# zyt334/AdaFace

Hardware: AMD Instinct MI355X
Metric: 512x512 images/sec @ 50 DDIM steps, batch 8 (higher is better)
Workload: dtype bf16

## Files before the change

### adaface_amd/_lib.py

```python
from __future__ import annotations

import ctypes as C
import os
from pathlib import Path

AF_DTYPE_BF16 = 0
AF_DTYPE_F32 = 1
AF_DTYPE_F16 = 2
DTYPES = {"bf16": AF_DTYPE_BF16, "bfloat16": AF_DTYPE_BF16, "f32": AF_DTYPE_F32, "fp32": AF_DTYPE_F32,
          "float32": AF_DTYPE_F32, "f16": AF_DTYPE_F16, "fp16": AF_DTYPE_F16, "float16": AF_DTYPE_F16}

_LIB_PATH = Path(__file__).resolve().parent / "libadaface_hip.so"


class AfConfig(C.Structure):
    _fields_ = [
        ("dtype", C.c_int),
        ("build_unet", C.c_int),
        ("in_channels", C.c_int), ("model_channels", C.c_int), ("out_channels", C.c_int),
        ("num_res_blocks", C.c_int),
        ("n_attention_resolutions", C.c_int), ("attention_resolutions", C.c_int * 8),
        ("n_channel_mult", C.c_int), ("channel_mult", C.c_int * 8),
        ("num_heads", C.c_int), ("context_dim", C.c_int), ("transformer_depth", C.c_int),
        ("n_context_layers", C.c_int),
        ("build_vae", C.c_int),
        ("vae_ch", C.c_int), ("vae_out_ch", C.c_int), ("vae_num_res_blocks", C.c_int),
        ("vae_z_channels", C.c_int), ("vae_embed_dim", C.c_int),
        ("n_vae_ch_mult", C.c_int), ("vae_ch_mult", C.c_int * 8),
        ("build_vae_encoder", C.c_int), ("vae_in_channels", C.c_int),
        ("build_clip", C.c_int),
        ("clip_vocab", C.c_int), ("clip_hidden", C.c_int), ("clip_layers", C.c_int), ("clip_heads", C.c_int),
        ("clip_intermediate", C.c_int), ("clip_max_pos", C.c_int),
    ]


class AfError(RuntimeError):
    pass


_lib = None

_P = C.c_void_p
_SIGS = [
    ("af_last_error", C.c_char_p, []),
    ("af_version", C.c_int, []),
    ("af_create", C.c_int, [C.c_int, C.POINTER(AfConfig), C.POINTER(_P)]),
    ("af_destroy", None, [_P]),
    ("af_load_tensor", C.c_int, [_P, C.c_char_p, _P, C.c_int, C.POINTER(C.c_int64)]),
    ("af_load_tensor_device", C.c_int, [_P, C.c_char_p, _P, C.c_int, C.POINTER(C.c_int64)]),
    ("af_num_tensors", C.c_int, [_P]),
    ("af_tensor_name", C.c_char_p, [_P, C.c_int]),
    ("af_tensor_loaded", C.c_int, [_P, C.c_int]),
    ("af_tensor_shape", C.c_int, [_P, C.c_int, C.POINTER(C.c_int64)]),
    ("af_set_context", C.c_int, [_P, _P, C.c_int, C.c_int, C.c_int, _P]),
    ("af_unet_forward", C.c_int, [_P, _P, _P, _P, C.c_int, C.c_int, C.c_int, _P]),
    ("af_unet_forward_twin", C.c_int, [_P, _P, _P, _P, C.c_int, C.c_int, C.c_int, _P]),
    ("af_ddim_step", C.c_int, [_P, _P, _P, _P, C.c_int64, C.c_float, C.c_float, C.c_float, C.c_float, C.c_float,
                               C.c_float, _P, _P, _P]),
    ("af_lincomb", C.c_int, [_P, C.c_int64, _P, C.c_float, _P, C.c_float, _P, C.c_float, _P, C.c_float, C.c_int, _P]),
    ("af_vae_decode", C.c_int, [_P, _P, C.c_float, _P, _P, C.c_int, C.c_int, C.c_int, _P]),
    ("af_to_uint8", C.c_int, [_P, _P, C.c_int, C.c_int, C.c_int, _P]),
    ("af_arena_bytes", C.c_int64, [_P]),
    ("af_prof_enable", C.c_int, [C.c_int]),
    ("af_prof_reset", C.c_int, []),
    ("af_set_conv_attn", C.c_int, [_P, C.c_int, C.c_int, C.POINTER(C.c_int), C.POINTER(C.c_int)]),
    ("af_vae_encode", C.c_int, [_P, _P, _P, C.c_int, C.c_int, C.c_int, _P]),
    ("af_posterior_sample", C.c_int, [_P, _P, C.c_float, _P, C.c_int, C.c_int, C.c_int, _P]),
    ("af_prof_set_stride", C.c_int, [C.c_int]),
    ("af_last_gemm_plan", C.c_int, [C.POINTER(C.c_int), C.POINTER(C.c_int), C.POINTER(C.c_int)]),
    ("af_prof_collect", C.c_int, [C.c_int, C.POINTER(C.c_double), C.POINTER(C.c_int64), C.POINTER(C.c_double),
                                  C.POINTER(C.c_double)]),
    ("af_prof_event_overhead_us", C.c_double, [_P, C.c_int]),
    ("af_unet_num_blocks", C.c_int, [_P]),
    ("af_unet_block_shape", C.c_int, [_P, C.c_int, C.c_int, C.c_int, C.POINTER(C.c_int), C.POINTER(C.c_int), C.POINTER(C.c_int)]),
    ("af_unet_set_tap", C.c_int, [_P, C.c_int, _P]),
    ("af_gemm_plan_counts", C.c_int, [C.POINTER(C.c_int64)]),
    ("af_gemm_plan_counts_reset", C.c_int, []),
    ("af_knob_set", C.c_int, [C.c_char_p, C.c_int]),
    ("af_knob_get", C.c_int, [C.c_char_p, C.POINTER(C.c_int)]),
    ("af_knob_reset", C.c_int, []),
    ("af_op_conv2d", C.c_int, [C.c_int, _P, _P, _P, _P, _P] + [C.c_int] * 9 + [_P]),
    ("af_op_linear", C.c_int, [C.c_int, _P, _P, _P, _P, _P, C.c_int64, C.c_int, C.c_int, C.c_int, _P]),
    ("af_op_groupnorm", C.c_int, [C.c_int, _P, _P, _P, C.c_float, C.c_int, _P, C.c_int, C.c_int, C.c_int, C.c_int, _P]),
    ("af_op_conv_gn", C.c_int, [_P, _P, _P, _P, _P, _P, C.c_float, C.c_int, _P, _P] + [C.c_int] * 5 + [_P]),
    ("af_set_fp8", C.c_int, [_P, C.c_int]),
    ("af_fp8_gemm_launches", C.c_int64, []),
    ("af_set_fp8_scope", C.c_int, [_P, C.c_int]),
    ("af_get_fp8_scope", C.c_int, [_P]),
    ("af_ff8_launches", C.c_int64, []),
    ("af_op_ff_fp8", C.c_int, [_P] * 4 + [C.c_float] + [_P] * 5 + [C.c_int64] + [C.c_int] * 5 + [_P, _P, _P, C.POINTER(C.c_int), _P]),
    ("af_fp8_num_sites", C.c_int, [_P]),
    ("af_fp8_site_name", C.c_char_p, [_P, C.c_int]),
    ("af_fp8_record", C.c_int, [_P, C.c_int, _P]),
    ("af_fp8_read_record", C.c_int, [_P, C.c_int, C.POINTER(C.c_float), C.POINTER(C.c_int64), _P]),
    ("af_fp8_get_shifts", C.c_int, [_P, C.c_int, C.POINTER(C.c_int)]),
    ("af_fp8_set_shifts", C.c_int, [_P, C.c_int, C.POINTER(C.c_int)]),
    ("af_fp8_shift_for_amax", C.c_int, [C.c_float, C.c_int]),
    ("af_halo8_launches", C.c_int64, []),
    ("af_rowpanel_launches", C.c_int64, []),
    ("af_up_phase4_launches", C.c_int64, []),
    ("af_gn_producer_launches", C.c_int64, []),
    ("af_attn_short_launches", C.c_int64, []),
    ("af_gn_consumer_launches", C.c_int64, []),
    ("af_xattn_fused_launches", C.c_int64, []),
    ("af_conv_attn_short_launches", C.c_int64, []),
    ("af_op_conv_attention", C.c_int, [C.c_int, _P, _P, _P, _P] + [C.c_int] * 6 + [C.c_float] + [C.c_int] * 3 + [_P]),
    ("af_op_xattn_fused", C.c_int, [C.c_void_p] * 10 + [C.c_int] * 3 + [C.c_void_p]),
    ("af_op_conv2d_fp8", C.c_int, [_P, _P, _P, _P, _P] + [C.c_int] * 10 + [_P]),
    ("af_op_groupnorm_fp8", C.c_int, [_P, _P, _P, C.c_float, C.c_int, _P, C.c_int, C.c_int, C.c_int, C.c_int, C.c_int, _P]),
    ("af_op_layernorm_fp8", C.c_int, [_P, _P, _P, C.c_float, _P, C.c_int64, C.c_int, C.c_int, _P]),
    ("af_op_groupnorm_fp8_rec", C.c_int, [_P, _P, _P, C.c_float, C.c_int, _P, C.c_int, C.c_int, C.c_int, C.c_int, C.c_int, _P, _P]),
    ("af_op_layernorm_fp8_rec", C.c_int, [_P, _P, _P, C.c_float, _P, C.c_int64, C.c_int, C.c_int, _P, _P]),
    ("af_op_layernorm", C.c_int, [C.c_int, _P, _P, _P, C.c_float, _P, C.c_int64, C.c_int, _P]),
    ("af_op_attention", C.c_int, [C.c_int, _P, _P, _P, _P, C.c_int, C.c_int, C.c_int, C.c_int, C.c_int, C.c_float, C.c_int, _P]),
    ("af_clip_embed_tokens", C.c_int, [_P, _P, C.c_int64, _P, _P]),
    ("af_clip_text_forward", C.c_int, [_P, _P, C.c_int, C.c_int, C.c_float, C.c_float, _P, _P]),
    ("af_clip_text_forward3", C.c_int, [_P, _P, C.c_int, C.c_int, C.c_float, C.c_float, C.c_float, _P, _P]),
    ("af_op_timestep_embedding", C.c_int, [C.c_int, _P, _P, C.c_int, C.c_int, _P]),
    ("af_op_gn_conv1x1", C.c_int, [_P, _P, _P, C.c_float, _P, _P, _P, _P] + [C.c_int] * 5 + [_P]),
    ("af_flops_issued", C.c_double, [C.c_int]),
    ("af_clock_probe", C.c_int, [_P, C.c_int, C.POINTER(C.c_double), C.POINTER(C.c_double)]),
]
EXPORTED_SYMBOLS = [s[0] for s in _SIGS]


def lib_path() -> Path:
    return _LIB_PATH


def load():
    global _lib
    if _lib is not None:
        return _lib
    if not _LIB_PATH.exists():
        raise AfError(
            f"{_LIB_PATH} not found: build it with `python -m adaface_amd.build` (needs hipcc). "
            "adaface_amd has no fallback path.")
    lib = C.CDLL(os.fspath(_LIB_PATH))
    for name, res, args in _SIGS:
        fn = getattr(lib, name)
        fn.restype = res
        fn.argtypes = args
    _lib = lib
    return lib


def set_knob(name: str, value: int) -> None:
    check(load().af_knob_set(name.encode(), int(value)), f"af_knob_set({name})")


def reset_knobs() -> None:
    load().af_knob_reset()


def plan_counts(reset: bool = False) -> dict:
    lib = load()
    c = (C.c_int64 * 10)()
    check(lib.af_gemm_plan_counts(c), "af_gemm_plan_counts")
    out = {f"tile{i}": int(c[i]) for i in range(6)}
    out["halo"], out["splitk"], out["ln_consumer"], out["ln_producer"] = int(c[6]), int(c[7]), int(c[8]), int(c[9])
    out["fp8"] = int(lib.af_fp8_gemm_launches())
    out["ff8"] = int(lib.af_ff8_launches())
    out["halo8"] = int(lib.af_halo8_launches())
    out["rowpanel"] = int(lib.af_rowpanel_launches())
    out["up_phase4"] = int(lib.af_up_phase4_launches())
    out["gn_producer"] = int(lib.af_gn_producer_launches())
    out["attn_short"] = int(lib.af_attn_short_launches())
    out["gn_consumer"] = int(lib.af_gn_consumer_launches())
    out["xattn_fused"] = int(lib.af_xattn_fused_launches())
    out["conv_attn_short"] = int(lib.af_conv_attn_short_launches())
    if reset:
        lib.af_gemm_plan_counts_reset()
    return out


def check(rc: int, what: str = "") -> None:
    if rc != 0:
        msg = load().af_last_error().decode("utf-8", "replace")
        raise AfError(f"{what or 'libadaface_hip'} failed (rc={rc}): {msg}")


def stream_ptr():
    import torch
    return C.c_void_p(torch.cuda.current_stream().cuda_stream)


def ptr(t):
    return C.c_void_p(0 if t is None else t.data_ptr())
```

### adaface_amd/csrc/af_common.h

```cpp
#pragma once
#include <hip/hip_runtime.h>
#include <stdint.h>
#include <atomic>

typedef __bf16 bf16;
typedef __attribute__((ext_vector_type(8))) __bf16 bf16x8;
typedef _Float16 f16;
typedef __attribute__((ext_vector_type(8))) _Float16 f16x8;
enum AfStorage { AF_ST_BF16 = 0, AF_ST_F32 = 1, AF_ST_F16 = 2 };
template <typename T> struct StorageOf;
template <> struct StorageOf<__bf16> { static constexpr AfStorage value = AF_ST_BF16; };
template <> struct StorageOf<float> { static constexpr AfStorage value = AF_ST_F32; };
template <> struct StorageOf<_Float16> { static constexpr AfStorage value = AF_ST_F16; };
typedef __attribute__((ext_vector_type(16))) float f32x16;
typedef __attribute__((ext_vector_type(4))) float f32x4;

#define AF_WAVE 64

#define HIP_CHECK_RET(expr)                                                       \
  do {                                                                            \
    hipError_t _e = (expr);                                                       \
    if (_e != hipSuccess) {                                                       \
      af_set_error_msg("%s failed: %s (%s:%d)", #expr, hipGetErrorString(_e),     \
                       __FILE__, __LINE__);                                       \
// ... 32 lines not shown
    if (on) af_prof_begin_impl(cls, s, flops, bytes);
  }
  ~AfProfScope() {
    if (on) af_prof_end_impl(s);
  }
};

struct AfKnobs {
  int splitk_target;
  int conv_halo;
  int gemm_pp;
  int gemm_pp_minfill;
  int gemm_tile;
  int gemm_splitk;
  int gemm_groupm;
  int gemm_dma;
  int attn_ring;
  int gn_small;
  int ln_fuse;
  int geglu_rowpanel;
  int conv_halo8;
  int ablate;
  int gn_producer;
  int conv_up_phase4;
  int attn_short;
  int gemm_m128;
  int small_m_tile64;
  int gn_consumer;
  int xattn_fused;
  int plan_log;
  int ff8_min_k;
  int ff8_min_rows;
  int conv_attn_short;
};
extern AfKnobs g_af_knobs;

template <typename T> __device__ __forceinline__ float to_f32(T v);
template <> __device__ __forceinline__ float to_f32<float>(float v) { return v; }
template <> __device__ __forceinline__ float to_f32<bf16>(bf16 v) { return (float)v; }
template <> __device__ __forceinline__ float to_f32<f16>(f16 v) { return (float)v; }

template <typename T> __device__ __forceinline__ T from_f32(float v);
template <> __device__ __forceinline__ float from_f32<float>(float v) { return v; }
template <> __device__ __forceinline__ bf16 from_f32<bf16>(float v) { return (bf16)v; }
template <> __device__ __forceinline__ f16 from_f32<f16>(float v) { return (f16)v; }

template <typename T> struct Vec16 {
  static constexpr int N = 16 / sizeof(T);
  union {
    uint4 u;
    T e[N];
  };
};

template <typename T> struct Quad;
template <> struct Quad<bf16> {
  union {
    uint2 u;
    bf16 e[4];
  };
  __device__ __forceinline__ void load(const bf16* p) { u = *reinterpret_cast<const uint2*>(p); }
  __device__ __forceinline__ void store(bf16* p) const { *reinterpret_cast<uint2*>(p) = u; }
};
template <> struct Quad<f16> {
  union {
    uint2 u;
// ... 109 lines not shown
    c = __builtin_amdgcn_mfma_f32_32x32x2f32(__builtin_bit_cast(float, a.y),
                                             __builtin_bit_cast(float, b.y), c, 0, 0, 0);
    c = __builtin_amdgcn_mfma_f32_32x32x2f32(__builtin_bit_cast(float, a.z),
                                             __builtin_bit_cast(float, b.z), c, 0, 0, 0);
    c = __builtin_amdgcn_mfma_f32_32x32x2f32(__builtin_bit_cast(float, a.w),
                                             __builtin_bit_cast(float, b.w), c, 0, 0, 0);
  }
};

__device__ __forceinline__ int acc_row(int r, int h) { return (r & 3) + 8 * (r >> 2) + 4 * h; }

enum { AF_EPI_NONE = 0, AF_EPI_GEGLU = 1 };

struct ConvGemmParams {
  const void* src;
  long src_batch_stride;
  int ldc;
  int Cin;
  int Hs, Ws;
  int up;
  int Hi, Wi;
  int Ho, Wo;
  int ks, stride, pad;
  const void* W;
  int ldw;
  int Wrows;
  int M, N, K;
  int k_logical;
  const float* bias;
  const void* rowbias;
  int ldrb;
  const void* residual;
  int ldr;
  void* out;
  int ldo;
  int epilogue;
  float alpha;
  long bs_src, bs_w, bs_out, bs_res;
  int splitk;
  void* ws;
  int group_m;
  int howo_shift, wo_shift;
  float* ln_stats_out;
  const float* ln_stats;
  const float* ln_colsum;
  int ln_parts_n;
  float ln_inv_count, ln_eps;
  int epi_direct;
  int ablate;
  int fp8;
  const unsigned char* w_scale;
  int x_scale_e8;
  const void* W_up4;
  int phase4;
  float* gn_stats_out;
  int gn_cpg;
  const float* gn_ab;
  int gn_hw;
};

struct AfGemmPlan {
  int tile;
  int splitk;
  size_t ws_bytes;
  int halo_tw;
  int group_m;
// ... 13 lines not shown
```

### adaface_amd/csrc/af_conv_gemm.hip

```cpp
#include "af_kernels.h"

#include <cstdlib>
#include <cstring>
#include <mutex>
#include <type_traits>

template <int BM, int BN> struct TileCfg {
  static constexpr int XR = BM / 32, WR = BN / 32;
  static constexpr int WM = BM / 2, WN = BN / 2;
  static constexpr int MI = WM / 32, NI = WN / 32;
  static constexpr int TILE_BYTES = (BM + BN) * 128;
  static constexpr int EPI_LD = BN + 4;
  static constexpr int EPI_BYTES = BM * EPI_LD * 4;
  static constexpr int LDS_BYTES = (2 * TILE_BYTES > EPI_BYTES) ? 2 * TILE_BYTES : EPI_BYTES;
};

__device__ __forceinline__ void lds_dma16(__amdgpu_buffer_rsrc_t rs, char* lds_base, unsigned voffset, unsigned soffset) {
#if defined(__HIP_DEVICE_COMPILE__)
  __builtin_amdgcn_raw_ptr_buffer_load_lds(rs, (__attribute__((address_space(3))) void*)lds_base, 16, voffset, soffset,
                                           0, 0);
#endif
}

__device__ __forceinline__ void tile_coords(int wg, int nwg, int ntm, int ntn, int gm, int& tm, int& tn) {
// ... 1016 lines not shown
  static constexpr int KC = KC_, MJ = MJ_, K = KC * 64, D = D_, NS = D_ + 1;
  static constexpr int WROWS = 16 * MJ, BM = 8 * WROWS;
  static constexpr int BN = GEGLU ? 128 : 160;
  static constexpr int WBYTES = BN * 128, WPIECES = BN / 8;
  static constexpr int NIW = BN / 16;
  static constexpr int OCOLS = GEGLU ? BN / 2 : BN;
  static constexpr int OPITCH = OCOLS * 2 + 16, OBYTES = WROWS * OPITCH;
  static constexpr int LDS_BYTES = NS * WBYTES + 8 * OBYTES;
  static constexpr int CPR = OCOLS / 8;
  static constexpr int NST = WROWS * CPR / 64;
  static_assert(LDS_BYTES <= 160 * 1024 && (WROWS * CPR) % 64 == 0 && (MJ * KC == 10 || (MJ == 1 && KC == 20)) && D >= 2 && D <= KC,
                "row-panel LDS / store mapping / 80 (K = 1280, 16 rows per wave: 160) fragment registers / ring depth");
};
typedef RowPanelCfgT<true> RowPanelCfg;

template <bool GEGLU, int LNMODE, bool RES, int KC_ = 5, int MJ_ = 2, int D_ = 2>
__global__ __launch_bounds__(512) void rowpanel_kernel(const ConvGemmParams p) {
  using C = RowPanelCfgT<GEGLU, KC_, MJ_, D_>;
  typedef bf16 T;
  constexpr int KC = C::KC, NIW = C::NIW, MJ = C::MJ, NST = C::NST, CPR = C::CPR, D = C::D, NS = C::NS;
  static_assert(!(GEGLU && (RES || LNMODE == 2)), "GEGLU: plain or LayerNorm-consumer epilogue, no residual");
  extern __shared__ __attribute__((aligned(1024))) char smem[];
  const int tid = threadIdx.x, lane = tid & 63, wid = __builtin_amdgcn_readfirstlane(tid >> 6);
  const int m0 = blockIdx.x * C::BM;
  const int r0 = m0 + wid * C::WROWS;
  const int ntn_all = p.N / C::BN;
  const int nt_begin = (int)((long)blockIdx.y * ntn_all / gridDim.y), nt_end = (int)((long)(blockIdx.y + 1) * ntn_all / gridDim.y);
  const int ntn = nt_end - nt_begin;
  const __amdgpu_buffer_rsrc_t rs_x = __builtin_amdgcn_make_buffer_rsrc(
      const_cast<T*>(reinterpret_cast<const T*>(p.src)), 0, (int)0xFFFFFFF0u, 0x00020000);
  const __amdgpu_buffer_rsrc_t rs_w = __builtin_amdgcn_make_buffer_rsrc(
      const_cast<T*>(reinterpret_cast<const T*>(p.W)), 0, (int)0xFFFFFFF0u, 0x00020000);
  const __amdgpu_buffer_rsrc_t rs_o = __builtin_amdgcn_make_buffer_rsrc(reinterpret_cast<T*>(p.out), 0, (int)0xFFFFFFF0u, 0x00020000);

  float* vecs = reinterpret_cast<float*>(smem + C::LDS_BYTES);
  const int nvcol = ntn * C::BN;
  float4 vb[3], vc[3];
#pragma unroll
  for (int r = 0; r < 3; ++r) {
    const int c4 = tid + 512 * r;
    const int col = nt_begin * C::BN + 4 * c4;
    vb[r] = vc[r] = float4{0.f, 0.f, 0.f, 0.f};
    if (c4 < nvcol / 4) {
      if (p.bias) vb[r] = *reinterpret_cast<const float4*>(p.bias + col);
      if constexpr (LNMODE == 1) vc[r] = *reinterpret_cast<const float4*>(p.ln_colsum + col);
    }
  }

  pp_u32x4 xr[MJ][KC][2];
  unsigned orow[NST];
#pragma unroll
  for (int i = 0; i < NST; ++i) {
    const int c = lane + 64 * i;
    const int row = c / CPR, ch = c - row * CPR;
    const int m = r0 + row;
    orow[i] = m < p.M ? (unsigned)((long)m * p.ldo * 2) + (unsigned)ch * 16u : 0xFFFFFFFFu;
  }
  float ln_mu[LNMODE == 1 ? MJ : 1], ln_rs[LNMODE == 1 ? MJ : 1];
#pragma unroll
  for (int j = 0; j < MJ; ++j) {
    const int m = r0 + j * 16 + (lane & 15);
    const bool ok = m < p.M;
    const unsigned xo = ok ? (unsigned)((long)m * p.ldc * 2) + (unsigned)(lane >> 4) * 16u : 0xFFFFFFFFu;
#pragma unroll
    for (int kc = 0; kc < KC; ++kc)
#pragma unroll
// ... 197 lines not shown
        }
      }
    } else {
      constexpr int NH = NIW / 2;
      static_assert(NIW % 2 == 0, "row-panel: even number of 16-column blocks");
      float ps[MJ], pq[MJ];
#pragma unroll
      for (int j = 0; j < MJ; ++j) ps[j] = pq[j] = 0.f;
#pragma unroll
      for (int hh = 0; hh < 2; ++hh) {
        float4 bvec[NH], cvec[LNMODE == 1 ? NH : 1];
        {
          const unsigned va = lds0 + (unsigned)C::LDS_BYTES + (unsigned)((ntl * C::BN + hh * NH * 16 + cl) * 4);
          pp_u32x4 tb[NH], tc[LNMODE == 1 ? NH : 1];
          pp_static_for<0, NH>([&](auto ic) {
            constexpr int ii = decltype(ic)::value;
            tb[ii] = pp_lds_read128<ii * 64>(va);
            if constexpr (LNMODE == 1) tc[ii] = pp_lds_read128<ii * 64>(va + (unsigned)nvcol * 4u);
          });
          pp_wait_lgkm0();
#pragma unroll
          for (int ii = 0; ii < NH; ++ii) {
            asm volatile("" : "+v"(tb[ii]));
            bvec[ii] = __builtin_bit_cast(float4, tb[ii]);
            if constexpr (LNMODE == 1) { asm volatile("" : "+v"(tc[ii])); cvec[ii] = __builtin_bit_cast(float4, tc[ii]); }
          }
        }
#pragma unroll
        for (int j = 0; j < MJ; ++j) {
          const int m = r0 + j * 16 + (lane & 15);
          const bool mok = m < p.M;
          Quad<T> rq[RES ? NH : 1];
          if constexpr (RES) {
            const T* rp = reinterpret_cast<const T*>(p.residual) + (long)(mok ? m : 0) * p.ldr + ncol + hh * NH * 16 + cl;
#pragma unroll
            for (int ii = 0; ii < NH; ++ii) rq[ii].load(rp + ii * 16);
          }
#pragma unroll
          for (int ii = 0; ii < NH; ++ii) {
            const int i = hh * NH + ii;
            const float* bp = reinterpret_cast<const float*>(&bvec[ii]);
            const float* cp = reinterpret_cast<const float*>(&cvec[LNMODE == 1 ? ii : 0]);
            Quad<T> o;
#pragma unroll
            for (int e = 0; e < 4; ++e) {
              float v;
              if constexpr (LNMODE == 1) v = (acc[i][j][e] - ln_mu[j] * cp[e]) * ln_rs[j] + bp[e];
              else v = acc[i][j][e] * p.alpha + bp[e];
              if constexpr (RES) v += to_f32<T>(rq[ii].e[e]);
              o.e[e] = from_f32<T>(v);
              if constexpr (LNMODE == 2) {
                const float vr = mok ? to_f32<T>(o.e[e]) : 0.f;
                ps[j] += vr;
                pq[j] += vr * vr;
              }
            }
            o.store(reinterpret_cast<T*>(otile + (j * 16 + (lane & 15)) * C::OPITCH) + i * 16 + cl);
          }
        }
        __builtin_amdgcn_sched_barrier(0);
      }
      if constexpr (LNMODE == 2) {
#pragma unroll
        for (int j = 0; j < MJ; ++j) {
          const int m = r0 + j * 16 + (lane & 15);
          float s1 = ps[j], s2 = pq[j];
          s1 += __shfl_xor(s1, 16, 64); s2 += __shfl_xor(s2, 16, 64);
// ... 1062 lines not shown
  const int lvl = g_af_knobs.geglu_rowpanel;
  if (!lvl || batch != 1 || p.ks != 1 || p.pad != 0 || p.stride != 1 || p.up != 0 || p.splitk > 1 || p.rowbias || p.fp8 ||
      p.Cin != p.K || p.ldc < p.Cin)
    return 0;
  const bool geglu = p.epilogue == AF_EPI_GEGLU;
  if (p.K == RowPanelCfg::K && p.M >= 128 * RowPanelCfg::BM) {
    if (p.gn_ab && (p.gn_hw <= 0 || p.gn_hw % RowPanelCfg::BM != 0)) return 0;
    if (geglu) return (p.N % RowPanelCfg::BN == 0 && !p.residual && !p.ln_stats_out) ? 1 : 0;
    return (lvl >= 2 && p.N % 160 == 0 && p.alpha == 1.0f && !(p.ln_stats && p.ln_stats_out) && (!p.residual || p.ldr % 4 == 0)) ? 2 : 0;
  }
  if (g_af_knobs.gemm_m128 && !geglu && !(p.ln_stats && p.ln_stats_out) && (!p.ln_stats || p.alpha == 1.0f) && !p.gn_ab && p.M % 128 == 0 &&
      p.M <= 8192 && p.N % 160 == 0 &&
      p.K % 64 == 0 && p.K >= 256 && (!p.residual || p.ldr % 4 == 0) && p.ldo % 8 == 0 && ((__UINTPTR_TYPE__)p.out & 15) == 0) {
    const long nb128 = (long)(p.M / 128) * (p.N / 160), nb256 = (long)((p.M + 255) / 256) * (p.N / 160);
    if (nb128 >= 128 && nb128 <= 512 && nb256 <= 170) return 6;
    if (nb128 % 256 == 0 && nb128 <= 1024 && nb256 % 256 != 0) return 6;
  }
  if (g_af_knobs.gemm_m128 && !geglu && !(p.ln_stats && p.ln_stats_out) && (!p.ln_stats || p.alpha == 1.0f) && !p.gn_ab && p.M % 128 == 0 &&
      p.M > 8192 && p.M <= 16384 && p.N % 160 == 0 && p.K % 64 == 0 && p.K >= 256 && p.K <= 1280 && (!p.residual || p.ldr % 4 == 0) &&
      p.ldo % 8 == 0 && ((__UINTPTR_TYPE__)p.out & 15) == 0 && (long)(p.M / 128) * (p.N / 160) == 512)
    return 6;
  if (p.K == 1280)
    return (lvl >= 4 && p.N == 1280 && p.M >= 4096 && !geglu && p.alpha == 1.0f && !p.ln_stats && !p.ln_stats_out && !p.gn_ab &&
            (!p.residual || p.ldr % 4 == 0)) ? 3 : 0;
  if (p.K == 640 && lvl >= 3 && p.M >= 16384 && !p.residual) {
    if (p.gn_ab) return 0;
    if (p.ln_stats_out) return 0;
    if (geglu) return p.N % 128 == 0 ? 4 : 0;
    return (p.N % 160 == 0 && p.N >= 1920 && p.alpha == 1.0f) ? 5 : 0;
  }
  return 0;
}

template <typename T>
int af_launch_conv_gemm(const ConvGemmParams& p_in, int batch, hipStream_t stream, const AfGemmPlan* plan, void* ws) {
  constexpr int BK = 128 / sizeof(T);
  ConvGemmParams p = p_in;
  if (p.fp8) {
    if constexpr (std::is_same_v<T, bf16>) return batch == 1 ? launch_conv_gemm_fp8(p, stream, plan, ws) : (af_set_error_msg("conv_gemm fp8: no batched form"), -1);
    else { af_set_error_msg("conv_gemm: fp8 operands need the bf16 storage mode"); return -1; }
  }
  if (p.gn_ab && !std::is_same_v<T, bf16>) { af_set_error_msg("conv_gemm: consumer-side GroupNorm exists on the bf16 row-panel kernels only"); return -1; }
  if (p.K % BK != 0 || p.Cin % BK != 0 || p.K != p.ks * p.ks * p.Cin) {
    af_set_error_msg("conv_gemm: K=%d Cin=%d ks=%d must satisfy K==ks*ks*Cin and Cin%%%d==0", p.K, p.Cin, p.ks, BK);
    return -1;
  }
  if (p.ldw % (16 / (int)sizeof(T)) != 0 || p.ldc % (16 / (int)sizeof(T)) != 0) {
    af_set_error_msg("conv_gemm: ldw/ldc must be multiples of 16 bytes");
    return -1;
  }
  if (p.N % 4 != 0 || p.ldo % 4 != 0 || (p.residual && p.ldr % 4 != 0) || (p.rowbias && p.ldrb % 4 != 0)) {
    af_set_error_msg("conv_gemm: N/ldo/ldr/ldrb must be multiples of 4 (N=%d ldo=%d)", p.N, p.ldo);
    return -1;
  }
  if (p.epilogue == AF_EPI_GEGLU && p.N % 64 != 0) { af_set_error_msg("conv_gemm: GEGLU needs N%%64==0"); return -1; }
  if (p.M <= 0 || p.N <= 0) return 0;
  {
    const int HoWo = p.Ho * p.Wo > 0 ? p.Ho * p.Wo : 1;
    const double nb = (double)((p.M + HoWo - 1) / HoWo);
    const double src_bytes = nb * (double)p.src_batch_stride * sizeof(T), w_bytes = (double)p.Wrows * p.ldw * sizeof(T);
    if (src_bytes >= 4294967280.0 || w_bytes >= 4294967280.0) {
      af_set_error_msg("conv_gemm: operand of %.2f GB exceeds the 4 GB range of the 32-bit gather offsets (split the batch)",
                       (src_bytes > w_bytes ? src_bytes : w_bytes) / 1e9);
      return -1;
    }
  }
  if constexpr (std::is_same_v<T, bf16>) {
    if (up_phase4_ok(p, batch)) return launch_up_phase4(p, stream);
  }
  AfGemmPlan pl = plan ? *plan : af_plan_conv_gemm(p, batch, StorageOf<T>::value);
  if (pl.splitk > 1 && !ws) pl.splitk = 1;
  if constexpr (std::is_same_v<T, bf16>) {
    if (pl.splitk > 1) {
      ConvGemmParams q = p;
// ... 13 lines not shown
  if (pl.splitk > 1) g_af_plan_counts[7] += 1;
  if (p.ln_stats) g_af_plan_counts[8] += 1;
  if (p.ln_stats_out) g_af_plan_counts[9] += 1;
  set_launch_fields(p, pl);
  if (p.gn_stats_out) {
    if (!std::is_same_v<T, bf16> || batch != 1 || !af_conv_gn_stats_ok(p, pl, p.gn_cpg)) {
      af_set_error_msg("conv_gemm: GroupNorm partial sums asked of a launch that cannot write them (ask af_conv_gn_stats_ok first)");
      return -1;
    }
    g_af_plan_counts[14] += 1;
  }
  const int prof_cls = pl.halo_tw == 256 ? AF_K_HALO8
                       : pl.tile == 5 ? ((p.ks == 1 && p.pad == 0) ? AF_K_PP160_PLAIN : AF_K_PP160_GATHER)
                                      : (pl.tile == 4 ? AF_K_PP128 : AF_K_CONV_GEMM);
  AfProfScope prof(prof_cls, stream, 2.0 * p.M * (double)p.N * (p.k_logical ? p.k_logical : p.K) * batch,
                   ((double)p.M * p.K / (p.ks * p.ks) + (double)p.N * p.K + (double)p.M * p.N) * batch * sizeof(T));
  int rc;
  int rk_pre = 0;
  if constexpr (std::is_same_v<T, bf16>) rk_pre = af_conv_rowpanel_kind(p, batch);
  if ((p.ln_stats || p.ln_stats_out) && rk_pre != 6 && !(pl.tile >= 4 && !pl.halo_tw)) {
    af_set_error_msg("conv_gemm: LayerNorm-fused launch planned on a kernel without that epilogue (tile %d)", pl.tile);
    return -1;
  }
  if constexpr (std::is_same_v<T, bf16>) {
    const int rk = rk_pre;
    if (p.ln_parts_n > 0 && !rk) {
      af_set_error_msg("conv_gemm: un-finalised LayerNorm statistics handed to a launch that is not a row-panel one");
      return -1;
    }
    if (p.gn_ab && !rk) {
      af_set_error_msg("conv_gemm: consumer-side GroupNorm asked of a launch that is not a row-panel one (ask af_conv_rowpanel_kind first)");
      return -1;
    }
    if (p.gn_ab) g_af_gn_consumer_launches += 1;
    if (rk) g_af_plan_counts[12] += 1;
    switch (rk) {
      case 1: return launch_geglu_rowpanel(p, stream);
      case 2: return launch_plain_rowpanel(p, stream);
      case 3: return launch_plain_rowpanel_k1280(p, stream);
      case 4: return launch_geglu_rowpanel(p, stream, true);
      case 5: return launch_plain_rowpanel(p, stream, true);
      case 6: return launch_gemm_m128(p, stream);
      default: break;
    }
  }
  if (pl.halo_tw == 8 || pl.halo_tw == 256) {
    if constexpr (std::is_same_v<T, bf16>) {
      rc = pl.halo_tw == 8 ? af_launch_conv_s8(p, stream) : launch_halo8(p, stream);
    } else {
      af_set_error_msg(pl.halo_tw == 8 ? "conv_gemm: the 8 x 8-map kernel is bf16 only" : "conv_gemm: the eight-wave halo kernel is bf16 only");
      return -1;
    }
  } else if (pl.halo_tw) {
    const bool bn128 = pl.tile == 0 || pl.tile == 1;
    if (pl.halo_tw == 32) return bn128 ? launch_halo<T, 32, 128>(p, stream) : launch_halo<T, 32, 64>(p, stream);
    return bn128 ? launch_halo<T, 16, 128>(p, stream) : launch_halo<T, 16, 64>(p, stream);
  } else {
    switch (pl.tile) {
      case 4:
      case 5:
        if constexpr (std::is_same_v<T, bf16>) {
          rc = pl.tile == 4 ? launch_pp<128>(p, stream) : launch_pp<160>(p, stream);
        } else {
          af_set_error_msg("conv_gemm: ping-pong tiles are bf16 only");
          return -1;
        }
// ... 15 lines not shown
```

### adaface_amd/csrc/af_kernels.h

```cpp
#pragma once
#include "af_common.h"

AfGemmPlan af_plan_conv_gemm(const ConvGemmParams& p, int batch, AfStorage st);
template <typename T>
int af_launch_conv_gemm(const ConvGemmParams& p, int batch, hipStream_t stream, const AfGemmPlan* plan = nullptr,
                        void* ws = nullptr);
template <typename T> int af_launch_attention(const AttnParams& p, int B, int dh, hipStream_t stream);
template <typename T> long af_attn_short_pack_elems(int B, int H, int dh, int Nk);
template <typename T>
int af_launch_attn_short_pack(const void* v, int ldv, long bsv, int Nk, int H, int dh, int B, void* vt, hipStream_t stream);
extern std::atomic<long> g_af_attn_short_launches;
bool af_conv_attn_short_ok(bool is_bf16, int dh, int Nk, bool vt_pack, int ks, int groups);
int af_launch_conv_attn_short(const AttnParams& p, int B, int dh, int ks, int groups, int Hh, int Ww, const float* amap,
                              hipStream_t stream);
extern std::atomic<long> g_af_conv_attn_short_launches;
struct AfXattnFusedParams {
  const void* x; int ldx; int M; int rows_per_sample;
  const float* ln_stats; int ln_parts_n; float ln_inv_count, ln_eps;
  const void* wq; int ldwq; const float* q_colsum; const float* q_bias;
  const void* kvpack;
  const void* wo; int ldwo; const float* o_bias;
  void* out; int ldo;
  float* ln_stats_out;
  int Nk;
};
bool af_xattn_fused_ok(int M, int rows_per_sample, int C, int H, int dh, int Nk);
long af_xattn_fused_pack_elems(int B, int H, int dh, int Nk);
int af_launch_xattn_fused_pack(const void* kv, int ldk, long bsk, int Nk, int B, void* pack, hipStream_t stream);
int af_launch_xattn_fused_permute_wo(const void* w, int ldw, int rows, void* wp, int ldp, hipStream_t stream);
int af_launch_xattn_fused(const AfXattnFusedParams& a, hipStream_t stream);
extern std::atomic<long> g_af_xattn_fused_launches;

bool af_ff_geglu_fp8_ok(const ConvGemmParams& p);
int af_launch_ff_geglu_fp8(ConvGemmParams p, float out_mul, unsigned* rec, hipStream_t stream);
extern std::atomic<long> g_af_ff8_launches;

size_t af_gn_workspace_bytes(int B, int HW);
template <typename T>
int af_launch_groupnorm(const void* x, long x_bs, int ldx, int B, int HW, int Cn, const float* gamma,
                        const float* beta, float eps, int silu, void* y, long y_bs, int ldy, void* workspace,
                        hipStream_t stream, float fp8_mul = 0.f,
                        const float* pre_partial = nullptr, int pre_npart = 0,
                        unsigned* fp8_rec = nullptr);
template <typename T>
int af_launch_groupnorm_fold(const void* x, long x_bs, int ldx, int B, int HW, int Cn, const float* gamma, const float* beta,
                             float eps, void* workspace, hipStream_t stream, const float* pre_partial, int pre_npart,
                             float* ab_out);
bool af_conv_gn_stats_ok(const ConvGemmParams& p, const AfGemmPlan& pl, int cpg);
bool af_conv_s8_ok(const ConvGemmParams& p, int batch);
int af_conv_s8_slices(const ConvGemmParams& p, int batch);
int af_launch_conv_s8(const ConvGemmParams& p, hipStream_t stream);
int af_conv_rowpanel_kind(const ConvGemmParams& p, int batch);
template <typename T>
int af_launch_layernorm(const void* x, int ldx, long rows, int Cn, const float* gamma, const float* beta,
                        float eps, void* y, int ldy, hipStream_t stream, float fp8_mul = 0.f, unsigned* fp8_rec = nullptr);

template <typename T>
int af_launch_nchw_to_nhwc(const float* x, void* y, int B, int Cn, int HW, int Cpad, float scale, hipStream_t s);
template <typename T> int af_launch_nhwc_to_nchw(const void* x, float* y, int B, int Cn, int HW, int ld, hipStream_t s);
template <typename T> int af_launch_cast_f32(const float* x, void* y, long n, hipStream_t s);
template <typename T>
int af_launch_gather_rows_cast(const float* x, const int* rowmap, void* y, long rows, int D, hipStream_t s);
template <typename T>
int af_launch_conv_attn(const void* q, int ldq, long bsq, const void* kv, int ldk, long bsk, int tok0, float* sN,
// ... 49 lines not shown
```

### adaface_amd/csrc/af_model.hip

```cpp
#include "../../include/adaface_hip.h"
#include "af_kernels.h"

#include <cmath>
#include <cstdarg>
#include <cstdio>
#include <cstdlib>
#include <cstring>
#include <algorithm>
#include <map>
#include <memory>
#include <string>
#include <vector>

static thread_local char g_err[1024] = "";
void af_set_error_msg(const char* fmt, ...) {
  va_list ap;
  va_start(ap, fmt);
  vsnprintf(g_err, sizeof(g_err), fmt, ap);
  va_end(ap);
}
static int knob_env(const char* name, int dflt) {
  const char* s = getenv(name);
  return s ? atoi(s) : dflt;
}
AfKnobs g_af_knobs = {
    knob_env("AF_SPLITK_TARGET", 320), knob_env("AF_CONV_HALO", 1),       knob_env("AF_GEMM_PP", 1),
    knob_env("AF_GEMM_PP_MINFILL", 50), knob_env("AF_GEMM_TILE", -1),
    knob_env("AF_GEMM_SPLITK", -1),    knob_env("AF_GEMM_GROUPM", -1),    knob_env("AF_GEMM_DMA", -1),
    knob_env("AF_ATTN_RING", 3),       knob_env("AF_GN_SMALL", 1),
    knob_env("AF_LN_FUSE", 1),         knob_env("AF_GEGLU_ROWPANEL", 4), knob_env("AF_CONV_HALO8", 3), knob_env("AF_ABLATE", 0),
    knob_env("AF_GN_PRODUCER", 1),     knob_env("AF_CONV_UP_PHASE4", 1), knob_env("AF_ATTN_SHORT", 1),
    knob_env("AF_GEMM_M128", 1),       knob_env("AF_SMALL_M_TILE64", 1),  knob_env("AF_GN_CONSUMER", 1),
    knob_env("AF_XATTN_FUSED", 1),     knob_env("AF_PLAN_LOG", 0),      knob_env("AF_FF8_MIN_K", 512),   knob_env("AF_FF8_MIN_ROWS", 0),
    knob_env("AF_CONV_ATTN_SHORT", 1)};
static const AfKnobs g_af_knobs_initial = g_af_knobs;
static int* knob_slot(const char* name) {
  static const struct { const char* n; int AfKnobs::*m; } tab[] = {
      {"splitk_target", &AfKnobs::splitk_target}, {"conv_halo", &AfKnobs::conv_halo}, {"gemm_pp", &AfKnobs::gemm_pp},
      {"gemm_pp_minfill", &AfKnobs::gemm_pp_minfill},
      {"gemm_tile", &AfKnobs::gemm_tile}, {"gemm_splitk", &AfKnobs::gemm_splitk}, {"gemm_groupm", &AfKnobs::gemm_groupm},
      {"gemm_dma", &AfKnobs::gemm_dma}, {"attn_ring", &AfKnobs::attn_ring},
      {"gn_small", &AfKnobs::gn_small}, {"ln_fuse", &AfKnobs::ln_fuse},
      {"geglu_rowpanel", &AfKnobs::geglu_rowpanel}, {"conv_halo8", &AfKnobs::conv_halo8}, {"ablate", &AfKnobs::ablate}, {"gn_producer", &AfKnobs::gn_producer}, {"conv_up_phase4", &AfKnobs::conv_up_phase4},
      {"attn_short", &AfKnobs::attn_short},
      {"gemm_m128", &AfKnobs::gemm_m128}, {"small_m_tile64", &AfKnobs::small_m_tile64}, {"gn_consumer", &AfKnobs::gn_consumer}, {"xattn_fused", &AfKnobs::xattn_fused}, {"plan_log", &AfKnobs::plan_log}, {"ff8_min_k", &AfKnobs::ff8_min_k}, {"ff8_min_rows", &AfKnobs::ff8_min_rows},
      {"conv_attn_short", &AfKnobs::conv_attn_short}};
  if (!name) return nullptr;
  for (auto& t : tab)
    if (strcmp(t.n, name) == 0) return &(g_af_knobs.*(t.m));
  return nullptr;
}

int g_af_prof_enabled = 0;
int g_af_prof_stride = 1;
std::atomic<long> g_af_prof_seen[AF_K_COUNT] = {};
std::atomic<double> g_af_flops_issued{0.0};
namespace {
struct ProfRec {
  hipEvent_t start, stop;
  int cls;
  double flops, bytes;
};
std::vector<ProfRec> g_prof_recs;
std::vector<hipEvent_t> g_prof_pool;
size_t g_prof_pool_used = 0;
hipEvent_t prof_event() {
  if (g_prof_pool_used == g_prof_pool.size()) {
    hipEvent_t e;
    hipEventCreate(&e);
    g_prof_pool.push_back(e);
  }
  return g_prof_pool[g_prof_pool_used++];
}
}
void af_prof_begin_impl(int cls, hipStream_t s, double flops, double bytes) {
  ProfRec r;
  r.start = prof_event();
  r.stop = prof_event();
  r.cls = cls;
// ... 151 lines not shown
  std::vector<VLevel> vlevels;
  Linear quant_conv, enc_conv_in, enc_conv_out;
  Norm enc_norm_out;
  VaeAttnW eattn;
  std::vector<Linear> edown;
  int emid1 = -1, emid2 = -1;
  std::vector<VLevel> elevels;

  void* clip_tok = nullptr;
  void* clip_pos = nullptr;
  std::vector<ClipLayerW> clip_layers;
  Norm clip_final_ln;

  int conv_ks = 0;
  std::vector<int> conv_batch;
  std::vector<int> conv_tokens;
  int* ctx_rowmap = nullptr;
  size_t ctx_rowmap_n = 0;

  bool ln_fold_dirty = true;
  bool fp8_on = false;
  bool fp8_dirty = true;
  int fp8_scope = AF_FP8_SCOPE_BASE;
  int fp8_nbase = 0;
  int fp8_nsites() const { return (fp8_scope & AF_FP8_SCOPE_FF) ? (int)fp8_shift.size() : fp8_nbase; }
  std::vector<int> fp8_shift;
  std::vector<std::string> fp8_site_names;
  unsigned* fp8_rec = nullptr;
  bool fp8_recording = false;
  bool up4_dirty = true;
  float* gn_carry = nullptr;
  size_t gn_carry_bytes = 0, gn_carry_need = 0;

  int tap_index = -1;
  float* tap_out = nullptr;

  Arena arena;
  float* stage = nullptr;
  size_t stage_bytes = 0;
  std::vector<CtxKV> ctx_kv;
  void* ctx_cast = nullptr;
  size_t ctx_cast_bytes = 0;
  int ctx_Bf = 0, ctx_tokens = 0;
  bool ctx_set = false;
};

struct Builder {
  af_handle* h;
  int rc = 0;
  void* dmalloc(size_t bytes, bool zero = true) {
    void* p = nullptr;
    if (hipMalloc(&p, bytes) != hipSuccess) {
      af_set_error_msg("hipMalloc(%zu) failed", bytes);
      rc = AF_ERR_HIP;
      return nullptr;
    }
    if (zero) hipMemset(p, 0, bytes);
    h->owned.push_back(p);
    return p;
  }
  void add_slot(const std::string& name, const Slot& s) {
    h->slots[name] = s;
    h->slot_names.push_back(name);
  }
  void alloc_linear(Linear& L, int cin, int cout_rows, int ks, bool pad_cin) {
    const int bk = bk_of(h->dtype);
// ... 489 lines not shown
    Act f8 = x8;
    f8.C = f8.ld = ff2.cin;
    ConvGemmParams p;
    conv_params(p, ff1, x8, f8, 1, 0, nullptr, nullptr, 0, ff1.cout, -1);
    return af_ff_geglu_fp8_ok(p) && fp8_capable(ff2, f8, out);
  }
  int ff_geglu8(const Linear& L, const Act& x8, Act& y8) {
    AF_TRY(check(y8));
    if (!x8.f8 || !y8.f8 || !L.w8) { af_set_error_msg("ff_geglu8: e4m3 operands and an fp8 weight twin needed"); return AF_ERR_STATE; }
    ConvGemmParams p;
    conv_params(p, L, x8, y8, 1, 0, nullptr, nullptr, 0, L.cout, -1);
    if (dry) return 0;
    return af_launch_ff_geglu_fp8(p, ldexpf(1.f, y8.f8_shift), fp8_rec_of(y8), s);
  }
  int ln_capable(const Linear& L, const Act& x, const Act& out, int n_valid = -1) const {
    if (dt != AF_DTYPE_BF16 || L.ks != 1) return 0;
    ConvGemmParams p;
    conv_params(p, L, x, out, 1, 0, nullptr, nullptr, 0, n_valid, -1);
    const AfGemmPlan pl = af_plan_conv_gemm(p, 1, storage_of(dt));
    if (pl.tile < 4 || pl.splitk > 1 || pl.halo_tw) return 0;
    return (p.N / (pl.tile == 5 ? 160 : 128)) * 2;
  }
  bool rowpanel_capable(const Linear& L, const Act& x, const Act& out, const LnArgs* ln, int gn_hw) const {
    if (dt != AF_DTYPE_BF16 || L.ks != 1 || x.f8) return false;
    ConvGemmParams p;
    conv_params(p, L, x, out, 1, 0, nullptr, nullptr, 0, -1, -1);
    if (ln) { p.ln_stats = ln->stats; p.ln_colsum = ln->colsum; p.ln_stats_out = ln->stats_out; }
    p.gn_ab = reinterpret_cast<const float*>(1);
    p.gn_hw = gn_hw;
    const AfGemmPlan pl = af_plan_conv_gemm(p, 1, storage_of(dt));
    p.splitk = pl.splitk;
    return af_conv_rowpanel_kind(p, 1) != 0;
  }
  int groupnorm_fold(const Norm& N, const Act& x, float* ab) {
    const int HW = x.H * x.W;
    void* ws = A.alloc(af_gn_workspace_bytes(x.B, HW));
    if (!ws || !ab) { af_set_error_msg("arena exhausted (groupnorm fold)"); return AF_ERR_STATE; }
    if (dry) return 0;
    if (x.C != N.C) { af_set_error_msg("groupnorm: C mismatch %d vs %d", x.C, N.C); return AF_ERR_INVALID; }
    const float* pre = g_af_knobs.gn_producer ? x.gn_part : nullptr;
    return DISPATCH(dt, af_launch_groupnorm_fold<bf16>(x.p, (long)HW * x.ld, x.ld, x.B, HW, x.C, N.gamma, N.beta, N.eps, ws, s, pre, x.gn_npart, ab),
                    af_launch_groupnorm_fold<float>(x.p, (long)HW * x.ld, x.ld, x.B, HW, x.C, N.gamma, N.beta, N.eps, ws, s, pre, x.gn_npart, ab),
                    af_launch_groupnorm_fold<f16>(x.p, (long)HW * x.ld, x.ld, x.B, HW, x.C, N.gamma, N.beta, N.eps, ws, s, pre, x.gn_npart, ab));
  }
  int conv(const Linear& L, const Act& x, Act& out, int stride, int up, const Act* residual, const void* rowbias,
           int ldrb, int n_valid = -1, int pad = -1, const LnArgs* ln = nullptr, int want_gn = 0) {
    AF_TRY(check(out));
    out.gn_part = nullptr; out.gn_npart = 0;
    ConvGemmParams p;
    conv_params(p, L, x, out, stride, up, residual, rowbias, ldrb, n_valid, pad);
    bool ln_parts_pending = false;
    if (ln) {
      p.ln_stats = ln->stats; p.ln_colsum = ln->colsum;
      p.ln_stats_out = ln->stats_out;
      if (ln->parts_in) {
        p.ln_stats = ln->stats_buf;
        ln_parts_pending = true;
      }
      p.gn_ab = ln->gn_ab;
      p.gn_hw = ln->gn_hw;
    }
    if (x.C < L.cin || x.ld < L.cin_pad) {
      af_set_error_msg("conv: input has %d channels (ld %d), layer expects %d (padded %d)", x.C, x.ld, L.cin, L.cin_pad);
      return AF_ERR_INVALID;
    }
    if (x.f8 && (!L.w8 || ln)) { af_set_error_msg("conv: e4m3 input without an fp8 weight twin"); return AF_ERR_STATE; }
    const AfGemmPlan pl = af_plan_conv_gemm(p, 1, storage_of(dt));
    if (x.f8 && pl.tile < 4) { af_set_error_msg("conv: e4m3 input on a shape without an fp8 plan"); return AF_ERR_STATE; }
    if (ln_parts_pending) {
      ConvGemmParams q = p;
      q.splitk = pl.splitk;
      int kind = dt == AF_DTYPE_BF16 ? af_conv_rowpanel_kind(q, 1) : 0;
      if (!kind && dt == AF_DTYPE_BF16 && pl.splitk > 1) {
        q.splitk = 1;
        if (af_conv_rowpanel_kind(q, 1) == 6) kind = 6;
      }
      if (kind) {
        p.ln_stats = ln->parts_in;
        p.ln_parts_n = ln->parts_n;
        p.ln_inv_count = 1.0f / (float)ln->count;
        p.ln_eps = ln->eps;
      } else {
        AF_TRY(ln_finalize(ln->parts_in, ln->parts_n, (long)p.M, ln->count, ln->eps, ln->stats_buf));
// ... 92 lines not shown

static int run_resblock(Runner& R, const ResBlockW& w, const Act& x, Act& out, const void* emb_all, int emb_ld) {
  const size_t mk = R.A.mark();
  Act t2 = R.alloc_act(x.B, x.H, x.W, w.cout);
  Act t1 = R.fp8_capable(w.c1, x, t2) ? R.alloc_act8(x.B, x.H, x.W, x.C, w.c1) : R.alloc_act(x.B, x.H, x.W, x.C);
  AF_TRY(R.groupnorm(w.n1, x, t1, 1));
  const void* rb = (emb_all && w.emb_off >= 0) ? R.elem_ptr(const_cast<void*>(emb_all), w.emb_off) : nullptr;
  AF_TRY(R.conv(w.c1, t1, t2, 1, 0, nullptr, rb, emb_ld, -1, -1, nullptr, 1));
  Act t3 = R.fp8_capable(w.c2, t2, out) ? R.alloc_act8(x.B, x.H, x.W, w.cout, w.c2) : R.alloc_act(x.B, x.H, x.W, w.cout);
  AF_TRY(R.groupnorm(w.n2, t2, t3, 1));
  Act sk = x;
  if (w.has_skip) {
    sk = R.alloc_act(x.B, x.H, x.W, w.cout);
    AF_TRY(R.conv(w.skip, x, sk, 1, 0, nullptr, nullptr, 0));
  }
  AF_TRY(R.conv(w.c2, t3, out, 1, 0, &sk, nullptr, 0, -1, -1, nullptr, 2));
  R.A.release(mk);
  return 0;
}

static int run_xfmr(Runner& R, const XfmrW& w, const Act& x, Act& out, bool twin = false) {
  af_handle* h = R.h;
  const size_t mk = R.A.mark();
  const int Bh = x.B, B = twin ? 2 * x.B : x.B, H = x.H, W = x.W, N = H * W, C = w.heads * w.dh;
  auto half = [&](Act a) { if (twin) a.B = Bh; return a; };
  auto dup = [&](const Act& a) -> int {
    Act src = a, dst = a;
    src.B = dst.B = Bh;
    dst.p = R.elem_ptr(a.p, (long)Bh * a.H * a.W * a.ld);
    return R.copy_channels(src, dst, 0);
  };
  Act g = R.alloc_act(B, H, W, x.C);
  Act t = R.alloc_act(B, H, W, C);
  Act f_probe = t;
  f_probe.C = 4 * C; f_probe.ld = 4 * C;
  Act qkv_probe = t;
  qkv_probe.C = 3 * C; qkv_probe.ld = 3 * C;
  int ln_parts = 0;
  if (g_af_knobs.ln_fuse && !w.blocks.empty() && w.blocks[0].qkv1_ln.w) {
    const XfmrBlockW& b0 = w.blocks[0];
    const int pp = R.ln_capable(w.proj_in, g, t);
    const bool ok = pp > 0 && R.ln_capable(b0.out1, t, t) == pp && R.ln_capable(b0.out2, t, t) == pp &&
                    R.ln_capable(b0.ff2, f_probe, t) == pp && R.ln_capable(b0.qkv1_ln, t, qkv_probe) > 0 &&
                    R.ln_capable(b0.q2_ln, t, t) > 0 && R.ln_capable(b0.ff1_ln, t, f_probe, 8 * C) > 0;
    if (ok) ln_parts = pp;
    if (ok && twin) {
      const Act gh = half(g), th = half(t), qh = half(qkv_probe);
      if (R.ln_capable(w.proj_in, gh, th) != pp || R.ln_capable(b0.out1, th, th) != pp || R.ln_capable(b0.qkv1_ln, th, qh) <= 0)
        ln_parts = 0;
    }
  }
  const size_t st_elems = (size_t)ln_parts * B * N * 2;
  float* st_part = ln_parts ? reinterpret_cast<float*>(R.A.alloc(st_elems * sizeof(float))) : nullptr;
  float* st_row = ln_parts ? reinterpret_cast<float*>(R.A.alloc((size_t)B * N * 2 * sizeof(float))) : nullptr;
  if (ln_parts && !st_row) { af_set_error_msg("arena exhausted (LayerNorm statistics)"); return AF_ERR_STATE; }
  float *st_t = st_part, *st_1 = st_part, *st_2 = st_part;
  auto producer = [&](float* st) { Runner::LnArgs a; a.stats_out = st; return a; };
  auto consumer = [&](const float* st, const float* cs, const Norm& ln) {
    Runner::LnArgs a; a.colsum = cs;
    a.parts_in = st; a.parts_n = ln_parts; a.count = C; a.eps = ln.eps;
    a.stats_buf = st_row;
    return a;
  };
  auto consumer_final = [&](const float* cs) {
    Runner::LnArgs a; a.colsum = cs;
    a.stats = st_row;
// ... 24 lines not shown
    const bool pre = twin && d == 0;
    const int Bp = pre ? Bh : B;
    auto pv = [&](Act a) { a.B = Bp; return a; };
    Act n = R.alloc_act(B, H, W, C);
    Act qkv = R.alloc_act(B, H, W, 3 * C);
    {
      const Act tp = pv(t);
      Act np = pv(n), qkvp = pv(qkv);
      if (R.fp8_capable(blk.qkv1, tp, qkvp)) {
        Act n8 = R.alloc_act8(Bp, H, W, C, blk.qkv1);
        AF_TRY(R.layernorm(blk.ln1, tp, n8));
        AF_TRY(R.conv(blk.qkv1, n8, qkvp, 1, 0, nullptr, nullptr, 0));
      } else if (ln_parts) {
        const Runner::LnArgs ca = consumer(st_t, blk.qkv1_cs, blk.ln1);
        AF_TRY(R.conv(blk.qkv1_ln, tp, qkvp, 1, 0, nullptr, nullptr, 0, -1, -1, &ca));
      } else {
        AF_TRY(R.layernorm(blk.ln1, tp, np));
        AF_TRY(R.conv(blk.qkv1, np, qkvp, 1, 0, nullptr, nullptr, 0));
      }
    }
    Act a = R.alloc_act(B, H, W, C);
    {
      Act ap = pv(a);
      AF_TRY(R.attention(qkv.p, 3 * C, (long)N * 3 * C, R.elem_ptr(qkv.p, C), 3 * C, (long)N * 3 * C,
                         R.elem_ptr(qkv.p, 2 * C), 3 * C, (long)N * 3 * C, ap, N, N, w.heads, w.dh));
    }
    Act t1 = R.alloc_act(B, H, W, C);
    {
      const Runner::LnArgs pa = producer(st_1);
      const Act ap = pv(a), tp = pv(t);
      Act t1p = pv(t1);
      AF_TRY(R.conv(blk.out1, ap, t1p, 1, 0, &tp, nullptr, 0, -1, -1, ln_parts ? &pa : nullptr));
    }
    if (pre) {
      AF_TRY(R.check(t1));
      AF_TRY(dup(t1));
      AF_TRY(dup(x));
    }
    const CtxKV& kv = h->ctx_kv[w.ca_slot + d];
    const int S = h->ctx_tokens;
    if (!R.dry && (!kv.kv || h->ctx_Bf != B)) {
      af_set_error_msg("context not set for batch %d (af_set_context)", B);
      return AF_ERR_STATE;
    }
    const int ca_layer = (w.ca_slot + (int)d) / (int)w.blocks.size();
    const bool conv_attn = h->conv_ks >= 2 && !h->conv_batch.empty() && !(ca_layer >= 6 && ca_layer <= 10);
    Act t2 = R.alloc_act(B, H, W, C);
    Act q = R.alloc_act(B, H, W, C);
    const bool fused_ca = g_af_knobs.xattn_fused && R.dt == AF_DTYPE_BF16 && ln_parts == 4 && !conv_attn && blk.out2_perm && blk.q2_ln.w &&
                          t1.ld == C && t2.ld == C && af_xattn_fused_ok(B * N, N, C, w.heads, w.dh, S > 0 ? S : 77);
    if (fused_ca) {
      AF_TRY(R.check(t2));
      if (pre) AF_TRY(finalize(st_1, blk.ln2, (long)Bh * N));
      if (pre && !R.dry)
        HIP_CHECK_RET(hipMemcpyAsync(st_row + (size_t)Bh * N * 2, st_row, (size_t)Bh * N * 2 * sizeof(float), hipMemcpyDeviceToDevice, R.s));
      if (!R.dry) {
        if (!kv.xf_pack) { af_set_error_msg("fused cross-attention: no K / V pack for this layer (af_set_context)"); return AF_ERR_STATE; }
        AfXattnFusedParams a;
        memset(&a, 0, sizeof(a));
        a.x = t1.p; a.ldx = t1.ld; a.M = B * N; a.rows_per_sample = N;
        if (pre) { a.ln_stats = st_row; a.ln_parts_n = 0; }
        else { a.ln_stats = st_1; a.ln_parts_n = ln_parts; a.ln_inv_count = 1.0f / (float)C; a.ln_eps = blk.ln2.eps; }
        a.wq = blk.q2_ln.w; a.ldwq = blk.q2_ln.ldw; a.q_colsum = blk.q2_cs; a.q_bias = blk.q2_ln.bias;
        a.kvpack = kv.xf_pack;
        a.wo = blk.out2_perm; a.ldwo = blk.out2.ldw; a.o_bias = blk.out2.bias;
        a.out = t2.p; a.ldo = t2.ld;
        a.ln_stats_out = st_2;
        a.Nk = S;
        AF_TRY(af_launch_xattn_fused(a, R.s));
      }
    } else {
    if (ln_parts) {
      Runner::LnArgs ca = consumer(st_1, blk.q2_cs, blk.ln2);
      if (pre) {
        AF_TRY(finalize(st_1, blk.ln2, (long)Bh * N));
        if (!R.dry)
          HIP_CHECK_RET(hipMemcpyAsync(st_row + (size_t)Bh * N * 2, st_row, (size_t)Bh * N * 2 * sizeof(float), hipMemcpyDeviceToDevice, R.s));
        ca = consumer_final(blk.q2_cs);
      }
      AF_TRY(R.conv(blk.q2_ln, t1, q, 1, 0, nullptr, nullptr, 0, -1, -1, &ca));
    } else {
      AF_TRY(R.layernorm(blk.ln2, t1, n));
      AF_TRY(R.conv(blk.q2, n, q, 1, 0, nullptr, nullptr, 0));
    }
    if (!conv_attn) {
      AF_TRY(R.attention(q.p, C, (long)N * C, kv.kv, 2 * C, (long)S * 2 * C, R.dry ? nullptr : R.elem_ptr(kv.kv, C),
                         2 * C, (long)S * 2 * C, a, N, S, w.heads, w.dh, 0, -1, nullptr, 0, kv.vt, B > 0 ? kv.vt_bytes / (size_t)B : 0));
    } else {
      const size_t mk3 = R.A.mark();
      const int nt = h->conv_ks * h->conv_ks;
      auto groups = [&](int b) { return (int)std::count(h->conv_batch.begin(), h->conv_batch.end(), b); };
      int ng_max = 0;
      for (int b = 0; b < B; ++b) ng_max = std::max(ng_max, groups(b));
// ... 53 lines not shown
        }
        b0 = b1;
      }
      R.A.release(mk3);
    }
    {
      const Runner::LnArgs pa = producer(st_2);
      AF_TRY(R.conv(blk.out2, a, t2, 1, 0, &t1, nullptr, 0, -1, -1, ln_parts ? &pa : nullptr));
    }
    }
    if (!(ln_parts && d + 1 < w.blocks.size()) && R.ff8_capable(blk.ff1, blk.ff2, t2, t)) {
      Act n8 = R.alloc_act8(B, H, W, C, blk.ff1);
      AF_TRY(R.layernorm(blk.ln3, t2, n8));
      Act f8 = R.alloc_act8(B, H, W, 4 * C, blk.ff2);
      AF_TRY(R.ff_geglu8(blk.ff1, n8, f8));
      AF_TRY(R.conv(blk.ff2, f8, t, 1, 0, &t2, nullptr, 0));
      R.A.release(mk2);
      continue;
    }
    Act f = R.alloc_act(B, H, W, 4 * C);
    if (ln_parts) {
      const Runner::LnArgs ca = consumer(st_2, blk.ff1_cs, blk.ln3);
      AF_TRY(R.conv(blk.ff1_ln, t2, f, 1, 0, nullptr, nullptr, 0, 8 * C, -1, &ca));
    } else {
      AF_TRY(R.layernorm(blk.ln3, t2, n));
      AF_TRY(R.conv(blk.ff1, n, f, 1, 0, nullptr, nullptr, 0, 8 * C));
    }
    {
      const Runner::LnArgs pa = producer(st_t);
      AF_TRY(R.conv(blk.ff2, f, t, 1, 0, &t2, nullptr, 0, -1, -1, (ln_parts && d + 1 < w.blocks.size()) ? &pa : nullptr));
    }
    R.A.release(mk2);
  }
  {
    Act xf = x;
    xf.B = B;
    AF_TRY(R.conv(w.proj_out, t, out, 1, 0, &xf, nullptr, 0));
  }
  R.A.release(mk);
  return 0;
}

static int fold_layernorms(af_handle* h, hipStream_t s) {
  if (!h->ln_fold_dirty || h->dtype != AF_DTYPE_BF16) { h->ln_fold_dirty = false; return 0; }
  for (auto& x : h->xf)
    for (auto& t : x.blocks) {
      if (!t.qkv1_ln.w) continue;
      const int C = x.heads * x.dh;
      AF_TRY(af_launch_ln_fold<bf16>(t.qkv1.w, t.qkv1_ln.w, t.ln1.gamma, t.ln1.beta, t.qkv1.bias, t.qkv1_cs, t.qkv1_ln.bias,
                                     t.qkv1.rows_pad, C, t.qkv1.ldw, s));
      AF_TRY(af_launch_ln_fold<bf16>(t.q2.w, t.q2_ln.w, t.ln2.gamma, t.ln2.beta, t.q2.bias, t.q2_cs, t.q2_ln.bias,
                                     t.q2.rows_pad, C, t.q2.ldw, s));
      AF_TRY(af_launch_ln_fold<bf16>(t.ff1.w, t.ff1_ln.w, t.ln3.gamma, t.ln3.beta, t.ff1.bias, t.ff1_cs, t.ff1_ln.bias,
                                     t.ff1.rows_pad, C, t.ff1.ldw, s));
      if (t.out2_perm) AF_TRY(af_launch_xattn_fused_permute_wo(t.out2.w, t.out2.ldw, C, t.out2_perm, t.out2.ldw, s));
    }
  h->ln_fold_dirty = false;
  return 0;
}

static std::vector<Linear*> fp8_twin_list(af_handle* h, int scope) {
  std::vector<Linear*> twins;
  if (scope & AF_FP8_SCOPE_BASE) {
    for (auto& r : h->res) { twins.push_back(&r.c1); twins.push_back(&r.c2); }
    for (auto& x : h->xf)
      for (auto& t : x.blocks) twins.push_back(&t.qkv1);
  }
  if (scope & AF_FP8_SCOPE_FF)
    for (auto& x : h->xf)
      for (auto& t : x.blocks) {
        if (t.ff1.cin_pad % 64 != 0 || t.ff2.cin_pad % 64 != 0) continue;
// ... 72 lines not shown
    AF_TRY(af_launch_up_phase4_weights(L->w, L->rows_pad, L->cin_pad, L->ldw, L->w_up4, s));
  }
  return 0;
}

static int ensure_gn_carry(af_handle* h, hipStream_t s) {
  if (h->gn_carry_need <= h->gn_carry_bytes) return 0;
  HIP_CHECK_RET(hipStreamSynchronize(s));
  void* p = nullptr;
  if (hipMalloc(&p, h->gn_carry_need) != hipSuccess) { af_set_error_msg("hipMalloc of the GroupNorm carry buffer failed"); return AF_ERR_HIP; }
  h->owned.push_back(p);
  h->gn_carry = reinterpret_cast<float*>(p);
  h->gn_carry_bytes = h->gn_carry_need;
  return 0;
}

static int ensure_arena(af_handle* h, size_t need) {
  if (need <= h->arena.cap) return 0;
  if (h->arena.base) hipFree(h->arena.base);
  h->arena.base = nullptr;
  h->arena.cap = 0;
  need += need / 16;
  void* p = nullptr;
  if (hipMalloc(&p, need) != hipSuccess) {
    af_set_error_msg("hipMalloc of %zu-byte activation arena failed", need);
    return AF_ERR_HIP;
  }
  h->arena.base = reinterpret_cast<char*>(p);
  h->arena.cap = need;
  return 0;
}

static int unet_forward_impl(af_handle* h, hipStream_t s, const float* x_dev, const int64_t* t_dev, float* eps_dev,
                             int Bf, int H, int W, bool twin = false) {
  Runner R(h, s);
  const af_config& c = h->cfg;
  const int dt = h->dtype;
  const int mc = c.model_channels, ted = 4 * mc;
  R.A.off = 0;
  const int Bin = twin ? Bf / 2 : Bf;
  auto dup_half = [&](const Act& a) -> int {
    Act src = a, dst = a;
    src.B = dst.B = Bin;
    dst.p = R.elem_ptr(a.p, (long)Bin * a.H * a.W * a.ld);
    return R.copy_channels(src, dst, 0);
  };
  const bool twin_prefix = twin && h->input_blocks.size() >= 2 && h->input_blocks[0].layers.size() == 1 &&
                           h->input_blocks[0].layers[0].kind == L_CONV_IN && h->input_blocks[1].layers.size() == 2 &&
                           h->input_blocks[1].layers[0].kind == L_RES && h->input_blocks[1].layers[1].kind == L_XFMR;

  Act x = R.alloc_act(Bf, H, W, c.in_channels, h->conv_in.cin_pad);
  AF_TRY(R.check(x));
  Act temb = R.alloc_act(Bf, 1, 1, mc);
  Act e1 = R.alloc_act(Bf, 1, 1, ted);
  Act e2 = R.alloc_act(Bf, 1, 1, ted);
  Act emb_all = R.alloc_act(Bf, 1, 1, h->emb_total);
  AF_TRY(R.check(emb_all));
  if (!R.dry) {
    AF_TRY(DISPATCH(dt, af_launch_nchw_to_nhwc<bf16>(x_dev, x.p, Bin, c.in_channels, H * W, x.ld, 1.0f, s),
                    af_launch_nchw_to_nhwc<float>(x_dev, x.p, Bin, c.in_channels, H * W, x.ld, 1.0f, s),
                    af_launch_nchw_to_nhwc<f16>(x_dev, x.p, Bin, c.in_channels, H * W, x.ld, 1.0f, s)));
    AF_TRY(DISPATCH(dt, af_launch_timestep_embedding<bf16>((const long long*)t_dev, temb.p, Bin, mc, s),
                    af_launch_timestep_embedding<float>((const long long*)t_dev, temb.p, Bin, mc, s),
                    af_launch_timestep_embedding<f16>((const long long*)t_dev, temb.p, Bin, mc, s)));
  }
  if (twin && !twin_prefix) AF_TRY(dup_half(x));
  {
    Act tb = temb, e1b = e1, e2b = e2, eab = emb_all;
    tb.B = e1b.B = e2b.B = eab.B = Bin;
    AF_TRY(R.conv(h->time_embed0, tb, e1b, 1, 0, nullptr, nullptr, 0));
    if (!R.dry) AF_TRY(DISPATCH(dt, af_launch_silu<bf16>(e1.p, e1.p, (long)Bin * ted, s), af_launch_silu<float>(e1.p, e1.p, (long)Bin * ted, s), af_launch_silu<f16>(e1.p, e1.p, (long)Bin * ted, s)));
    AF_TRY(R.conv(h->time_embed2, e1b, e2b, 1, 0, nullptr, nullptr, 0));
    if (!R.dry) AF_TRY(DISPATCH(dt, af_launch_silu<bf16>(e2.p, e2.p, (long)Bin * ted, s), af_launch_silu<float>(e2.p, e2.p, (long)Bin * ted, s), af_launch_silu<f16>(e2.p, e2.p, (long)Bin * ted, s)));
    AF_TRY(R.conv(h->emb_all, e2b, eab, 1, 0, nullptr, nullptr, 0));
    if (twin) AF_TRY(dup_half(emb_all));
  }

  auto run_block = [&](const UBlock& ub, Act hcur, Act& result, const Act* final_out, int nb, bool twin_x) -> int {
    hcur.B = nb;
    for (size_t li = 0; li < ub.layers.size(); ++li) {
      const LayerRef& l = ub.layers[li];
      const bool use_final = final_out && li + 1 == ub.layers.size();
      Act out;
      auto new_act = [&](int Hh, int Ww, int Cc) -> Act {
        Act v;
        if (use_final) {
          v = *final_out;
          if (v.H != Hh || v.W != Ww || v.C != Cc) v.p = nullptr;
        } else {
          v = R.alloc_act(Bf, Hh, Ww, Cc);
        }
        v.B = nb;
        return v;
      };
      switch (l.kind) {
        case L_CONV_IN: {
          out = new_act(hcur.H, hcur.W, mc);
          Act xin = hcur;
          xin.C = h->conv_in.cin;
          AF_TRY(R.conv(h->conv_in, xin, out, 1, 0, nullptr, nullptr, 0));
        } break;
        case L_RES: {
          const ResBlockW& w = h->res[l.idx];
          out = new_act(hcur.H, hcur.W, w.cout);
          AF_TRY(run_resblock(R, w, hcur, out, emb_all.p, emb_all.ld));
        } break;
        case L_XFMR: {
          out = new_act(hcur.H, hcur.W, hcur.C);
          if (twin_x) {
            out.B = 2 * nb;
            nb = 2 * nb;
            AF_TRY(run_xfmr(R, h->xf[l.idx], hcur, out, true));
          } else {
            AF_TRY(run_xfmr(R, h->xf[l.idx], hcur, out));
          }
        } break;
        case L_DOWN: {
          out = new_act(hcur.H / 2, hcur.W / 2, hcur.C);
          AF_TRY(R.conv(h->updown[l.idx], hcur, out, 2, 0, nullptr, nullptr, 0));
        } break;
        case L_UP: {
          out = new_act(hcur.H * 2, hcur.W * 2, hcur.C);
          AF_TRY(R.conv(h->updown[l.idx], hcur, out, 1, 1, nullptr, nullptr, 0));
        } break;
      }
      hcur = out;
    }
    result = hcur;
    return 0;
  };

  struct Shp { int C, H, W; };
  auto out_shape = [&](const UBlock& ub, Shp in) -> Shp {
    for (auto& l : ub.layers) {
      if (l.kind == L_CONV_IN) in.C = mc;
      else if (l.kind == L_RES) in.C = h->res[l.idx].cout;
      else if (l.kind == L_DOWN) { in.H /= 2; in.W /= 2; }
      else if (l.kind == L_UP) { in.H *= 2; in.W *= 2; }
// ... 319 lines not shown
    int rc = build_vae(b);
    if (rc) { af_destroy(h.release()); return rc; }
    if (cfg->build_vae_encoder) {
      if (cfg->vae_in_channels <= 0) { af_set_error_msg("af_create: vae_in_channels"); af_destroy(h.release()); return AF_ERR_INVALID; }
      rc = build_vae_encoder(b);
      if (rc) { af_destroy(h.release()); return rc; }
    }
  }
  if (cfg->build_clip) {
    if (cfg->clip_vocab <= 0 || cfg->clip_layers <= 0 || cfg->clip_max_pos <= 0) { af_set_error_msg("af_create: bad CLIP config"); af_destroy(h.release()); return AF_ERR_INVALID; }
    int rc = build_clip(b);
    if (rc) { af_destroy(h.release()); return rc; }
  }
  if (b.rc) { af_destroy(h.release()); return b.rc; }
  if (hipError_t e = hipDeviceSynchronize(); e != hipSuccess) {
    af_set_error_msg("af_create: %s", hipGetErrorString(e));
    af_destroy(h.release());
    return AF_ERR_HIP;
  }
  *out = h.release();
  return 0;
}

void af_destroy(af_handle* h) {
  if (!h) return;
  hipSetDevice(h->device);
  hipDeviceSynchronize();
  for (void* p : h->owned) hipFree(p);
  for (auto& kv : h->ctx_kv) { if (kv.kv) hipFree(kv.kv); if (kv.vt) hipFree(kv.vt); if (kv.xf_pack) hipFree(kv.xf_pack); }
  if (h->ctx_rowmap) hipFree(h->ctx_rowmap);
  if (h->ctx_cast) hipFree(h->ctx_cast);
  if (h->arena.base) hipFree(h->arena.base);
  if (h->stage) hipFree(h->stage);
  delete h;
}

int af_num_tensors(af_handle* h) { return h ? (int)h->slot_names.size() : 0; }
const char* af_tensor_name(af_handle* h, int i) {
  if (!h || i < 0 || i >= (int)h->slot_names.size()) return nullptr;
  return h->slot_names[i].c_str();
}
int af_tensor_loaded(af_handle* h, int i) {
  if (!h || i < 0 || i >= (int)h->slot_names.size()) return 0;
  return h->slots[h->slot_names[i]].loaded ? 1 : 0;
}
int af_tensor_shape(af_handle* h, int i, int64_t* shape4) {
  if (!h || i < 0 || i >= (int)h->slot_names.size()) return AF_ERR_INVALID;
  const Slot& s = h->slots[h->slot_names[i]];
  for (int d = 0; d < 4; ++d) shape4[d] = d < (int)s.shape.size() ? s.shape[d] : 0;
  return (int)s.shape.size();
}

static int load_tensor_impl(af_handle* h, const char* name, const float* data, int ndim, const int64_t* shape,
                            bool on_device);
int af_load_tensor(af_handle* h, const char* name, const float* host_data, int ndim, const int64_t* shape) {
  return load_tensor_impl(h, name, host_data, ndim, shape, false);
}
int af_load_tensor_device(af_handle* h, const char* name, const float* dev_data, int ndim, const int64_t* shape) {
  return load_tensor_impl(h, name, dev_data, ndim, shape, true);
}
static int load_tensor_impl(af_handle* h, const char* name, const float* host_data, int ndim, const int64_t* shape,
                            bool on_device) {
  if (!h || !name || !host_data) { af_set_error_msg("af_load_tensor: null argument"); return AF_ERR_INVALID; }
  auto it = h->slots.find(name);
  if (it == h->slots.end()) { af_set_error_msg("af_load_tensor: unknown tensor '%s'", name); return AF_ERR_NAME; }
  Slot& s = it->second;
// ... 10 lines not shown
  HIP_CHECK_RET(hipSetDevice(h->device));
  const size_t bytes = (size_t)n * sizeof(float);
  const float* srcp = host_data;
  if (on_device) {
    HIP_CHECK_RET(hipDeviceSynchronize());
  } else if (bytes > h->stage_bytes) {
    if (h->stage) hipFree(h->stage);
    h->stage = nullptr;
    h->stage_bytes = 0;
    void* p = nullptr;
    HIP_CHECK_RET(hipMalloc(&p, bytes));
    h->stage = reinterpret_cast<float*>(p);
    h->stage_bytes = bytes;
  }
  if (!on_device) {
    HIP_CHECK_RET(hipMemcpy(h->stage, host_data, bytes, hipMemcpyHostToDevice));
    srcp = h->stage;
  }
  if (s.kind == Slot::TABLE) {
    AF_TRY(DISPATCH(h->dtype, af_launch_cast_f32<bf16>(srcp, s.dst, (long)n, 0), af_launch_cast_f32<float>(srcp, s.dst, (long)n, 0), af_launch_cast_f32<f16>(srcp, s.dst, (long)n, 0)));
  } else if (s.kind == Slot::WEIGHT) {
    AF_TRY(DISPATCH(h->dtype,
                    af_launch_repack_weight<bf16>(srcp, s.dst, s.rows, s.cin, s.cin_pad, s.ks, s.ldw, s.row_off, s.perm, 0),
                    af_launch_repack_weight<float>(srcp, s.dst, s.rows, s.cin, s.cin_pad, s.ks, s.ldw, s.row_off, s.perm, 0),
                    af_launch_repack_weight<f16>(srcp, s.dst, s.rows, s.cin, s.cin_pad, s.ks, s.ldw, s.row_off, s.perm, 0)));
  } else {
    AF_TRY(af_launch_permute_bias(srcp, s.dst_f, s.rows, s.perm, 0));
  }
  HIP_CHECK_RET(hipStreamSynchronize(0));
  s.loaded = true;
  h->ln_fold_dirty = true;
  h->fp8_dirty = true;
  h->up4_dirty = true;
  return 0;
}

static int check_loaded(af_handle* h, const char* prefix) {
  for (auto& kv : h->slots)
    if (!kv.second.loaded && kv.first.compare(0, strlen(prefix), prefix) == 0) {
      af_set_error_msg("tensor '%s' has not been loaded (af_load_tensor)", kv.first.c_str());
      return AF_ERR_STATE;
    }
  return 0;
}

int af_set_conv_attn(af_handle* h, int ks, int n_subj, const int* batch_idx, const int* token_idx) {
  if (!h) { af_set_error_msg("af_set_conv_attn: null handle"); return AF_ERR_INVALID; }
  if (ks <= 1 || n_subj <= 0) {
    h->conv_ks = 0; h->conv_batch.clear(); h->conv_tokens.clear();
    h->ctx_set = false;
    return AF_OK;
  }
  if (ks > 4) { af_set_error_msg("af_set_conv_attn: kernel size %d (the reference has 2, 3 and 4: ldm/util.py:747-760)", ks); return AF_ERR_INVALID; }
  if (!batch_idx || !token_idx) { af_set_error_msg("af_set_conv_attn: null index arrays"); return AF_ERR_INVALID; }
  h->conv_ks = ks;
  h->conv_batch.assign(batch_idx, batch_idx + n_subj);
  h->conv_tokens.assign(token_idx, token_idx + (size_t)n_subj * ks * ks);
  h->ctx_set = false;
  return AF_OK;
}

int af_set_context(af_handle* h, const float* ctx_dev, int Bf, int n_tokens, int layerwise, void* stream) {
  if (!h || !ctx_dev || Bf <= 0 || n_tokens <= 0) { af_set_error_msg("af_set_context: bad argument"); return AF_ERR_INVALID; }
  if (!h->cfg.build_unet) { af_set_error_msg("af_set_context: handle has no UNet"); return AF_ERR_STATE; }
  HIP_CHECK_RET(hipSetDevice(h->device));
  AF_TRY(check_loaded(h, "model.diffusion_model."));
// ... 80 lines not shown
                    af_launch_gather_rows_cast<f16>(ctx_dev, h->ctx_rowmap, h->ctx_cast, (long)rows, D, s)));
  } else {
    AF_TRY(DISPATCH(dt, af_launch_cast_f32<bf16>(ctx_dev, h->ctx_cast, (long)n, s), af_launch_cast_f32<float>(ctx_dev, h->ctx_cast, (long)n, s), af_launch_cast_f32<f16>(ctx_dev, h->ctx_cast, (long)n, s)));
  }
  for (size_t i = 0; i < h->ca_list.size(); ++i) {
    const XfmrW& x = h->xf[h->ca_list[i].first];
    const XfmrBlockW& blk = x.blocks[h->ca_list[i].second];
    const int C = x.heads * x.dh;
    const int layer = layerwise ? x.ca_slot / (int)x.blocks.size() : 0;
    ConvGemmParams p;
    memset(&p, 0, sizeof(p));
    p.src = reinterpret_cast<char*>(h->ctx_cast) + (size_t)layer * n_tokens * D * esize(dt);
    p.src_batch_stride = (long)L * n_tokens * D;
    p.ldc = D; p.Cin = D;
    p.Hs = 1; p.Ws = n_tokens; p.Hi = 1; p.Wi = n_tokens; p.Ho = 1; p.Wo = n_tokens;
    p.ks = 1; p.stride = 1; p.pad = 0;
    p.W = blk.kv2.w; p.ldw = blk.kv2.ldw; p.Wrows = blk.kv2.rows_pad;
    p.M = Bf * n_tokens; p.N = 2 * C; p.K = D;
    p.out = h->ctx_kv[i].kv; p.ldo = 2 * C; p.alpha = 1.0f;
    AF_TRY(DISPATCH(dt, af_launch_conv_gemm<bf16>(p, 1, s), af_launch_conv_gemm<float>(p, 1, s), af_launch_conv_gemm<f16>(p, 1, s)));
    if (h->ctx_kv[i].xf_pack)
      AF_TRY(af_launch_xattn_fused_pack(h->ctx_kv[i].kv, 2 * C, (long)n_tokens * 2 * C, n_tokens, Bf,
                                        h->ctx_kv[i].xf_pack, s));
    if (h->ctx_kv[i].vt)
      AF_TRY(af_launch_attn_short_pack<bf16>(reinterpret_cast<char*>(h->ctx_kv[i].kv) + (size_t)C * 2, 2 * C, (long)n_tokens * 2 * C,
                                             n_tokens, x.heads, x.dh, Bf, h->ctx_kv[i].vt, s));
  }
  h->ctx_Bf = Bf;
  h->ctx_tokens = n_tokens;
  h->ctx_set = true;
  return 0;
}

static int unet_forward_entry(af_handle* h, const float* x_dev, const int64_t* t_dev, float* eps_dev, int Bf, int H, int W,
                              void* stream, bool twin) {
  if (!h || !x_dev || !t_dev || !eps_dev) { af_set_error_msg("af_unet_forward: null argument"); return AF_ERR_INVALID; }
  if (twin && (Bf < 2 || Bf % 2)) { af_set_error_msg("af_unet_forward_twin: the batch [x; x] must be even, got %d", Bf); return AF_ERR_INVALID; }
  if (!h->cfg.build_unet) { af_set_error_msg("af_unet_forward: handle has no UNet"); return AF_ERR_STATE; }
  if (!h->ctx_set || h->ctx_Bf != Bf) { af_set_error_msg("af_unet_forward: call af_set_context for batch %d first", Bf); return AF_ERR_STATE; }
  const int down = 1 << (h->cfg.n_channel_mult - 1);
  if (H % down || W % down) { af_set_error_msg("af_unet_forward: H,W must be multiples of %d", down); return AF_ERR_INVALID; }
  HIP_CHECK_RET(hipSetDevice(h->device));
  hipStream_t s = reinterpret_cast<hipStream_t>(stream);
  AF_TRY(fold_layernorms(h, s));
  AF_TRY(ensure_fp8_twins(h, s));
  AF_TRY(ensure_up4_twins(h, s));
  h->arena.dry = true; h->arena.peak = 0;
  int rc = unet_forward_impl(h, s, x_dev, t_dev, eps_dev, Bf, H, W, twin);
  h->arena.dry = false;
  if (rc) return rc;
  if (h->arena.peak > h->arena.cap) { HIP_CHECK_RET(hipStreamSynchronize(s)); AF_TRY(ensure_arena(h, h->arena.peak)); }
  AF_TRY(ensure_gn_carry(h, s));
  return unet_forward_impl(h, s, x_dev, t_dev, eps_dev, Bf, H, W, twin);
}
int af_unet_forward(af_handle* h, const float* x_dev, const int64_t* t_dev, float* eps_dev, int Bf, int H, int W,
                    void* stream) {
  return unet_forward_entry(h, x_dev, t_dev, eps_dev, Bf, H, W, stream, false);
}
int af_unet_forward_twin(af_handle* h, const float* x_dev, const int64_t* t_dev, float* eps_dev, int Bf, int H, int W,
                         void* stream) {
  return unet_forward_entry(h, x_dev, t_dev, eps_dev, Bf, H, W, stream, true);
}

int af_unet_num_blocks(af_handle* h) {
  return (h && h->cfg.build_unet) ? (int)(h->input_blocks.size() + 1 + h->output_blocks.size()) : 0;
}

int af_unet_block_shape(af_handle* h, int block, int H, int W, int* C_out, int* H_out, int* W_out) {
  if (!h || !h->cfg.build_unet || block < 0 || block >= af_unet_num_blocks(h) || !C_out || !H_out || !W_out) {
    af_set_error_msg("af_unet_block_shape: bad argument");
    return AF_ERR_INVALID;
  }
  int C = h->cfg.in_channels, idx = 0;
  auto walk = [&](const UBlock& ub, int skipC) {
    C += skipC;
    for (auto& l : ub.layers) {
      if (l.kind == L_CONV_IN) C = h->cfg.model_channels;
      else if (l.kind == L_RES) C = h->res[l.idx].cout;
      else if (l.kind == L_DOWN) { H /= 2; W /= 2; }
      else if (l.kind == L_UP) { H *= 2; W *= 2; }
    }
  };
  for (auto& ub : h->input_blocks) { walk(ub, 0); if (idx++ == block) goto done; }
  walk(h->middle_block, 0);
  if (idx++ == block) goto done;
  for (auto& ub : h->output_blocks) { walk(ub, 0); if (idx++ == block) goto done; }
// ... 96 lines not shown
  if (!h->cfg.build_vae || !h->cfg.build_vae_encoder) { af_set_error_msg("af_vae_encode: handle has no VAE encoder"); return AF_ERR_STATE; }
  const int f = 1 << (h->cfg.n_vae_ch_mult - 1);
  if (H % f != 0 || W % f != 0) { af_set_error_msg("af_vae_encode: H, W must be multiples of %d", f); return AF_ERR_INVALID; }
  HIP_CHECK_RET(hipSetDevice(h->device));
  AF_TRY(check_loaded(h, "first_stage_model.encoder."));
  AF_TRY(check_loaded(h, "first_stage_model.quant_conv."));
  hipStream_t s = reinterpret_cast<hipStream_t>(stream);
  h->arena.dry = true; h->arena.peak = 0;
  int rc = vae_encode_impl(h, s, x_dev, moments_dev, B, H, W);
  h->arena.dry = false;
  if (rc) return rc;
  if (h->arena.peak > h->arena.cap) { HIP_CHECK_RET(hipStreamSynchronize(s)); AF_TRY(ensure_arena(h, h->arena.peak)); }
  AF_TRY(ensure_gn_carry(h, s));
  return vae_encode_impl(h, s, x_dev, moments_dev, B, H, W);
}

int af_posterior_sample(const float* moments_dev, const float* noise_dev, float scale, float* z_dev, int B, int C,
                        int HW, void* stream) {
  if (!moments_dev || !z_dev || B <= 0 || C <= 0 || HW <= 0) { af_set_error_msg("af_posterior_sample: bad argument"); return AF_ERR_INVALID; }
  return af_launch_posterior_sample(moments_dev, noise_dev, scale, z_dev, B, C, (long)HW, reinterpret_cast<hipStream_t>(stream));
}

int af_to_uint8(const float* img_dev, uint8_t* u8_dev, int B, int H, int W, void* stream) {
  if (!img_dev || !u8_dev) { af_set_error_msg("af_to_uint8: null argument"); return AF_ERR_INVALID; }
  return af_launch_nchw_to_uint8(img_dev, u8_dev, B, H * W, reinterpret_cast<hipStream_t>(stream));
}

int64_t af_arena_bytes(af_handle* h) { return h ? (int64_t)h->arena.cap : 0; }

int af_knob_set(const char* name, int value) {
  int* k = knob_slot(name);
  if (!k) { af_set_error_msg("af_knob_set: unknown knob '%s'", name ? name : "(null)"); return AF_ERR_NAME; }
  *k = value;
  return AF_OK;
}
int af_knob_get(const char* name, int* value) {
  int* k = knob_slot(name);
  if (!k || !value) { af_set_error_msg("af_knob_get: unknown knob '%s'", name ? name : "(null)"); return AF_ERR_NAME; }
  *value = *k;
  return AF_OK;
}
int af_knob_reset(void) {
  g_af_knobs = g_af_knobs_initial;
  return AF_OK;
}

int af_prof_enable(int class_mask) {
  g_af_prof_enabled = class_mask;
  return 0;
}
int af_prof_reset(void) {
  g_prof_recs.clear();
  g_prof_pool_used = 0;
  for (int c = 0; c < AF_K_COUNT; ++c) g_af_prof_seen[c] = 0;
  return 0;
}
double af_flops_issued(int reset) {
  const double v = reset ? g_af_flops_issued.exchange(0.0) : g_af_flops_issued.load();
  return v;
}
int af_prof_set_stride(int every) {
  if (every < 1) { af_set_error_msg("af_prof_set_stride: stride must be >= 1"); return AF_ERR_INVALID; }
  g_af_prof_stride = every;
  return AF_OK;
}
int af_last_gemm_plan(int* tile, int* splitk, int* halo_tw) {
  const AfGemmPlan lp = af_get_last_plan();
  if (tile) *tile = lp.tile;
  if (splitk) *splitk = lp.splitk;
  if (halo_tw) *halo_tw = lp.halo_tw;
  return AF_OK;
}
int af_gemm_plan_counts(int64_t* counts10) {
  if (!counts10) { af_set_error_msg("af_gemm_plan_counts: null argument"); return AF_ERR_INVALID; }
  for (int i = 0; i < 10; ++i) counts10[i] = g_af_plan_counts[i];
  return AF_OK;
}
int af_gemm_plan_counts_reset(void) {
  g_af_attn_short_launches = 0;
  g_af_xattn_fused_launches = 0;
  g_af_conv_attn_short_launches = 0;
  g_af_gn_consumer_launches = 0;
  g_af_ff8_launches = 0;
  for (int i = 0; i < 15; ++i) g_af_plan_counts[i] = 0;
  return AF_OK;
}
int64_t af_fp8_gemm_launches(void) { return g_af_plan_counts[10]; }
int64_t af_ff8_launches(void) { return g_af_ff8_launches; }
int64_t af_halo8_launches(void) { return g_af_plan_counts[11]; }
int64_t af_rowpanel_launches(void) { return g_af_plan_counts[12]; }
int64_t af_up_phase4_launches(void) { return g_af_plan_counts[13]; }
int64_t af_gn_producer_launches(void) { return g_af_plan_counts[14]; }
int64_t af_attn_short_launches(void) { return g_af_attn_short_launches; }
int64_t af_xattn_fused_launches(void) { return g_af_xattn_fused_launches; }
int64_t af_conv_attn_short_launches(void) { return g_af_conv_attn_short_launches; }
int64_t af_gn_consumer_launches(void) { return g_af_gn_consumer_launches; }
int af_set_fp8(af_handle* h, int on) {
  if (!h) { af_set_error_msg("af_set_fp8: null handle"); return AF_ERR_INVALID; }
  if (on && h->dtype != AF_DTYPE_BF16) { af_set_error_msg("af_set_fp8: the fp8 convolutions extend the bf16 mode (handle is %s)", h->dtype == AF_DTYPE_F16 ? "f16" : "f32"); return AF_ERR_STATE; }
  h->fp8_on = on != 0;
  return AF_OK;
}
int af_set_fp8_scope(af_handle* h, int mask) {
  if (!h) { af_set_error_msg("af_set_fp8_scope: null handle"); return AF_ERR_INVALID; }
  if (h->dtype != AF_DTYPE_BF16) { af_set_error_msg("af_set_fp8_scope: the fp8 mode extends the bf16 mode (handle is %s)", h->dtype == AF_DTYPE_F16 ? "f16" : "f32"); return AF_ERR_STATE; }
  if (!(mask & AF_FP8_SCOPE_BASE) || (mask & ~(AF_FP8_SCOPE_BASE | AF_FP8_SCOPE_FF))) {
    af_set_error_msg("af_set_fp8_scope: mask %d (AF_FP8_SCOPE_BASE is always part of the scope, AF_FP8_SCOPE_FF may be added)", mask);
    return AF_ERR_INVALID;
  }
  if (mask != h->fp8_scope) h->fp8_dirty = true;
  h->fp8_scope = mask;
  return AF_OK;
}
int af_get_fp8_scope(af_handle* h) { return h ? h->fp8_scope : 0; }
int af_fp8_num_sites(af_handle* h) { return h ? h->fp8_nsites() : 0; }
const char* af_fp8_site_name(af_handle* h, int i) {
  if (!h || i < 0 || i >= h->fp8_nsites()) return nullptr;
  return h->fp8_site_names[i].c_str();
}
static int fp8_sites_arg(af_handle* h, int n, const char* who) {
  if (!h) { af_set_error_msg("%s: null handle", who); return AF_ERR_INVALID; }
  if (n != h->fp8_nsites()) { af_set_error_msg("%s: n = %d, the handle has %d fp8 sites in its scope", who, n, h->fp8_nsites()); return AF_ERR_INVALID; }
  return AF_OK;
}
int af_fp8_record(af_handle* h, int on, void* stream) {
  if (!h) { af_set_error_msg("af_fp8_record: null handle"); return AF_ERR_INVALID; }
  if (on && !h->fp8_rec) { af_set_error_msg("af_fp8_record: the handle has no fp8 sites (f32 or fp16 handle, or no UNet)"); return AF_ERR_STATE; }
// ... 83 lines not shown
```

### adaface_amd/csrc/af_xattn_fused.hip

```cpp
#include "af_kernels.h"

#include <type_traits>

namespace xf {
typedef bf16 T;
typedef __attribute__((ext_vector_type(4))) unsigned u32x4;
typedef __attribute__((ext_vector_type(2))) unsigned u32x2;

constexpr int C = 320, H = 8, DH = 40, KC = 5, NPAIR = 4;
constexpr int BNT = 80, NIW = 5, NTILE = 4;
constexpr int MJ = 2, WROWS = 32, BM = 256;
constexpr int D = 4, NS = 5;
constexpr int WBYTES = BNT * 128, WPIECES = BNT / 8;
constexpr int NKB = 5, SMAX = 16 * NKB;
constexpr int NSP = (NKB + 1) / 2;
constexpr int K_FRAGS = 2 * NKB * 2, V_FRAGS = 2 * 3 * NSP;
constexpr int KV_PPW = (K_FRAGS + V_FRAGS + 7) / 8;
constexpr int KVBUF = KV_PPW * 8 * 1024;
constexpr int BN3 = 160, NIW3 = 10, NTILE3 = 2, D3 = 2, NS3 = 3, WBYTES3 = BN3 * 128, WPIECES3 = BN3 / 8;
constexpr int OPITCH = BN3 * 2 + 16;
constexpr int OCH = BN3 / 8, OSLOTS = OCH + 1;
constexpr int NST = WROWS * OCH / 64;
constexpr int NRES = (WROWS * OSLOTS + 63) / 64;
constexpr int OBYTES = NRES * 1024;
// ... 84 lines not shown
}
template <int I, int N, typename F> __device__ __forceinline__ void static_for(F&& f) {
  if constexpr (I < N) {
    f(std::integral_constant<int, I>{});
    static_for<I + 1, N>(f);
  }
}
__device__ __forceinline__ f32x4 mma(const u32x4& a, const u32x4& b, const f32x4& c) {
  return __builtin_amdgcn_mfma_f32_16x16x32_bf16(__builtin_bit_cast(bf16x8, a), __builtin_bit_cast(bf16x8, b), c, 0, 0, 0);
}
__device__ __forceinline__ unsigned pack2(float a, float b) {
  typedef __attribute__((ext_vector_type(2))) __bf16 bf16x2;
  return __builtin_bit_cast(unsigned, __builtin_convertvector(f32x2{a, b}, bf16x2));
}
template <int NOPS> __device__ __forceinline__ float max3f(float a, float b, float c) {
  float r;
  if constexpr (NOPS > 0) asm volatile("s_nop %4\n\tv_max3_f32 %0, %1, %2, %3" : "=v"(r) : "v"(a), "v"(b), "v"(c), "n"(NOPS - 1));
  else asm volatile("v_max3_f32 %0, %1, %2, %3" : "=v"(r) : "v"(a), "v"(b), "v"(c));
  return r;
}
__device__ __forceinline__ f32x2 unpack2(unsigned w) {
  return f32x2{__builtin_bit_cast(float, w << 16), __builtin_bit_cast(float, w & 0xFFFF0000u)};
}
__device__ __forceinline__ float xgroup_max(float v) {
  v = fmaxf(v, __shfl_xor(v, 16, 64));
  return fmaxf(v, __shfl_xor(v, 32, 64));
}
__device__ __forceinline__ u32x2 pack4(const f32x4& v) { return u32x2{pack2(v[0], v[1]), pack2(v[2], v[3])}; }
__device__ __forceinline__ u32x4 cat(const u32x2& a, const u32x2& b) { return u32x4{a.x, a.y, b.x, b.y}; }

struct Params {
  const void* x; int ldx;
  int M;
  const float* ln_stats;
  int ln_parts_n; float ln_inv_count, ln_eps;
  const void* wq; int ldwq;
  const float* q_colsum; const float* q_bias;
  const void* kvpack; int rows_per_sample;
  const void* wo; int ldwo;
  const float* o_bias;
  void* out; int ldo;
  float* ln_stats_out;
  int Nk;
  float sl2;
  int lab;
};

__global__ __launch_bounds__(512) void xattn_fused_kernel(const Params p) {
  extern __shared__ __attribute__((aligned(1024))) char smem[];
  const int tid = threadIdx.x, lane = tid & 63, wid = __builtin_amdgcn_readfirstlane(tid >> 6);
#ifdef AF_LAB_ABLATE
  const int lab = p.lab;
#else
  constexpr int lab = 0;
#endif
  const int l15 = lane & 15, g = lane >> 4;
  const int m0 = blockIdx.x * BM, r0 = m0 + wid * WROWS;
  const int bsample = m0 / p.rows_per_sample;
  const __amdgpu_buffer_rsrc_t rs_x = __builtin_amdgcn_make_buffer_rsrc(const_cast<T*>(reinterpret_cast<const T*>(p.x)), 0, (int)0xFFFFFFF0u, 0x00020000);
  const __amdgpu_buffer_rsrc_t rs_wq = __builtin_amdgcn_make_buffer_rsrc(const_cast<T*>(reinterpret_cast<const T*>(p.wq)), 0, (int)0xFFFFFFF0u, 0x00020000);
  const __amdgpu_buffer_rsrc_t rs_wo = __builtin_amdgcn_make_buffer_rsrc(const_cast<T*>(reinterpret_cast<const T*>(p.wo)), 0, (int)0xFFFFFFF0u, 0x00020000);
  const __amdgpu_buffer_rsrc_t rs_kv = __builtin_amdgcn_make_buffer_rsrc(
      const_cast<T*>(reinterpret_cast<const T*>(p.kvpack) + (long)bsample * NPAIR * PACK_ELEMS_PER_PAIR), 0,
      (int)(NPAIR * PACK_ELEMS_PER_PAIR * 2), 0x00020000);
  const __amdgpu_buffer_rsrc_t rs_o = __builtin_amdgcn_make_buffer_rsrc(reinterpret_cast<T*>(p.out), 0, (int)0xFFFFFFF0u, 0x00020000);

  auto stage_kv = [&](int pair) {
    char* base = smem + KV0 + (pair & 1) * KVBUF;
#pragma unroll
    for (int q = 0; q < KV_PPW; ++q) {
      const int piece = wid + 8 * q;
      lds_dma16(rs_kv, base + piece * 1024, (unsigned)(lane * 16), (unsigned)(pair * (int)(PACK_ELEMS_PER_PAIR * 2) + piece * 1024));
    }
  };
  stage_kv(0);
  stage_kv(1);
  if (tid < 3 * (C / 4)) {
    const int v = tid / (C / 4), c4 = tid - v * (C / 4);
    const float* src = v == 0 ? p.q_colsum : (v == 1 ? p.q_bias : p.o_bias);
    const float4 val = src ? *reinterpret_cast<const float4*>(src + 4 * c4) : float4{0.f, 0.f, 0.f, 0.f};
    *reinterpret_cast<float4*>(smem + VEC0 + (v * C + 4 * c4) * 4) = val;
  }
  asm volatile("s_waitcnt lgkmcnt(0)" ::: "memory");

  u32x4 xr[MJ][KC][2];
  float ln_mu[MJ], ln_rs[MJ];
#pragma unroll
  for (int j = 0; j < MJ; ++j) {
    const int m = r0 + j * 16 + l15;
    const bool ok = m < p.M;
    const unsigned xo = ok ? (unsigned)((long)m * p.ldx * 2) + (unsigned)g * 16u : 0xFFFFFFFFu;
#pragma unroll
    for (int kc = 0; kc < KC; ++kc)
#pragma unroll
      for (int u = 0; u < 2; ++u)
        xr[j][kc][u] = (lab & 8) ? u32x4{0u, 0u, 0u, 0u} : __builtin_bit_cast(u32x4, __builtin_amdgcn_raw_buffer_load_b128(rs_x, xo, (kc * 64 + u * 32) * 2, 0));
    float2 st = float2{0.f, 0.f};
    if (ok && p.ln_parts_n > 0) {
      float s1 = 0.f, s2 = 0.f;
      for (int q = 0; q < p.ln_parts_n; ++q) {
        const float2 pq2 = *reinterpret_cast<const float2*>(p.ln_stats + ((long)q * p.M + m) * 2);
        s1 += pq2.x;
        s2 += pq2.y;
      }
      const float mu = s1 * p.ln_inv_count;
      const float var = fmaxf(s2 * p.ln_inv_count - mu * mu, 0.f);
      st = float2{mu, __builtin_amdgcn_rsqf(var + p.ln_eps)};
    } else if (ok) {
      st = *reinterpret_cast<const float2*>(p.ln_stats + (long)m * 2);
    }
    ln_mu[j] = st.x;
    ln_rs[j] = st.y;
  }

  const int srow = lane >> 3;
  const unsigned dchunk = (unsigned)((lane & 7) ^ srow);
  const int nwq = wid < WPIECES - 8 ? 2 : 1;
  unsigned wq_off[2];
#pragma unroll
  for (int q = 0; q < 2; ++q) wq_off[q] = (unsigned)(((wid + 8 * q) * 8 + srow) * p.ldwq * 2) + dchunk * 16u;
  const unsigned tstride_q = (unsigned)(BNT * p.ldwq * 2);
  constexpr int T1 = NTILE * KC;
  auto stage = [&](int t, int slot) {
    const bool live = t < T1;
    const int ntl = t / KC, kc = t - ntl * KC;
    const unsigned so = (unsigned)ntl * tstride_q + (unsigned)kc * 128u;
    lds_dma16(rs_wq, smem + RING0 + slot * WBYTES + wid * 1024, live ? wq_off[0] : 0xFFFFFFFFu, so);
    if (wid < WPIECES - 8) lds_dma16(rs_wq, smem + RING0 + slot * WBYTES + (wid + 8) * 1024, live ? wq_off[1] : 0xFFFFFFFFu, so);
  };
  unsigned wo_off[3];
#pragma unroll
  for (int q = 0; q < 3; ++q) wo_off[q] = (unsigned)(((wid + 8 * q) * 8 + srow) * p.ldwo * 2) + dchunk * 16u;
  const unsigned tstride_o = (unsigned)(BN3 * p.ldwo * 2);
  const int nw3 = wid < WPIECES3 - 16 ? 3 : 2;
  constexpr int T3 = NTILE3 * KC;
  auto stage3 = [&](int t, int slot) {
    const bool live = t < T3;
    const int ntl = t / KC, kc = t - ntl * KC;
    const unsigned so = (unsigned)ntl * tstride_o + (unsigned)kc * 128u;
    lds_dma16(rs_wo, smem + RING0 + slot * WBYTES3 + wid * 1024, live ? wo_off[0] : 0xFFFFFFFFu, so);
    lds_dma16(rs_wo, smem + RING0 + slot * WBYTES3 + (wid + 8) * 1024, live ? wo_off[1] : 0xFFFFFFFFu, so);
    if (wid < WPIECES3 - 16) lds_dma16(rs_wo, smem + RING0 + slot * WBYTES3 + (wid + 16) * 1024, live ? wo_off[2] : 0xFFFFFFFFu, so);
// ... 349 lines not shown
    if constexpr (nt + 1 < NTILE3) {
      asm volatile("s_waitcnt lgkmcnt(0)" ::: "memory");
      stage_res(nt + 1);
      init_acc3((nt + 1) * BN3);
    }
  });
  wait_vm<NST>();
}
}

long af_xattn_fused_pack_elems(int B, int H, int dh, int Nk) {
  if (H != xf::H || dh != xf::DH || Nk <= xf::SMAX - 16 || Nk > xf::SMAX || B <= 0) return 0;
  return (long)B * xf::NPAIR * xf::PACK_ELEMS_PER_PAIR;
}
int af_launch_xattn_fused_pack(const void* kv, int ldk, long bsk, int Nk, int B, void* pack, hipStream_t stream) {
  const long total = (long)B * xf::NPAIR * xf::PACK_ELEMS_PER_PAIR;
  unsigned blocks = (unsigned)((total + 255) / 256);
  if (blocks > 4096) blocks = 4096;
  hipLaunchKernelGGL(xf::pack_kv_kernel, dim3(blocks), dim3(256), 0, stream, reinterpret_cast<const bf16*>(kv), ldk, bsk, Nk, B,
                     reinterpret_cast<bf16*>(pack));
  HIP_CHECK_RET(hipGetLastError());
  return 0;
}
int af_launch_xattn_fused_permute_wo(const void* w, int ldw, int rows, void* wp, int ldp, hipStream_t stream) {
  hipLaunchKernelGGL(xf::permute_wo_kernel, dim3(400), dim3(256), 0, stream, reinterpret_cast<const bf16*>(w), ldw, rows,
                     reinterpret_cast<bf16*>(wp), ldp);
  HIP_CHECK_RET(hipGetLastError());
  return 0;
}
bool af_xattn_fused_ok(int M, int rows_per_sample, int C, int H, int dh, int Nk) {
  return C == xf::C && H == xf::H && dh == xf::DH && Nk > xf::SMAX - 16 && Nk <= xf::SMAX && rows_per_sample % xf::BM == 0 && M % xf::BM == 0 && M > 0;
}
std::atomic<long> g_af_xattn_fused_launches{0};
int af_launch_xattn_fused(const AfXattnFusedParams& a, hipStream_t stream) {
  if (!af_xattn_fused_ok(a.M, a.rows_per_sample, xf::C, xf::H, xf::DH, a.Nk) || a.ldx % 8 || a.ldo % 8 || a.ldwq % 8 || a.ldwo % 8) {
    af_set_error_msg("xattn_fused: unsupported shape M=%d rows/sample=%d Nk=%d", a.M, a.rows_per_sample, a.Nk);
    return -1;
  }
  static unsigned long long attr_done = 0;
  if (int rc = af_ensure_dynamic_lds(attr_done, reinterpret_cast<const void*>(&xf::xattn_fused_kernel), xf::LDS_BYTES)) return rc;
  xf::Params p;
  p.x = a.x; p.ldx = a.ldx; p.M = a.M;
  p.ln_stats = a.ln_stats; p.ln_parts_n = a.ln_parts_n; p.ln_inv_count = a.ln_inv_count; p.ln_eps = a.ln_eps;
  p.wq = a.wq; p.ldwq = a.ldwq; p.q_colsum = a.q_colsum; p.q_bias = a.q_bias;
  p.kvpack = a.kvpack; p.rows_per_sample = a.rows_per_sample;
  p.wo = a.wo; p.ldwo = a.ldwo; p.o_bias = a.o_bias;
  p.out = a.out; p.ldo = a.ldo; p.ln_stats_out = a.ln_stats_out; p.Nk = a.Nk;
  p.sl2 = 1.0f / sqrtf((float)xf::DH) * 1.44269504088896340736f;
  p.lab = g_af_knobs.xattn_fused >> 4;
  const double flops = 2.0 * 2.0 * a.M * (double)xf::C * xf::C + 4.0 * a.M * (double)a.Nk * xf::C;
  AfProfScope prof(AF_K_ATTENTION, stream, flops, 2.0 * a.M * (double)xf::C * 2);
  hipLaunchKernelGGL(xf::xattn_fused_kernel, dim3(a.M / xf::BM), dim3(512), xf::LDS_BYTES, stream, p);
  HIP_CHECK_RET(hipGetLastError());
  g_af_xattn_fused_launches += 1;
  return 0;
}
```

### adaface_amd/engine.py

```python
from __future__ import annotations

import contextlib
import ctypes as C
from typing import Dict, Iterable, Optional, Sequence

import torch

from . import _lib
from ._lib import AfConfig, DTYPES, check, ptr, stream_ptr

UNET_PREFIX = "model.diffusion_model."
VAE_PREFIX = "first_stage_model."


def _fill(arr, values: Sequence[int]):
    if len(values) > 8:
        raise ValueError("at most 8 entries supported")
    for i, v in enumerate(values):
        arr[i] = int(v)


class Engine:
    def __init__(self, *, dtype: str = "bf16", device: int = 0, unet: Optional[dict] = None, vae: Optional[dict] = None,
                 clip: Optional[dict] = None):
# ... 77 lines not shown

    def load_state_dict(self, sd: Dict[str, torch.Tensor], prefix: str = "", strict: bool = True):
        table = self.tensor_table()
        for name in table:
            key = name if not prefix else name
            if key in sd:
                self.load_tensor(name, sd[key])
        missing = self.missing_tensors()
        if strict and missing:
            raise KeyError(f"{len(missing)} tensors missing from state_dict, e.g. {missing[:5]}")
        return missing

    def set_context(self, ctx: torch.Tensor, Bf: int, layerwise: bool):
        if not ctx.is_cuda:
            raise ValueError("context must be a device tensor")
        ctx = ctx.contiguous().float()
        n_tokens = ctx.shape[1]
        L = self.unet_cfg.get("n_context_layers", 16) if layerwise else 1
        if ctx.shape[0] != Bf * L or ctx.shape[2] != self.unet_cfg["context_dim"]:
            raise ValueError(f"context shape {tuple(ctx.shape)} does not match batch {Bf} x layers {L}")
        check(self._lib.af_set_context(self._h, ptr(ctx), Bf, n_tokens, 1 if layerwise else 0, stream_ptr()),
              "af_set_context")

    def set_conv_attn(self, ks: int, batch_idx=(), token_idx=()):
        n = len(batch_idx)
        bi = (C.c_int * max(n, 1))(*[int(b) for b in batch_idx])
        flat = [int(t) for row in token_idx for t in row]
        ti = (C.c_int * max(len(flat), 1))(*flat)
        if n and len(flat) != ks * ks * n:
            raise ValueError(f"set_conv_attn: {ks * ks} token positions per subject sample for a {ks}x{ks} kernel")
        check(self._lib.af_set_conv_attn(self._h, int(ks), n, bi, ti), "af_set_conv_attn")
        self._ctx_key = None

    def unet_forward(self, x: torch.Tensor, t: torch.Tensor, out: Optional[torch.Tensor] = None) -> torch.Tensor:
        x = x.contiguous().float()
        t = t.contiguous().long()
        Bf, _, H, W = x.shape
        if out is None:
            out = torch.empty(Bf, self.unet_cfg["out_channels"], H, W, device=x.device, dtype=torch.float32)
        check(self._lib.af_unet_forward(self._h, ptr(x), ptr(t), ptr(out), Bf, H, W, stream_ptr()), "af_unet_forward")
        return out

    def unet_forward_twin(self, x: torch.Tensor, t: torch.Tensor, out: Optional[torch.Tensor] = None) -> torch.Tensor:
        x = x.contiguous().float()
        t = t.contiguous().long()
        B, _, H, W = x.shape
        if out is None:
            out = torch.empty(2 * B, self.unet_cfg["out_channels"], H, W, device=x.device, dtype=torch.float32)
        check(self._lib.af_unet_forward_twin(self._h, ptr(x), ptr(t), ptr(out), 2 * B, H, W, stream_ptr()),
              "af_unet_forward_twin")
        return out

    def unet_block_outputs(self, x: torch.Tensor, t: torch.Tensor, blocks=None) -> Dict[int, torch.Tensor]:
        x = x.contiguous().float()
        Bf, _, H, W = x.shape
        n = self._lib.af_unet_num_blocks(self._h)
        out = {}
        c, hh, ww = C.c_int(), C.c_int(), C.c_int()
        for b in (range(n) if blocks is None else blocks):
            check(self._lib.af_unet_block_shape(self._h, b, H, W, C.byref(c), C.byref(hh), C.byref(ww)), "af_unet_block_shape")
            buf = torch.empty(Bf, c.value, hh.value, ww.value, device=x.device, dtype=torch.float32)
            check(self._lib.af_unet_set_tap(self._h, b, ptr(buf)), "af_unet_set_tap")
            try:
                self.unet_forward(x, t)
            finally:
                self._lib.af_unet_set_tap(self._h, -1, None)
            out[b] = buf
        return out

    def vae_decode(self, z: torch.Tensor, scale_factor: float = 1.0, want_uint8: bool = False, want_float: bool = True):
        z = z.contiguous().float()
        B, _, H, W = z.shape
        f = 2 ** (len(self.vae_cfg["ch_mult"]) - 1)
        img = torch.empty(B, self.vae_cfg["out_ch"], H * f, W * f, device=z.device, dtype=torch.float32) if want_float else None
        u8 = torch.empty(B, H * f, W * f, 3, device=z.device, dtype=torch.uint8) if want_uint8 else None
        check(self._lib.af_vae_decode(self._h, ptr(z), float(scale_factor), ptr(img), ptr(u8), B, H, W, stream_ptr()),
              "af_vae_decode")
        if want_float and want_uint8:
            return img, u8
        return u8 if want_uint8 else img

    def vae_encode(self, x: torch.Tensor) -> torch.Tensor:
        x = x.contiguous().float()
        B, _, H, W = x.shape
# ... 113 lines not shown
```

### adaface_amd/ldm/models/diffusion/ddim.py

```python
from __future__ import annotations

import numpy as np
import torch

from adaface_amd import ops
from adaface_amd.ldm.modules.diffusionmodules.util import (extract_into_tensor, make_ddim_sampling_parameters,
                                                           make_ddim_timesteps, noise_like)


class DDIMSampler(object):
    def __init__(self, model, schedule="linear", **kwargs):
        super().__init__()
        self.model = model
        self.ddpm_num_timesteps = model.num_timesteps
        self.schedule = schedule
        self._twin_cache = None

    def register_buffer(self, name, attr):
        if isinstance(attr, torch.Tensor) and attr.device != self.model.device:
            attr = attr.to(self.model.device)
        setattr(self, name, attr)

    def make_schedule(self, ddim_num_steps, ddim_discretize="uniform", ddim_eta=0., verbose=True):
        self.ddim_timesteps = make_ddim_timesteps(ddim_discr_method=ddim_discretize, num_ddim_timesteps=ddim_num_steps,
                                                  num_ddpm_timesteps=self.ddpm_num_timesteps, verbose=verbose)
        alphas_cumprod = self.model.alphas_cumprod
        assert alphas_cumprod.shape[0] == self.ddpm_num_timesteps, 'alphas have to be defined for each timestep'
        to_torch = lambda x: x.clone().detach().to(torch.float32).to(self.model.device)
        acp_cpu = alphas_cumprod.detach().float().cpu()

        self.register_buffer('betas', to_torch(self.model.betas))
        self.register_buffer('alphas_cumprod', to_torch(alphas_cumprod))
        self.register_buffer('alphas_cumprod_prev', to_torch(self.model.alphas_cumprod_prev))
        self.register_buffer('sqrt_alphas_cumprod', to_torch(np.sqrt(acp_cpu)))
        self.register_buffer('sqrt_one_minus_alphas_cumprod', to_torch(np.sqrt(1. - acp_cpu)))
        self.register_buffer('log_one_minus_alphas_cumprod', to_torch(np.log(1. - acp_cpu)))
        self.register_buffer('sqrt_recip_alphas_cumprod', to_torch(np.sqrt(1. / acp_cpu)))
        self.register_buffer('sqrt_recipm1_alphas_cumprod', to_torch(np.sqrt(1. / acp_cpu - 1)))

        ddim_sigmas, ddim_alphas, ddim_alphas_prev = make_ddim_sampling_parameters(
# ... 21 lines not shown
                                  noise_dropout=noise_dropout, temperature=temperature,
                                  score_corrector=score_corrector, corrector_kwargs=corrector_kwargs, x_T=x_T,
                                  log_every_t=log_every_t, guidance_scale=guidance_scale,
                                  unconditional_conditioning=unconditional_conditioning, verbose=verbose, **kwargs)

    @torch.no_grad()
    def ddim_sampling(self, cond, shape, x_T=None, ddim_use_original_steps=False, callback=None, timesteps=None,
                      quantize_denoised=False, mask=None, x0=None, img_callback=None, log_every_t=100,
                      temperature=1., noise_dropout=0., score_corrector=None, corrector_kwargs=None,
                      guidance_scale=1., unconditional_conditioning=None, verbose=False, **kwargs):
        device = self.model.betas.device
        b = shape[0]
        img = torch.randn(shape, device=device) if x_T is None else x_T
        if timesteps is None:
            timesteps = self.ddpm_num_timesteps if ddim_use_original_steps else self.ddim_timesteps
        elif not ddim_use_original_steps:
            subset_end = int(min(timesteps / self.ddim_timesteps.shape[0], 1) * self.ddim_timesteps.shape[0]) - 1
            timesteps = self.ddim_timesteps[:subset_end]
        intermediates = {'x_inter': [img], 'pred_x0': [img]}
        time_range = reversed(range(0, timesteps)) if ddim_use_original_steps else np.flip(timesteps)
        total_steps = timesteps if ddim_use_original_steps else timesteps.shape[0]
        if verbose:
            print(f"Running DDIM Sampling with {total_steps} timesteps")

        if isinstance(guidance_scale, (list, tuple)):
            max_guide_scale, min_guide_scale = guidance_scale
        else:
            max_guide_scale = min_guide_scale = guidance_scale
        max_guide_anneal_steps = total_steps - 1
        delta = (max_guide_scale - min_guide_scale) / max_guide_anneal_steps if max_guide_anneal_steps > 0 else 0.
        guide_scale = max_guide_scale
        self._twin_cache = None

        for i, step in enumerate(time_range):
            index = total_steps - i - 1
            ts = torch.full((b,), int(step), device=device, dtype=torch.long)
            if mask is not None:
                assert x0 is not None
                img_orig = self.model.q_sample(x0, ts)
                img = img_orig * mask + (1. - mask) * img
            img, pred_x0 = self.p_sample_ddim(img, cond, ts, index=index, use_original_steps=ddim_use_original_steps,
                                              quantize_denoised=quantize_denoised, temperature=temperature,
                                              noise_dropout=noise_dropout, score_corrector=score_corrector,
                                              corrector_kwargs=corrector_kwargs, guidance_scale=guide_scale,
                                              unconditional_conditioning=unconditional_conditioning)
            if callback:
                callback(i)
            if img_callback:
                img_callback(pred_x0, i)
            if index % log_every_t == 0 or index == total_steps - 1:
                intermediates['x_inter'].append(img)
                intermediates['pred_x0'].append(pred_x0)
            guide_scale = guide_scale - delta if i <= max_guide_anneal_steps else 1
        self._twin_cache = None
        return img, intermediates

    def _twin_condition(self, c, uc):
        key = (id(c), id(uc))
        if self._twin_cache is not None and self._twin_cache[0] == key:
            return self._twin_cache[1]
        if isinstance(c, tuple):
            c_c, c_in_c, extra_info = c
            c_u, c_in_u, _ = uc
            twin = (torch.cat([c_c, c_u]), sum([list(c_in_c), list(c_in_u)], []), extra_info)
        else:
            twin = torch.cat([c, uc])
        self._twin_cache = (key, twin, c, uc)
        return twin

    @torch.no_grad()
    def p_sample_ddim(self, x, c, t, index, repeat_noise=False, use_original_steps=False, quantize_denoised=False,
                      temperature=1., noise_dropout=0., score_corrector=None, corrector_kwargs=None,
                      guidance_scale=1., unconditional_conditioning=None):
        b, device = x.shape[0], x.device
        if unconditional_conditioning is None or guidance_scale == 1.:
            e_c, e_u = self.model.apply_model(x, t, c), None
        else:
            twin = self._twin_condition(c, unconditional_conditioning)
            if hasattr(self.model, "apply_model_cfg_twin"):
                e = self.model.apply_model_cfg_twin(x, t, twin)
            else:
                e = self.model.apply_model(torch.cat([x] * 2), torch.cat([t] * 2), twin)
            e_c, e_u = e[:b], e[b:]

        alphas = self.model.alphas_cumprod if use_original_steps else self.ddim_alphas
        alphas_prev = self.model.alphas_cumprod_prev if use_original_steps else self.ddim_alphas_prev
        sqrt_one_minus_alphas = self.model.sqrt_one_minus_alphas_cumprod if use_original_steps else self.ddim_sqrt_one_minus_alphas
        sigmas = self.ddim_sigmas_for_original_num_steps if use_original_steps else self.ddim_sigmas
        f32 = lambda v: float(np.float32(float(v)))
        sigma_t = f32(sigmas[index])
        noise = noise_like(x.shape, device, repeat_noise)
        if noise_dropout > 0.:
            noise = torch.nn.functional.dropout(noise, p=noise_dropout)
        if sigma_t == 0.:
            noise = None
        if score_corrector is not None:
            assert self.model.parameterization == "eps"
            e_t = e_c if e_u is None else ops.lincomb([(e_c, guidance_scale), (e_u, 0.0)], cfg=True)
            e_c, e_u = score_corrector.modify_score(self.model, e_t, x, t, c, **(corrector_kwargs or {})), None
        x_prev, pred_x0 = ops.ddim_step(x, e_c, e_u, guidance_scale, f32(alphas[index]), f32(alphas_prev[index]),
                                        f32(sqrt_one_minus_alphas[index]), sigma_t, noise, temperature)
        if quantize_denoised:
            q, _, *_ = self.model.first_stage_model.quantize(pred_x0)
            sa = float(np.sqrt(np.float32(f32(alphas_prev[index]))))
            x_prev = ops.lincomb([(x_prev, 1.0), (pred_x0, -sa), (q, sa)])
            pred_x0 = q
        return x_prev, pred_x0

    @torch.no_grad()
    def stochastic_encode(self, x0, t, use_original_steps=False, noise=None):
        if use_original_steps:
            sqrt_alphas_cumprod = self.sqrt_alphas_cumprod
            sqrt_one_minus_alphas_cumprod = self.sqrt_one_minus_alphas_cumprod
        else:
            sqrt_alphas_cumprod = torch.sqrt(self.ddim_alphas).to(x0.device)
            sqrt_one_minus_alphas_cumprod = torch.as_tensor(self.ddim_sqrt_one_minus_alphas).to(x0.device)
        if noise is None:
            noise = torch.randn_like(x0)
        return (extract_into_tensor(sqrt_alphas_cumprod, t, x0.shape) * x0 +
                extract_into_tensor(sqrt_one_minus_alphas_cumprod, t, x0.shape) * noise)

    @torch.no_grad()
    def decode(self, x_latent, cond, t_start, guidance_scale=1.0, unconditional_conditioning=None,
               use_original_steps=False):
        timesteps = np.arange(self.ddpm_num_timesteps) if use_original_steps else self.ddim_timesteps
        timesteps = timesteps[:t_start]
        time_range = np.flip(timesteps)
        total_steps = timesteps.shape[0]
        max_g = guidance_scale
        min_g = min(2.0, max_g)
        delta = (max_g - min_g) / (total_steps - 1) if total_steps > 1 else 0.
        g = max_g
        x_dec = x_latent
        self._twin_cache = None
        for i, step in enumerate(time_range):
            index = total_steps - i - 1
            ts = torch.full((x_latent.shape[0],), int(step), device=x_latent.device, dtype=torch.long)
            x_dec, _ = self.p_sample_ddim(x_dec, cond, ts, index=index, use_original_steps=use_original_steps,
                                          guidance_scale=g, unconditional_conditioning=unconditional_conditioning)
            g = g - delta
        self._twin_cache = None
        return x_dec
```

### adaface_amd/ldm/models/diffusion/ddpm.py

```python
from __future__ import annotations

from contextlib import contextmanager
from functools import partial

import numpy as np
import torch
import torch.nn as nn

from adaface_amd.ldm.modules.diffusionmodules.util import extract_into_tensor, make_beta_schedule
from adaface_amd.ldm.util import instantiate_from_config


class DiffusionWrapper(nn.Module):

    def __init__(self, diff_model_config, conditioning_key):
        super().__init__()
        self.diffusion_model = instantiate_from_config(diff_model_config)
        self.conditioning_key = conditioning_key
        if conditioning_key not in (None, "crossattn"):
            raise NotImplementedError(f"conditioning_key '{conditioning_key}' is not used by SD-v1 txt2img")

    def forward(self, x, t, c_concat: list = None, c_crossattn: list = None, cfg_twin: bool = False):
        if self.conditioning_key is None:
            raise NotImplementedError("unconditional UNet is not on the path")
        c0 = c_crossattn[0]
        if isinstance(c0, tuple):
            c_static_emb, c_in, extra_info = c0
        else:
            c_static_emb, c_in, extra_info = c0, None, None
        if cfg_twin:
            return self.diffusion_model(x, t, context=c_static_emb, context_in=c_in, extra_info=extra_info, cfg_twin=True)
        return self.diffusion_model(x, t, context=c_static_emb, context_in=c_in, extra_info=extra_info)


class DDPM(nn.Module):

    def __init__(self, unet_config, timesteps=1000, beta_schedule="linear", linear_start=1e-4, linear_end=2e-2,
                 cosine_s=8e-3, given_betas=None, conditioning_key=None, parameterization="eps", use_ema=True,
                 first_stage_key="image", image_size=256, channels=3, log_every_t=100, v_posterior=0.,
                 use_layerwise_embedding=False, **ignored_training_kwargs):
        super().__init__()
        assert parameterization in ("eps", "x0")
        self.parameterization = parameterization
        self.first_stage_key = first_stage_key
        self.image_size = image_size
        self.channels = channels
        self.log_every_t = log_every_t
        self.use_layerwise_embedding = use_layerwise_embedding
        self.N_CA_LAYERS = 16 if use_layerwise_embedding else 1
        self.use_ema = False
        self.v_posterior = v_posterior
        self.model = DiffusionWrapper(unet_config, conditioning_key)
        self.register_schedule(given_betas=given_betas, beta_schedule=beta_schedule, timesteps=timesteps,
                               linear_start=linear_start, linear_end=linear_end, cosine_s=cosine_s)

    def register_schedule(self, given_betas=None, beta_schedule="linear", timesteps=1000, linear_start=1e-4,
                          linear_end=2e-2, cosine_s=8e-3):
        betas = given_betas if given_betas is not None else make_beta_schedule(
            beta_schedule, timesteps, linear_start=linear_start, linear_end=linear_end, cosine_s=cosine_s)
        alphas = 1. - betas
        alphas_cumprod = np.cumprod(alphas, axis=0)
        alphas_cumprod_prev = np.append(1., alphas_cumprod[:-1])
        self.num_timesteps = int(betas.shape[0])
        self.linear_start, self.linear_end = linear_start, linear_end
        to_torch = partial(torch.tensor, dtype=torch.float32)
# ... 72 lines not shown
                                      "(ddpm.py:1010-1053): not part of the inference path")
        if zs_clip_features is not None or zs_id_embs is not None:
            if not getattr(self.embedding_manager, "do_zero_shot", False):
                raise NotImplementedError("zero-shot identity conditioning needs an EmbeddingManager built with do_zero_shot=True "
                                          "(plus the Arc2Face encoder and SubjBasisGenerator weights, absent offline)")
            self.embedding_manager.set_zs_image_features(zs_clip_features, zs_id_embs, zs_out_id_embs_scale_range)
        if self.cond_stage_model is None:
            raise RuntimeError("this LatentDiffusion was built without a cond_stage_config: pass an embedding tensor")
        self.cond_stage_model.device = self.device
        if self.empty_context is not None:
            self.empty_context = self.empty_context.to(self.device)
        if randomize_clip_weights:
            self.cond_stage_model.sample_last_layers_skip_weights()
        self.embedding_manager.set_curr_iter_type(embman_iter_type or 'recon_iter')
        static_prompt_embedding = self.cond_stage_model.encode(cond_in, embedding_manager=self.embedding_manager)
        import copy
        extra_info = {'use_layerwise_context': self.use_layerwise_embedding,
                      'use_conv_attn_kernel_size': self.embedding_manager.use_conv_attn_kernel_size,
                      'placeholder2indices': copy.copy(self.embedding_manager.placeholder2indices),
                      'prompt_emb_mask': copy.copy(self.embedding_manager.prompt_emb_mask),
                      'is_training': self.embedding_manager.training,
                      'compel_cfg_weight_level_range': self.compel_cfg_weight_level_range,
                      'apply_compel_cfg_prob': self.apply_compel_cfg_prob,
                      'empty_context': self.empty_context,
                      'capture_distill_attn': False}
        prompts = list(cond_in) if not isinstance(cond_in, torch.Tensor) else [""] * cond_in.shape[0]
        return (static_prompt_embedding, prompts, extra_info)

    @staticmethod
    def layerwise_repeat(emb, n_layers=16):
        B, T, D = emb.shape
        return emb.unsqueeze(1).expand(B, n_layers, T, D).reshape(B * n_layers, T, D).contiguous()

    def apply_model(self, x_noisy, t, cond, return_ids=False):
        if not isinstance(cond, dict):
            if not isinstance(cond, list):
                cond = [cond]
            key = 'c_concat' if self.model.conditioning_key == 'concat' else 'c_crossattn'
            cond = {key: cond}
        x_recon = self.model(x_noisy, t, **cond)
        if isinstance(x_recon, tuple) and not return_ids:
            return x_recon[0]
        return x_recon

    def apply_model_cfg_twin(self, x_noisy, t, cond_twin):
        cond = cond_twin
        if not isinstance(cond, dict):
            if not isinstance(cond, list):
                cond = [cond]
            cond = {'c_crossattn': cond}
        if 'c_crossattn' not in cond:
            return self.apply_model(torch.cat([x_noisy] * 2), torch.cat([t] * 2), cond_twin)
        return self.model(x_noisy, t, cfg_twin=True, **cond)

    @torch.no_grad()
    def decode_first_stage(self, z, predict_cids=False, force_not_quantize=False):
        if predict_cids:
            raise NotImplementedError("VQ codebook ids are not used by the KL autoencoder")
        return self.first_stage_model.decode(z, scale_factor=self.scale_factor)

    @torch.no_grad()
    def decode_first_stage_uint8(self, z):
        return self.first_stage_model.decode(z, scale_factor=self.scale_factor, return_uint8=True)

    @torch.no_grad()
    def encode_first_stage(self, x, mask=None):
        return self.first_stage_model.encode(x, mask)

    @torch.no_grad()
    def get_first_stage_encoding(self, encoder_posterior):
        from adaface_amd.ldm.models.autoencoder import DiagonalGaussianDistribution
        if isinstance(encoder_posterior, DiagonalGaussianDistribution):
            return encoder_posterior.sample(scale=self.scale_factor)
        if isinstance(encoder_posterior, torch.Tensor):
            return self.scale_factor * encoder_posterior
        raise NotImplementedError(f"encoder_posterior of type '{type(encoder_posterior)}' not yet implemented")

    @torch.no_grad()
    def calibrate_fp8(self, conditioning, unconditional_conditioning=None, shape=None, batch_size=1, S=10,
                      guidance_scale=7.5, x_T=None, passes=2, headroom=1):
        from adaface_amd.ldm.models.diffusion.ddim import DDIMSampler
        unet = self.model.diffusion_model
        if shape is None:
            shape = [unet.in_channels, unet.image_size, unet.image_size]
        if x_T is None:
# ... 32 lines not shown
```

### adaface_amd/ldm/models/diffusion/plms.py

```python
from __future__ import annotations

import numpy as np
import torch

from adaface_amd import ops
from adaface_amd.ldm.modules.diffusionmodules.util import (make_ddim_sampling_parameters, make_ddim_timesteps,
                                                            noise_like)


class PLMSSampler(object):
    def __init__(self, model, schedule="linear", **kwargs):
        super().__init__()
        self.model = model
        self.ddpm_num_timesteps = model.num_timesteps
        self.schedule = schedule
        self._twin_cache = None

    def register_buffer(self, name, attr):
        if isinstance(attr, torch.Tensor) and attr.device != self.model.device:
            attr = attr.to(self.model.device)
        setattr(self, name, attr)

    def make_schedule(self, ddim_num_steps, ddim_discretize="uniform", ddim_eta=0., verbose=True):
        if ddim_eta != 0:
            raise ValueError('ddim_eta must be 0 for PLMS')
        self.ddim_timesteps = make_ddim_timesteps(ddim_discr_method=ddim_discretize, num_ddim_timesteps=ddim_num_steps,
                                                  num_ddpm_timesteps=self.ddpm_num_timesteps, verbose=verbose)
        acp = self.model.alphas_cumprod.detach().float().cpu()
        assert acp.shape[0] == self.ddpm_num_timesteps, 'alphas have to be defined for each timestep'
        to_dev = lambda x: x.clone().detach().to(torch.float32).to(self.model.device)
        self.register_buffer('betas', to_dev(self.model.betas))
        self.register_buffer('alphas_cumprod', to_dev(self.model.alphas_cumprod))
        self.register_buffer('alphas_cumprod_prev', to_dev(self.model.alphas_cumprod_prev))
        self.register_buffer('sqrt_one_minus_alphas_cumprod', to_dev(np.sqrt(1. - acp)))
        sig, a, a_prev = make_ddim_sampling_parameters(alphacums=acp, ddim_timesteps=self.ddim_timesteps, eta=ddim_eta,
                                                       verbose=verbose)
        self.ddim_sigmas, self.ddim_alphas, self.ddim_alphas_prev = sig, a, a_prev
        self.ddim_sqrt_one_minus_alphas = np.sqrt(1. - a)

    @torch.no_grad()
    def sample(self, S, batch_size, shape, conditioning=None, callback=None, normals_sequence=None, img_callback=None,
               quantize_x0=False, eta=0., mask=None, x0=None, temperature=1., noise_dropout=0., score_corrector=None,
               corrector_kwargs=None, verbose=True, x_T=None, log_every_t=100, unconditional_guidance_scale=1.,
               unconditional_conditioning=None, **kwargs):
        self.make_schedule(ddim_num_steps=S, ddim_eta=eta, verbose=verbose)
        C, H, W = shape
        return self.plms_sampling(conditioning, (batch_size, C, H, W), callback=callback, img_callback=img_callback,
                                  quantize_denoised=quantize_x0, mask=mask, x0=x0, ddim_use_original_steps=False,
                                  noise_dropout=noise_dropout, temperature=temperature, score_corrector=score_corrector,
                                  corrector_kwargs=corrector_kwargs, x_T=x_T, log_every_t=log_every_t,
                                  unconditional_guidance_scale=unconditional_guidance_scale,
                                  unconditional_conditioning=unconditional_conditioning)

    @torch.no_grad()
    def plms_sampling(self, cond, shape, x_T=None, ddim_use_original_steps=False, callback=None, timesteps=None,
                      quantize_denoised=False, mask=None, x0=None, img_callback=None, log_every_t=100, temperature=1.,
                      noise_dropout=0., score_corrector=None, corrector_kwargs=None, unconditional_guidance_scale=1.,
                      unconditional_conditioning=None):
        if ddim_use_original_steps:
            raise NotImplementedError("ddim_use_original_steps is not used by txt2img")
        device = self.model.betas.device
        b = shape[0]
        img = torch.randn(shape, device=device) if x_T is None else x_T
        if timesteps is None:
            timesteps = self.ddim_timesteps
        else:
            subset_end = int(min(timesteps / self.ddim_timesteps.shape[0], 1) * self.ddim_timesteps.shape[0]) - 1
            timesteps = self.ddim_timesteps[:subset_end]
        intermediates = {'x_inter': [img], 'pred_x0': [img]}
        time_range = np.flip(timesteps)
        total_steps = timesteps.shape[0]
        old_eps = []
        self._twin_cache = None
        for i, step in enumerate(time_range):
            index = total_steps - i - 1
            ts = torch.full((b,), int(step), device=device, dtype=torch.long)
            ts_next = torch.full((b,), int(time_range[min(i + 1, len(time_range) - 1)]), device=device, dtype=torch.long)
            if mask is not None:
                assert x0 is not None
                img = self.model.q_sample(x0, ts) * mask + (1. - mask) * img
            img, pred_x0, e_t = self.p_sample_plms(img, cond, ts, index=index, quantize_denoised=quantize_denoised,
                                                   temperature=temperature, noise_dropout=noise_dropout,
                                                   score_corrector=score_corrector, corrector_kwargs=corrector_kwargs,
                                                   unconditional_guidance_scale=unconditional_guidance_scale,
                                                   unconditional_conditioning=unconditional_conditioning,
                                                   old_eps=old_eps, t_next=ts_next)
            old_eps.append(e_t)
            if len(old_eps) >= 4:
                old_eps.pop(0)
            if callback:
                callback(i)
            if img_callback:
                img_callback(pred_x0, i)
            if index % log_every_t == 0 or index == total_steps - 1:
                intermediates['x_inter'].append(img)
                intermediates['pred_x0'].append(pred_x0)
        self._twin_cache = None
        return img, intermediates

    def _twin_condition(self, c, uc):
        key = (id(c), id(uc))
        if self._twin_cache is not None and self._twin_cache[0] == key:
            return self._twin_cache[1]
        if isinstance(c, tuple):
            c_c, c_in_c, info = c
            c_u, c_in_u, _ = uc
            twin = (torch.cat([c_u, c_c]), sum([list(c_in_u), list(c_in_c)], []), info)
        else:
            twin = torch.cat([uc, c])
        self._twin_cache = (key, twin, c, uc)
        return twin

    @torch.no_grad()
    def p_sample_plms(self, x, c, t, index, repeat_noise=False, use_original_steps=False, quantize_denoised=False,
                      temperature=1., noise_dropout=0., score_corrector=None, corrector_kwargs=None,
                      unconditional_guidance_scale=1., unconditional_conditioning=None, old_eps=None, t_next=None):
        if quantize_denoised or score_corrector is not None or use_original_steps:
            raise NotImplementedError("quantize_denoised / score_corrector / use_original_steps are not on the txt2img path")
        b = x.shape[0]
        f32 = lambda v: float(np.float32(float(v)))

        def get_model_output(xx, tt):
            if unconditional_conditioning is None or unconditional_guidance_scale == 1.:
                return self.model.apply_model(xx, tt, c)
            twin = self._twin_condition(c, unconditional_conditioning)
            if hasattr(self.model, "apply_model_cfg_twin"):
                e = self.model.apply_model_cfg_twin(xx, tt, twin)
            else:
                e = self.model.apply_model(torch.cat([xx] * 2), torch.cat([tt] * 2), twin)
            return ops.lincomb([(e[b:], unconditional_guidance_scale), (e[:b], 0.0)], cfg=True)

        def get_x_prev_and_pred_x0(e, idx):
            sigma_t = f32(self.ddim_sigmas[idx])
            noise = noise_like(x.shape, x.device, repeat_noise)
            if noise_dropout > 0.:
                noise = torch.nn.functional.dropout(noise, p=noise_dropout)
            return ops.ddim_step(x, e, None, 1.0, f32(self.ddim_alphas[idx]), f32(self.ddim_alphas_prev[idx]),
                                 f32(self.ddim_sqrt_one_minus_alphas[idx]), sigma_t,
                                 None if sigma_t == 0. else noise, temperature)

        e_t = get_model_output(x, t)
        if len(old_eps) == 0:
            x_prev, _ = get_x_prev_and_pred_x0(e_t, index)
            e_t_next = get_model_output(x_prev, t_next)
            e_t_prime = ops.lincomb([(e_t, 0.5), (e_t_next, 0.5)])
        elif len(old_eps) == 1:
            e_t_prime = ops.lincomb([(e_t, 3 / 2), (old_eps[-1], -1 / 2)])
        elif len(old_eps) == 2:
            e_t_prime = ops.lincomb([(e_t, 23 / 12), (old_eps[-1], -16 / 12), (old_eps[-2], 5 / 12)])
        else:
            e_t_prime = ops.lincomb([(e_t, 55 / 24), (old_eps[-1], -59 / 24), (old_eps[-2], 37 / 24), (old_eps[-3], -9 / 24)])
        x_prev, pred_x0 = get_x_prev_and_pred_x0(e_t_prime, index)
        return x_prev, pred_x0, e_t
```

### adaface_amd/ldm/modules/diffusionmodules/openaimodel.py

```python
from __future__ import annotations

from typing import Optional

import torch

from adaface_amd import layout
from adaface_amd.ldm._hipmodule import HipModule, build_param_tree


class UNetModel(HipModule):
    _ckpt_prefix = "model.diffusion_model."

    def __init__(self, image_size, in_channels, model_channels, out_channels, num_res_blocks, attention_resolutions,
                 dropout=0, channel_mult=(1, 2, 4, 8), conv_resample=True, dims=2, num_classes=None,
                 use_checkpoint=False, use_fp16=False, num_heads=-1, num_head_channels=-1, num_heads_upsample=-1,
                 use_scale_shift_norm=False, resblock_updown=False, use_new_attention_order=False,
                 use_spatial_transformer=False, transformer_depth=1, context_dim=None, n_embed=None, legacy=True):
        super().__init__()
        unsupported = {
            "dims != 2": dims != 2, "num_classes": num_classes is not None, "use_scale_shift_norm": use_scale_shift_norm,
            "resblock_updown": resblock_updown, "n_embed": n_embed is not None, "dropout": dropout != 0,
            "not conv_resample": not conv_resample, "not use_spatial_transformer": not use_spatial_transformer,
            "num_head_channels": num_head_channels != -1,
            "num_heads_upsample": num_heads_upsample not in (-1, num_heads),
# ... 66 lines not shown
            if half > 0:
                ctx[:half, l] = ops.lincomb([(ctx[:half, l].contiguous(), w), (e, 1.0 - w)])
        ctx = ctx.reshape(context.shape)
        if deterministic:
            object.__setattr__(self, "_compel_key", key)
            object.__setattr__(self, "_compel_ctx", ctx)
            object.__setattr__(self, "_compel_refs", (context, empty))
        return ctx, deterministic

    @staticmethod
    def _conv_attn_spec(ks, placeholder2indices):
        if ks is None or ks <= 1 or not placeholder2indices:
            return (0, (), ())
        if ks not in (2, 3, 4):
            raise NotImplementedError(f"conv attention kernel size {ks}: the reference pads for 2, 3 and 4 only (util.py:747-760)")
        batch, tokens = [], []
        for indices in placeholder2indices.values():
            if indices is None:
                continue
            idx_b = [int(v) for v in torch.as_tensor(indices[0]).tolist()]
            idx_n = [int(v) for v in torch.as_tensor(indices[1]).tolist()]
            if not idx_b:
                continue
            uniq = sorted(set(idx_b))
            M = len(idx_n) // len(uniq)
            if M < ks * ks:
                raise ValueError(f"{M} embeddings are not enough to cover a {ks}x{ks} kernel")
            for i, bi in enumerate(uniq):
                batch.append(bi)
                tokens.append(tuple(idx_n[i * M: i * M + ks * ks]))
        return (ks, tuple(batch), tuple(tokens))

    @torch.no_grad()
    def forward(self, x, timesteps=None, context=None, y=None, context_in=None, extra_info=None, cfg_twin=False, **kwargs):
        if y is not None:
            raise NotImplementedError("class-conditional UNet (num_classes) is not on the path")
        if timesteps is None or context is None:
            raise ValueError("UNetModel.forward needs timesteps and context")
        info = extra_info if extra_info is not None else {}
        layerwise = bool(info.get("use_layerwise_context", False))
        ks = info.get("use_conv_attn_kernel_size", None)
        conv = self._conv_attn_spec(ks, info.get("placeholder2indices", None))
        if info.get("img_mask", None) is not None or info.get("capture_distill_attn", False):
            raise NotImplementedError("img_mask / capture_distill_attn are training-time options")
        if info.get("iter_type", "normal_recon") == "mix_hijk":
            raise NotImplementedError("iter_type 'mix_hijk' (separate k/v contexts) is a training-time option")
        eng = self.engine(x.device)
        B = x.shape[0] * (2 if cfg_twin else 1)
        cache_ok = True
        if layerwise and info.get("apply_compel_cfg_prob", 0) > 0:
            context, cache_ok = self._compel_cfg(context.to(x.device), B, info)
        key = (id(context), getattr(context, "_version", 0), tuple(context.shape), layerwise, B, conv)
        if key != self._ctx_key or not cache_ok:
            eng.set_conv_attn(*conv)
            eng.set_context(context.to(x.device), B, layerwise)
            object.__setattr__(self, "_ctx_key", key if cache_ok else None)
            object.__setattr__(self, "_ctx_ref", context)
        out = (eng.unet_forward_twin if cfg_twin else eng.unet_forward)(x, timesteps.to(x.device))
        if extra_info is not None:
            extra_info["ca_layers_activations"] = {k: {} for k in ("outfeat", "attn", "attnscore", "q")}
        return out.type(x.dtype) if x.dtype != torch.float32 else out
```

### adaface_amd/ldm/modules/diffusionmodules/util.py

```python
from __future__ import annotations

import numpy as np
import torch


def make_beta_schedule(schedule, n_timestep, linear_start=1e-4, linear_end=2e-2, cosine_s=8e-3):
    if schedule == "linear":
        betas = torch.linspace(linear_start ** 0.5, linear_end ** 0.5, n_timestep, dtype=torch.float64) ** 2
    elif schedule == "sqrt_linear":
        betas = torch.linspace(linear_start, linear_end, n_timestep, dtype=torch.float64)
    elif schedule == "sqrt":
        betas = torch.linspace(linear_start, linear_end, n_timestep, dtype=torch.float64) ** 0.5
    elif schedule == "cosine":
        steps = torch.arange(n_timestep + 1, dtype=torch.float64) / n_timestep + cosine_s
        alphas = torch.cos(steps / (1 + cosine_s) * np.pi / 2).pow(2)
        alphas = alphas / alphas[0]
        betas = (1 - alphas[1:] / alphas[:-1]).clamp(min=0, max=0.999)
    else:
        raise ValueError(f"schedule '{schedule}' unknown.")
    return betas.numpy()


def make_ddim_timesteps(ddim_discr_method, num_ddim_timesteps, num_ddpm_timesteps, verbose=True):
    if ddim_discr_method == "uniform":
# ... 6 lines not shown
    steps_out = ddim_timesteps + 1
    if verbose:
        print(f"Selected timesteps for ddim sampler: {steps_out}")
    return steps_out


def make_ddim_sampling_parameters(alphacums, ddim_timesteps, eta, verbose=True):
    alphas = alphacums[ddim_timesteps]
    alphas_prev = np.asarray([alphacums[0]] + alphacums[ddim_timesteps[:-1]].tolist())
    sigmas = eta * np.sqrt((1 - alphas_prev) / (1 - alphas) * (1 - alphas / alphas_prev))
    if verbose:
        print(f"Selected alphas for ddim sampler: a_t: {alphas}; a_(t-1): {alphas_prev}")
        print(f"For the chosen value of eta, which is {eta}, this results in sigma_t schedule {sigmas}")
    return sigmas, alphas, alphas_prev


def noise_like(shape, device, repeat=False):
    if repeat:
        return torch.randn((1, *shape[1:]), device=device).repeat(shape[0], *((1,) * (len(shape) - 1)))
    return torch.randn(shape, device=device)


def extract_into_tensor(a, t, x_shape):
    b = t.shape[0]
    out = a.gather(-1, t)
    return out.reshape(b, *((1,) * (len(x_shape) - 1)))


def timestep_embedding(timesteps, dim, max_period=10000, repeat_only=False, dtype="f32"):
    from adaface_amd import ops
    if max_period != 10000 or repeat_only:
        raise NotImplementedError("only max_period=10000, repeat_only=False is on the hot path")
    return ops.timestep_embedding(timesteps, dim, dtype=dtype)
```

### include/adaface_hip.h

```cpp
#ifndef ADAFACE_HIP_H
#define ADAFACE_HIP_H
#include <stdint.h>
#ifdef __cplusplus
extern "C" {
#endif

typedef struct af_handle af_handle;

enum { AF_DTYPE_BF16 = 0, AF_DTYPE_F32 = 1, AF_DTYPE_F16 = 2 };
enum {
  AF_OK = 0,
  AF_ERR_INVALID = -1,
  AF_ERR_HIP = -2,
  AF_ERR_NAME = -3,
  AF_ERR_STATE = -4
};

typedef struct af_config {
  int dtype;
  int build_unet;
  int in_channels, model_channels, out_channels, num_res_blocks;
  int n_attention_resolutions, attention_resolutions[8];
  int n_channel_mult, channel_mult[8];
  int num_heads, context_dim, transformer_depth;
  int n_context_layers;
  int build_vae;
  int vae_ch, vae_out_ch, vae_num_res_blocks, vae_z_channels, vae_embed_dim;
  int n_vae_ch_mult, vae_ch_mult[8];
  int build_vae_encoder;
  int vae_in_channels;
  int build_clip;
  int clip_vocab, clip_hidden, clip_layers, clip_heads, clip_intermediate, clip_max_pos;
} af_config;

const char* af_last_error(void);
int af_version(void);

int af_create(int device_id, const af_config* cfg, af_handle** out);
void af_destroy(af_handle* h);

int af_load_tensor(af_handle* h, const char* name, const float* host_data, int ndim, const int64_t* shape);
int af_load_tensor_device(af_handle* h, const char* name, const float* dev_data, int ndim, const int64_t* shape);
int af_num_tensors(af_handle* h);
const char* af_tensor_name(af_handle* h, int i);
int af_tensor_loaded(af_handle* h, int i);
int af_tensor_shape(af_handle* h, int i, int64_t* shape4 );

int af_set_conv_attn(af_handle* h, int ks, int n_subj, const int* batch_idx, const int* token_idx);
int af_set_context(af_handle* h, const float* ctx_dev, int Bf, int n_tokens, int layerwise, void* stream);

int af_unet_forward(af_handle* h, const float* x_dev, const int64_t* t_dev, float* eps_dev, int Bf, int H, int W,
                    void* stream);
int af_unet_forward_twin(af_handle* h, const float* x_dev, const int64_t* t_dev, float* eps_dev, int Bf, int H, int W,
                         void* stream);

int af_clip_embed_tokens(af_handle* h, const int64_t* ids_dev, int64_t n, float* emb_dev, void* stream);
int af_clip_text_forward(af_handle* h, const float* inputs_embeds_dev, int Bn, int T, float w_prev, float w_last,
                         float* out_dev, void* stream);
int af_clip_text_forward3(af_handle* h, const float* inputs_embeds_dev, int Bn, int T, float w_prev2, float w_prev, float w_last,
                          float* out_dev, void* stream);

int af_unet_num_blocks(af_handle* h);
int af_unet_block_shape(af_handle* h, int block, int H, int W, int* C_out, int* H_out, int* W_out);
int af_unet_set_tap(af_handle* h, int block, float* out_dev);

int af_ddim_step(const float* x_dev, const float* eps_cond_dev, const float* eps_uncond_dev, const float* noise_dev,
                 int64_t n, float guidance, float a_t, float a_prev, float sqrt_one_minus_at, float sigma_t,
                 float temperature, float* x_prev_dev, float* pred_x0_dev, void* stream);

int af_lincomb(float* out_dev, int64_t n, const float* x0_dev, float w0, const float* x1_dev, float w1,
               const float* x2_dev, float w2, const float* x3_dev, float w3, int mode, void* stream);

int af_vae_decode(af_handle* h, const float* z_dev, float scale_factor, float* img_dev, uint8_t* u8_dev, int B, int H,
                  int W, void* stream);

int af_vae_encode(af_handle* h, const float* x_dev, float* moments_dev, int B, int H, int W, void* stream);
int af_posterior_sample(const float* moments_dev, const float* noise_dev, float scale, float* z_dev, int B, int C,
                        int HW, void* stream);
int af_to_uint8(const float* img_dev, uint8_t* u8_dev, int B, int H, int W, void* stream);

int64_t af_arena_bytes(af_handle* h);

int af_prof_enable(int class_mask);
int af_prof_reset(void);
int af_prof_set_stride(int every);
double af_flops_issued(int reset);
int af_clock_probe(void* stream, int iters, double* mfma_mhz, double* mfma_tflops);
// ... 13 lines not shown
int af_op_linear(int dtype, const float* x_dev, const float* w_dev, const float* bias_dev, const float* residual_dev,
                 float* y_dev, int64_t M, int K, int N, int geglu, void* stream);
int af_op_conv_gn(const float* x_dev, const float* w_dev, const float* bias_dev, const float* residual_dev,
                  const float* gamma_dev, const float* beta_dev, float eps, int silu, float* h_dev, float* y_dev, int B,
                  int Cin, int H, int W, int Cout, void* stream);
int af_op_groupnorm(int dtype, const float* x_dev, const float* gamma_dev, const float* beta_dev, float eps, int silu,
                    float* y_dev, int B, int C, int H, int W, void* stream);
int af_set_fp8(af_handle* h, int on);
#define AF_FP8_SHIFT_MIN (-16)
#define AF_FP8_SHIFT_MAX 8
#define AF_FP8_SHIFT_DEFAULT 3
int af_fp8_num_sites(af_handle* h);
const char* af_fp8_site_name(af_handle* h, int i);
int af_fp8_record(af_handle* h, int on, void* stream);
int af_fp8_read_record(af_handle* h, int n, float* amax, int64_t* nsat, void* stream);
int af_fp8_get_shifts(af_handle* h, int n, int* shifts);
int af_fp8_set_shifts(af_handle* h, int n, const int* shifts);
int af_fp8_shift_for_amax(float amax, int headroom);
#define AF_FP8_SCOPE_BASE 1
#define AF_FP8_SCOPE_FF 2
int af_set_fp8_scope(af_handle* h, int mask);
int af_get_fp8_scope(af_handle* h);
int64_t af_ff8_launches(void);
int af_op_ff_fp8(const float* x_dev, const unsigned char* x8_dev, const float* gamma_dev, const float* beta_dev, float eps,
                 const float* w1_dev, const float* b1_dev, const float* w2_dev, const float* b2_dev, const float* residual_dev,
                 int64_t M, int C, int F, int Cout, int shift1, int shift2, void* rec_out_dev, float* y_dev,
                 unsigned char* mid8_dev, int* plan_out, void* stream);
int64_t af_fp8_gemm_launches(void);
int64_t af_halo8_launches(void);
int64_t af_gn_producer_launches(void);
int64_t af_attn_short_launches(void);
int64_t af_xattn_fused_launches(void);
int64_t af_conv_attn_short_launches(void);
int af_op_conv_attention(int dtype, const float* q_dev, const float* k_dev, const float* v_dev, float* o_dev, int B, int Hh,
                         int Ww, int Nk, int heads, int dh, float scale, int ks, int n_groups, int path, void* stream);
int af_op_xattn_fused(const float* x_dev, const float* ln_stats_dev, const float* gamma_dev, const float* beta_dev,
                      const float* wq_dev, const float* kv_dev, const float* wo_dev, const float* bo_dev, float* y_dev,
                      float* ln_parts_out_dev, int B, int N, int S, void* stream);
int64_t af_gn_consumer_launches(void);
int64_t af_up_phase4_launches(void);
int64_t af_rowpanel_launches(void);
int af_op_conv2d_fp8(const float* x_dev, const float* w_dev, const float* bias_dev, const float* residual_dev, float* y_dev,
                     int B, int Cin, int H, int W, int Cout, int ks, int stride, int pad, int upsample, int act_shift,
                     void* stream);
int af_op_groupnorm_fp8(const float* x_dev, const float* gamma_dev, const float* beta_dev, float eps, int silu,
                        unsigned char* y8_dev, int B, int C, int H, int W, int act_shift, void* stream);
int af_op_layernorm_fp8(const float* x_dev, const float* gamma_dev, const float* beta_dev, float eps, unsigned char* y8_dev,
                        int64_t rows, int C, int act_shift, void* stream);
int af_op_groupnorm_fp8_rec(const float* x_dev, const float* gamma_dev, const float* beta_dev, float eps, int silu,
                            unsigned char* y8_dev, int B, int C, int H, int W, int act_shift, void* rec_out_dev, void* stream);
int af_op_layernorm_fp8_rec(const float* x_dev, const float* gamma_dev, const float* beta_dev, float eps, unsigned char* y8_dev,
                            int64_t rows, int C, int act_shift, void* rec_out_dev, void* stream);
int af_op_gn_conv1x1(const float* x_dev, const float* gamma_dev, const float* beta_dev, float eps, const float* w_dev,
                     const float* bias_dev, float* y_plain_dev, float* y_fused_dev, int B, int C, int H, int W, int N,
                     void* stream);
int af_op_layernorm(int dtype, const float* x_dev, const float* gamma_dev, const float* beta_dev, float eps,
                    float* y_dev, int64_t rows, int C, void* stream);
int af_op_attention(int dtype, const float* q_dev, const float* k_dev, const float* v_dev, float* o_dev, int B, int Nq,
                    int Nk, int heads, int dh, float scale, int causal, void* stream);
int af_op_timestep_embedding(int dtype, const int64_t* t_dev, float* y_dev, int B, int dim, void* stream);

#ifdef __cplusplus
}
#endif
#endif
```

Measured before the change: 10.57.

## Cache timestep embeddings per step and read twin residuals via wrapped addressing

Adds a per-handle device cache of the projected timestep embedding, keyed by a uniform timestep value the sampler now passes down, so later calls with the same timestep skip the sinusoidal embedding, the time-MLP GEMMs and SiLU. It also stops duplicating the shared prefix half of x and t1 in the CFG-twin transformer path. Instead the proj_out row-panel GEMM and the fused cross-attention kernel read the residual and input through wrapped row offsets. The cache is keyed by timestep alone, invalidated on weight or knob changes and skipped during graph capture. This adds host-side bookkeeping and restricts the wrap to specific kernel configurations.

Result: no change. 10.64 (median of 6 runs) (+0.6%).

```diff
diff --git a/adaface_amd/_lib.py b/adaface_amd/_lib.py
--- a/adaface_amd/_lib.py
+++ b/adaface_amd/_lib.py
@@ -55,6 +55,9 @@
     ("af_set_context", C.c_int, [_P, _P, C.c_int, C.c_int, C.c_int, _P]),
     ("af_unet_forward", C.c_int, [_P, _P, _P, _P, C.c_int, C.c_int, C.c_int, _P]),
     ("af_unet_forward_twin", C.c_int, [_P, _P, _P, _P, C.c_int, C.c_int, C.c_int, _P]),
+    ("af_unet_forward_t", C.c_int, [_P, _P, _P, C.c_int64, _P, C.c_int, C.c_int, C.c_int, _P]),
+    ("af_unet_forward_twin_t", C.c_int, [_P, _P, _P, C.c_int64, _P, C.c_int, C.c_int, C.c_int, _P]),
+    ("af_temb_cache_stats", C.c_int, [_P, C.POINTER(C.c_int64), C.POINTER(C.c_int64), C.POINTER(C.c_int64)]),
     ("af_ddim_step", C.c_int, [_P, _P, _P, _P, C.c_int64, C.c_float, C.c_float, C.c_float, C.c_float, C.c_float,
                                C.c_float, _P, _P, _P]),
     ("af_lincomb", C.c_int, [_P, C.c_int64, _P, C.c_float, _P, C.c_float, _P, C.c_float, _P, C.c_float, C.c_int, _P]),
@@ -104,6 +107,7 @@
     ("af_gn_consumer_launches", C.c_int64, []),
     ("af_xattn_fused_launches", C.c_int64, []),
     ("af_conv_attn_short_launches", C.c_int64, []),
+    ("af_twin_wrap_launches", C.c_int64, []),
     ("af_op_conv_attention", C.c_int, [C.c_int, _P, _P, _P, _P] + [C.c_int] * 6 + [C.c_float] + [C.c_int] * 3 + [_P]),
     ("af_op_xattn_fused", C.c_int, [C.c_void_p] * 10 + [C.c_int] * 3 + [C.c_void_p]),
     ("af_op_conv2d_fp8", C.c_int, [_P, _P, _P, _P, _P] + [C.c_int] * 10 + [_P]),
@@ -169,6 +173,7 @@
     out["gn_consumer"] = int(lib.af_gn_consumer_launches())
     out["xattn_fused"] = int(lib.af_xattn_fused_launches())
     out["conv_attn_short"] = int(lib.af_conv_attn_short_launches())
+    out["twin_wrap"] = int(lib.af_twin_wrap_launches())
     if reset:
         lib.af_gemm_plan_counts_reset()
     return out
diff --git a/adaface_amd/csrc/af_common.h b/adaface_amd/csrc/af_common.h
--- a/adaface_amd/csrc/af_common.h
+++ b/adaface_amd/csrc/af_common.h
@@ -88,6 +88,8 @@
   int ff8_min_k;
   int ff8_min_rows;
   int conv_attn_short;
+  int twin_wrap;
+  int temb_cache_cap;
 };
 extern AfKnobs g_af_knobs;
 
@@ -263,6 +265,7 @@
   int ldrb;
   const void* residual;
   int ldr;
+  int res_wrap;
   void* out;
   int ldo;
   int epilogue;
diff --git a/adaface_amd/csrc/af_conv_gemm.hip b/adaface_amd/csrc/af_conv_gemm.hip
--- a/adaface_amd/csrc/af_conv_gemm.hip
+++ b/adaface_amd/csrc/af_conv_gemm.hip
@@ -1072,6 +1072,8 @@
   const __amdgpu_buffer_rsrc_t rs_w = __builtin_amdgcn_make_buffer_rsrc(
       const_cast<T*>(reinterpret_cast<const T*>(p.W)), 0, (int)0xFFFFFFF0u, 0x00020000);
   const __amdgpu_buffer_rsrc_t rs_o = __builtin_amdgcn_make_buffer_rsrc(reinterpret_cast<T*>(p.out), 0, (int)0xFFFFFFF0u, 0x00020000);
+  constexpr bool RES_WRAP = RES && LNMODE == 0 && KC_ == 5 && MJ_ == 2;
+  const T* __restrict__ res_base = reinterpret_cast<const T*>(p.residual) - ((RES_WRAP && p.res_wrap > 0 && m0 >= p.res_wrap) ? (long)p.res_wrap * p.ldr : 0L);
 
   float* vecs = reinterpret_cast<float*>(smem + C::LDS_BYTES);
   const int nvcol = ntn * C::BN;
@@ -1335,7 +1337,7 @@
           const bool mok = m < p.M;
           Quad<T> rq[RES ? NH : 1];
           if constexpr (RES) {
-            const T* rp = reinterpret_cast<const T*>(p.residual) + (long)(mok ? m : 0) * p.ldr + ncol + hh * NH * 16 + cl;
+            const T* rp = res_base + (long)(mok ? m : 0) * p.ldr + ncol + hh * NH * 16 + cl;
 #pragma unroll
             for (int ii = 0; ii < NH; ++ii) rq[ii].load(rp + ii * 16);
           }
@@ -2464,6 +2466,11 @@
   return 0;
 }
 
+bool af_conv_res_wrap_ok(const ConvGemmParams& p, int batch) {
+  return p.residual && !p.ln_stats && !p.ln_stats_out && p.res_wrap > 0 && p.res_wrap % RowPanelCfg::BM == 0 && p.M == 2 * p.res_wrap &&
+         af_conv_rowpanel_kind(p, batch) == 2;
+}
+
 template <typename T>
 int af_launch_conv_gemm(const ConvGemmParams& p_in, int batch, hipStream_t stream, const AfGemmPlan* plan, void* ws) {
   constexpr int BK = 128 / sizeof(T);
@@ -2472,6 +2479,7 @@
     if constexpr (std::is_same_v<T, bf16>) return batch == 1 ? launch_conv_gemm_fp8(p, stream, plan, ws) : (af_set_error_msg("conv_gemm fp8: no batched form"), -1);
     else { af_set_error_msg("conv_gemm: fp8 operands need the bf16 storage mode"); return -1; }
   }
+  if (p.res_wrap > 0 && !std::is_same_v<T, bf16>) { af_set_error_msg("conv_gemm: a wrapped residual exists on the bf16 row-panel kernel only"); return -1; }
   if (p.gn_ab && !std::is_same_v<T, bf16>) { af_set_error_msg("conv_gemm: consumer-side GroupNorm exists on the bf16 row-panel kernels only"); return -1; }
   if (p.K % BK != 0 || p.Cin % BK != 0 || p.K != p.ks * p.ks * p.Cin) {
     af_set_error_msg("conv_gemm: K=%d Cin=%d ks=%d must satisfy K==ks*ks*Cin and Cin%%%d==0", p.K, p.Cin, p.ks, BK);
@@ -2551,6 +2559,11 @@
       af_set_error_msg("conv_gemm: consumer-side GroupNorm asked of a launch that is not a row-panel one (ask af_conv_rowpanel_kind first)");
       return -1;
     }
+    if (p.res_wrap > 0 && !af_conv_res_wrap_ok(p, batch)) {
+      af_set_error_msg("conv_gemm: wrapped residual asked of a launch that cannot read it (ask af_conv_res_wrap_ok first)");
+      return -1;
+    }
+    if (p.res_wrap > 0) g_af_twin_wrap_launches += 1;
     if (p.gn_ab) g_af_gn_consumer_launches += 1;
     if (rk) g_af_plan_counts[12] += 1;
     switch (rk) {
diff --git a/adaface_amd/csrc/af_kernels.h b/adaface_amd/csrc/af_kernels.h
--- a/adaface_amd/csrc/af_kernels.h
+++ b/adaface_amd/csrc/af_kernels.h
@@ -2,6 +2,7 @@
 #include "af_common.h"
 
 AfGemmPlan af_plan_conv_gemm(const ConvGemmParams& p, int batch, AfStorage st);
+bool af_conv_res_wrap_ok(const ConvGemmParams& p, int batch);
 template <typename T>
 int af_launch_conv_gemm(const ConvGemmParams& p, int batch, hipStream_t stream, const AfGemmPlan* plan = nullptr,
                         void* ws = nullptr);
@@ -23,6 +24,7 @@
   void* out; int ldo;
   float* ln_stats_out;
   int Nk;
+  int x_wrap;
 };
 bool af_xattn_fused_ok(int M, int rows_per_sample, int C, int H, int dh, int Nk);
 long af_xattn_fused_pack_elems(int B, int H, int dh, int Nk);
@@ -30,6 +32,7 @@
 int af_launch_xattn_fused_permute_wo(const void* w, int ldw, int rows, void* wp, int ldp, hipStream_t stream);
 int af_launch_xattn_fused(const AfXattnFusedParams& a, hipStream_t stream);
 extern std::atomic<long> g_af_xattn_fused_launches;
+extern std::atomic<long> g_af_twin_wrap_launches;
 
 bool af_ff_geglu_fp8_ok(const ConvGemmParams& p);
 int af_launch_ff_geglu_fp8(ConvGemmParams p, float out_mul, unsigned* rec, hipStream_t stream);
diff --git a/adaface_amd/csrc/af_model.hip b/adaface_amd/csrc/af_model.hip
--- a/adaface_amd/csrc/af_model.hip
+++ b/adaface_amd/csrc/af_model.hip
@@ -32,8 +32,9 @@
     knob_env("AF_GN_PRODUCER", 1),     knob_env("AF_CONV_UP_PHASE4", 1), knob_env("AF_ATTN_SHORT", 1),
     knob_env("AF_GEMM_M128", 1),       knob_env("AF_SMALL_M_TILE64", 1),  knob_env("AF_GN_CONSUMER", 1),
     knob_env("AF_XATTN_FUSED", 1),     knob_env("AF_PLAN_LOG", 0),      knob_env("AF_FF8_MIN_K", 512),   knob_env("AF_FF8_MIN_ROWS", 0),
-    knob_env("AF_CONV_ATTN_SHORT", 1)};
+    knob_env("AF_CONV_ATTN_SHORT", 1), knob_env("AF_TWIN_WRAP", 1), knob_env("AF_TEMB_CACHE_CAP", 0)};
 static const AfKnobs g_af_knobs_initial = g_af_knobs;
+static long g_af_knob_gen = 0;
 static int* knob_slot(const char* name) {
   static const struct { const char* n; int AfKnobs::*m; } tab[] = {
       {"splitk_target", &AfKnobs::splitk_target}, {"conv_halo", &AfKnobs::conv_halo}, {"gemm_pp", &AfKnobs::gemm_pp},
@@ -44,7 +45,7 @@
       {"geglu_rowpanel", &AfKnobs::geglu_rowpanel}, {"conv_halo8", &AfKnobs::conv_halo8}, {"ablate", &AfKnobs::ablate}, {"gn_producer", &AfKnobs::gn_producer}, {"conv_up_phase4", &AfKnobs::conv_up_phase4},
       {"attn_short", &AfKnobs::attn_short},
       {"gemm_m128", &AfKnobs::gemm_m128}, {"small_m_tile64", &AfKnobs::small_m_tile64}, {"gn_consumer", &AfKnobs::gn_consumer}, {"xattn_fused", &AfKnobs::xattn_fused}, {"plan_log", &AfKnobs::plan_log}, {"ff8_min_k", &AfKnobs::ff8_min_k}, {"ff8_min_rows", &AfKnobs::ff8_min_rows},
-      {"conv_attn_short", &AfKnobs::conv_attn_short}};
+      {"conv_attn_short", &AfKnobs::conv_attn_short}, {"twin_wrap", &AfKnobs::twin_wrap}, {"temb_cache_cap", &AfKnobs::temb_cache_cap}};
   if (!name) return nullptr;
   for (auto& t : tab)
     if (strcmp(t.n, name) == 0) return &(g_af_knobs.*(t.m));
@@ -262,6 +263,12 @@
   float* gn_carry = nullptr;
   size_t gn_carry_bytes = 0, gn_carry_need = 0;
 
+  std::map<int64_t, void*> temb_rows;
+  std::vector<void*> temb_pool;
+  bool temb_dirty = false;
+  long temb_knob_gen = 0;
+  int64_t temb_hits = 0, temb_misses = 0;
+
   int tap_index = -1;
   float* tap_out = nullptr;
 
@@ -817,6 +824,14 @@
     p.splitk = pl.splitk;
     return af_conv_rowpanel_kind(p, 1) != 0;
   }
+  bool res_wrap_capable(const Linear& L, const Act& x, const Act& out, const Act& residual, int res_wrap) const {
+    if (dt != AF_DTYPE_BF16 || x.f8) return false;
+    ConvGemmParams p;
+    conv_params(p, L, x, out, 1, 0, &residual, nullptr, 0, -1, -1);
+    p.res_wrap = res_wrap;
+    p.splitk = af_plan_conv_gemm(p, 1, storage_of(dt)).splitk;
+    return af_conv_res_wrap_ok(p, 1);
+  }
   int groupnorm_fold(const Norm& N, const Act& x, float* ab) {
     const int HW = x.H * x.W;
     void* ws = A.alloc(af_gn_workspace_bytes(x.B, HW));
@@ -829,11 +844,12 @@
                     af_launch_groupnorm_fold<f16>(x.p, (long)HW * x.ld, x.ld, x.B, HW, x.C, N.gamma, N.beta, N.eps, ws, s, pre, x.gn_npart, ab));
   }
   int conv(const Linear& L, const Act& x, Act& out, int stride, int up, const Act* residual, const void* rowbias,
-           int ldrb, int n_valid = -1, int pad = -1, const LnArgs* ln = nullptr, int want_gn = 0) {
+           int ldrb, int n_valid = -1, int pad = -1, const LnArgs* ln = nullptr, int want_gn = 0, int res_wrap = 0) {
     AF_TRY(check(out));
     out.gn_part = nullptr; out.gn_npart = 0;
     ConvGemmParams p;
     conv_params(p, L, x, out, stride, up, residual, rowbias, ldrb, n_valid, pad);
+    p.res_wrap = res_wrap;
     bool ln_parts_pending = false;
     if (ln) {
       p.ln_stats = ln->stats; p.ln_colsum = ln->colsum;
@@ -992,6 +1008,9 @@
   };
   Act g = R.alloc_act(B, H, W, x.C);
   Act t = R.alloc_act(B, H, W, C);
+  Act xfull = x;
+  xfull.B = B;
+  const bool wrap_x = twin && g_af_knobs.twin_wrap && R.res_wrap_capable(w.proj_out, t, out, xfull, Bh * N);
   Act f_probe = t;
   f_probe.C = 4 * C; f_probe.ld = 4 * C;
   Act qkv_probe = t;
@@ -1082,11 +1101,7 @@
       Act t1p = pv(t1);
       AF_TRY(R.conv(blk.out1, ap, t1p, 1, 0, &tp, nullptr, 0, -1, -1, ln_parts ? &pa : nullptr));
     }
-    if (pre) {
-      AF_TRY(R.check(t1));
-      AF_TRY(dup(t1));
-      AF_TRY(dup(x));
-    }
+    if (pre) AF_TRY(R.check(t1));
     const CtxKV& kv = h->ctx_kv[w.ca_slot + d];
     const int S = h->ctx_tokens;
     if (!R.dry && (!kv.kv || h->ctx_Bf != B)) {
@@ -1099,16 +1114,20 @@
     Act q = R.alloc_act(B, H, W, C);
     const bool fused_ca = g_af_knobs.xattn_fused && R.dt == AF_DTYPE_BF16 && ln_parts == 4 && !conv_attn && blk.out2_perm && blk.q2_ln.w &&
                           t1.ld == C && t2.ld == C && af_xattn_fused_ok(B * N, N, C, w.heads, w.dh, S > 0 ? S : 77);
+    const bool wrap_t1 = pre && fused_ca && g_af_knobs.twin_wrap != 0;
+    if (pre && !wrap_t1) AF_TRY(dup(t1));
+    if (pre && !wrap_x) AF_TRY(dup(x));
     if (fused_ca) {
       AF_TRY(R.check(t2));
       if (pre) AF_TRY(finalize(st_1, blk.ln2, (long)Bh * N));
-      if (pre && !R.dry)
+      if (pre && !wrap_t1 && !R.dry)
         HIP_CHECK_RET(hipMemcpyAsync(st_row + (size_t)Bh * N * 2, st_row, (size_t)Bh * N * 2 * sizeof(float), hipMemcpyDeviceToDevice, R.s));
       if (!R.dry) {
         if (!kv.xf_pack) { af_set_error_msg("fused cross-attention: no K / V pack for this layer (af_set_context)"); return AF_ERR_STATE; }
         AfXattnFusedParams a;
         memset(&a, 0, sizeof(a));
         a.x = t1.p; a.ldx = t1.ld; a.M = B * N; a.rows_per_sample = N;
+        a.x_wrap = wrap_t1 ? Bh * N : 0;
         if (pre) { a.ln_stats = st_row; a.ln_parts_n = 0; }
         else { a.ln_stats = st_1; a.ln_parts_n = ln_parts; a.ln_inv_count = 1.0f / (float)C; a.ln_eps = blk.ln2.eps; }
         a.wq = blk.q2_ln.w; a.ldwq = blk.q2_ln.ldw; a.q_colsum = blk.q2_cs; a.q_bias = blk.q2_ln.bias;
@@ -1228,11 +1247,7 @@
     }
     R.A.release(mk2);
   }
-  {
-    Act xf = x;
-    xf.B = B;
-    AF_TRY(R.conv(w.proj_out, t, out, 1, 0, &xf, nullptr, 0));
-  }
+  AF_TRY(R.conv(w.proj_out, t, out, 1, 0, &xfull, nullptr, 0, -1, -1, nullptr, 0, wrap_x ? Bh * N : 0));
   R.A.release(mk);
   return 0;
 }
@@ -1371,7 +1386,7 @@
 }
 
 static int unet_forward_impl(af_handle* h, hipStream_t s, const float* x_dev, const int64_t* t_dev, float* eps_dev,
-                             int Bf, int H, int W, bool twin = false) {
+                             int Bf, int H, int W, bool twin = false, const void* temb_row = nullptr, void* temb_store = nullptr) {
   Runner R(h, s);
   const af_config& c = h->cfg;
   const int dt = h->dtype;
@@ -1395,16 +1410,17 @@
   Act e2 = R.alloc_act(Bf, 1, 1, ted);
   Act emb_all = R.alloc_act(Bf, 1, 1, h->emb_total);
   AF_TRY(R.check(emb_all));
+  const bool temb_hit = !R.dry && temb_row;
   if (!R.dry) {
     AF_TRY(DISPATCH(dt, af_launch_nchw_to_nhwc<bf16>(x_dev, x.p, Bin, c.in_channels, H * W, x.ld, 1.0f, s),
                     af_launch_nchw_to_nhwc<float>(x_dev, x.p, Bin, c.in_channels, H * W, x.ld, 1.0f, s),
                     af_launch_nchw_to_nhwc<f16>(x_dev, x.p, Bin, c.in_channels, H * W, x.ld, 1.0f, s)));
-    AF_TRY(DISPATCH(dt, af_launch_timestep_embedding<bf16>((const long long*)t_dev, temb.p, Bin, mc, s),
+    if (!temb_hit) AF_TRY(DISPATCH(dt, af_launch_timestep_embedding<bf16>((const long long*)t_dev, temb.p, Bin, mc, s),
                     af_launch_timestep_embedding<float>((const long long*)t_dev, temb.p, Bin, mc, s),
                     af_launch_timestep_embedding<f16>((const long long*)t_dev, temb.p, Bin, mc, s)));
   }
   if (twin && !twin_prefix) AF_TRY(dup_half(x));
-  {
+  if (!temb_hit) {
     Act tb = temb, e1b = e1, e2b = e2, eab = emb_all;
     tb.B = e1b.B = e2b.B = eab.B = Bin;
     AF_TRY(R.conv(h->time_embed0, tb, e1b, 1, 0, nullptr, nullptr, 0));
@@ -1413,7 +1429,11 @@
     if (!R.dry) AF_TRY(DISPATCH(dt, af_launch_silu<bf16>(e2.p, e2.p, (long)Bin * ted, s), af_launch_silu<float>(e2.p, e2.p, (long)Bin * ted, s), af_launch_silu<f16>(e2.p, e2.p, (long)Bin * ted, s)));
     AF_TRY(R.conv(h->emb_all, e2b, eab, 1, 0, nullptr, nullptr, 0));
     if (twin) AF_TRY(dup_half(emb_all));
-  }
+    if (!R.dry && temb_store)
+      HIP_CHECK_RET(hipMemcpyAsync(temb_store, emb_all.p, (size_t)h->emb_total * esize(dt), hipMemcpyDeviceToDevice, s));
+  }
+  const void* emb_p = temb_hit ? temb_row : emb_all.p;
+  const int emb_ld = temb_hit ? 0 : emb_all.ld;
 
   auto run_block = [&](const UBlock& ub, Act hcur, Act& result, const Act* final_out, int nb, bool twin_x) -> int {
     hcur.B = nb;
@@ -1442,7 +1462,7 @@
         case L_RES: {
           const ResBlockW& w = h->res[l.idx];
           out = new_act(hcur.H, hcur.W, w.cout);
-          AF_TRY(run_resblock(R, w, hcur, out, emb_all.p, emb_all.ld));
+          AF_TRY(run_resblock(R, w, hcur, out, emb_p, emb_ld));
         } break;
         case L_XFMR: {
           out = new_act(hcur.H, hcur.W, hcur.C);
@@ -1828,6 +1848,7 @@
   if (h->ctx_cast) hipFree(h->ctx_cast);
   if (h->arena.base) hipFree(h->arena.base);
   if (h->stage) hipFree(h->stage);
+  for (void* p : h->temb_pool) hipFree(p);
   delete h;
 }
 
@@ -1904,6 +1925,7 @@
   h->ln_fold_dirty = true;
   h->fp8_dirty = true;
   h->up4_dirty = true;
+  h->temb_dirty = true;
   return 0;
 }
 
@@ -2050,8 +2072,30 @@
   return 0;
 }
 
+static void temb_lookup(af_handle* h, hipStream_t s, int64_t t, int Bin, const void** row, void** store) {
+  *row = nullptr; *store = nullptr;
+  hipStreamCaptureStatus cap = hipStreamCaptureStatusNone;
+  if (Bin > 64 || hipStreamIsCapturing(s, &cap) != hipSuccess || cap != hipStreamCaptureStatusNone) { (void)hipGetLastError(); return; }
+  if (h->temb_dirty || h->temb_knob_gen != g_af_knob_gen) {
+    h->temb_rows.clear();
+    h->temb_dirty = false;
+    h->temb_knob_gen = g_af_knob_gen;
+  }
+  auto it = h->temb_rows.find(t);
+  if (it != h->temb_rows.end()) { *row = it->second; return; }
+  const size_t cap_n = g_af_knobs.temb_cache_cap > 0 ? (size_t)g_af_knobs.temb_cache_cap : 1000;
+  const size_t used = h->temb_rows.size();
+  if (used >= cap_n) return;
+  if (used >= h->temb_pool.size()) {
+    void* p = nullptr;
+    if (hipMalloc(&p, (size_t)h->emb_total * esize(h->dtype)) != hipSuccess) { (void)hipGetLastError(); return; }
+    h->temb_pool.push_back(p);
+  }
+  *store = h->temb_pool[used];
+}
+
 static int unet_forward_entry(af_handle* h, const float* x_dev, const int64_t* t_dev, float* eps_dev, int Bf, int H, int W,
-                              void* stream, bool twin) {
+                              void* stream, bool twin, const int64_t* t_uniform = nullptr) {
   if (!h || !x_dev || !t_dev || !eps_dev) { af_set_error_msg("af_unet_forward: null argument"); return AF_ERR_INVALID; }
   if (twin && (Bf < 2 || Bf % 2)) { af_set_error_msg("af_unet_forward_twin: the batch [x; x] must be even, got %d", Bf); return AF_ERR_INVALID; }
   if (!h->cfg.build_unet) { af_set_error_msg("af_unet_forward: handle has no UNet"); return AF_ERR_STATE; }
@@ -2069,7 +2113,31 @@
   if (rc) return rc;
   if (h->arena.peak > h->arena.cap) { HIP_CHECK_RET(hipStreamSynchronize(s)); AF_TRY(ensure_arena(h, h->arena.peak)); }
   AF_TRY(ensure_gn_carry(h, s));
-  return unet_forward_impl(h, s, x_dev, t_dev, eps_dev, Bf, H, W, twin);
+  if (!t_uniform) return unet_forward_impl(h, s, x_dev, t_dev, eps_dev, Bf, H, W, twin);
+  const void* row = nullptr;
+  void* store = nullptr;
+  temb_lookup(h, s, *t_uniform, twin ? Bf / 2 : Bf, &row, &store);
+  rc = unet_forward_impl(h, s, x_dev, t_dev, eps_dev, Bf, H, W, twin, row, store);
+  if (rc) return rc;
+  if (row) ++h->temb_hits; else ++h->temb_misses;
+  if (store) h->temb_rows[*t_uniform] = store;
+  return 0;
+}
+int af_unet_forward_t(af_handle* h, const float* x_dev, const int64_t* t_dev, int64_t t_value, float* eps_dev, int Bf, int H,
+                      int W, void* stream) {
+  return unet_forward_entry(h, x_dev, t_dev, eps_dev, Bf, H, W, stream, false, &t_value);
+}
+int af_unet_forward_twin_t(af_handle* h, const float* x_dev, const int64_t* t_dev, int64_t t_value, float* eps_dev, int Bf,
+                           int H, int W, void* stream) {
+  return unet_forward_entry(h, x_dev, t_dev, eps_dev, Bf, H, W, stream, true, &t_value);
+}
+int af_temb_cache_stats(af_handle* h, int64_t* hits, int64_t* misses, int64_t* entries) {
+  if (!h) { af_set_error_msg("af_temb_cache_stats: null handle"); return AF_ERR_INVALID; }
+  const bool stale = h->temb_dirty || h->temb_knob_gen != g_af_knob_gen;
+  if (hits) *hits = h->temb_hits;
+  if (misses) *misses = h->temb_misses;
+  if (entries) *entries = stale ? 0 : (int64_t)h->temb_rows.size();
+  return AF_OK;
 }
 int af_unet_forward(af_handle* h, const float* x_dev, const int64_t* t_dev, float* eps_dev, int Bf, int H, int W,
                     void* stream) {
@@ -2232,6 +2300,7 @@
   int* k = knob_slot(name);
   if (!k) { af_set_error_msg("af_knob_set: unknown knob '%s'", name ? name : "(null)"); return AF_ERR_NAME; }
   *k = value;
+  ++g_af_knob_gen;
   return AF_OK;
 }
 int af_knob_get(const char* name, int* value) {
@@ -2242,6 +2311,7 @@
 }
 int af_knob_reset(void) {
   g_af_knobs = g_af_knobs_initial;
+  ++g_af_knob_gen;
   return AF_OK;
 }
 
@@ -2279,6 +2349,7 @@
 int af_gemm_plan_counts_reset(void) {
   g_af_attn_short_launches = 0;
   g_af_xattn_fused_launches = 0;
+  g_af_twin_wrap_launches = 0;
   g_af_conv_attn_short_launches = 0;
   g_af_gn_consumer_launches = 0;
   g_af_ff8_launches = 0;
@@ -2293,6 +2364,7 @@
 int64_t af_gn_producer_launches(void) { return g_af_plan_counts[14]; }
 int64_t af_attn_short_launches(void) { return g_af_attn_short_launches; }
 int64_t af_xattn_fused_launches(void) { return g_af_xattn_fused_launches; }
+int64_t af_twin_wrap_launches(void) { return g_af_twin_wrap_launches; }
 int64_t af_conv_attn_short_launches(void) { return g_af_conv_attn_short_launches; }
 int64_t af_gn_consumer_launches(void) { return g_af_gn_consumer_launches; }
 int af_set_fp8(af_handle* h, int on) {
diff --git a/adaface_amd/csrc/af_xattn_fused.hip b/adaface_amd/csrc/af_xattn_fused.hip
--- a/adaface_amd/csrc/af_xattn_fused.hip
+++ b/adaface_amd/csrc/af_xattn_fused.hip
@@ -140,6 +140,7 @@
 struct Params {
   const void* x; int ldx;
   int M;
+  int x_wrap;
   const float* ln_stats;
   int ln_parts_n; float ln_inv_count, ln_eps;
   const void* wq; int ldwq;
@@ -165,7 +166,9 @@
   const int l15 = lane & 15, g = lane >> 4;
   const int m0 = blockIdx.x * BM, r0 = m0 + wid * WROWS;
   const int bsample = m0 / p.rows_per_sample;
-  const __amdgpu_buffer_rsrc_t rs_x = __builtin_amdgcn_make_buffer_rsrc(const_cast<T*>(reinterpret_cast<const T*>(p.x)), 0, (int)0xFFFFFFF0u, 0x00020000);
+  const long xback = (p.x_wrap > 0 && m0 >= p.x_wrap) ? (long)p.x_wrap : 0;
+  const float* __restrict__ ln_fin = p.ln_stats - xback * 2;
+  const __amdgpu_buffer_rsrc_t rs_x = __builtin_amdgcn_make_buffer_rsrc(const_cast<T*>(reinterpret_cast<const T*>(p.x) - xback * p.ldx), 0, (int)0xFFFFFFF0u, 0x00020000);
   const __amdgpu_buffer_rsrc_t rs_wq = __builtin_amdgcn_make_buffer_rsrc(const_cast<T*>(reinterpret_cast<const T*>(p.wq)), 0, (int)0xFFFFFFF0u, 0x00020000);
   const __amdgpu_buffer_rsrc_t rs_wo = __builtin_amdgcn_make_buffer_rsrc(const_cast<T*>(reinterpret_cast<const T*>(p.wo)), 0, (int)0xFFFFFFF0u, 0x00020000);
   const __amdgpu_buffer_rsrc_t rs_kv = __builtin_amdgcn_make_buffer_rsrc(
@@ -215,7 +218,7 @@
       const float var = fmaxf(s2 * p.ln_inv_count - mu * mu, 0.f);
       st = float2{mu, __builtin_amdgcn_rsqf(var + p.ln_eps)};
     } else if (ok) {
-      st = *reinterpret_cast<const float2*>(p.ln_stats + (long)m * 2);
+      st = *reinterpret_cast<const float2*>(ln_fin + (long)m * 2);
     }
     ln_mu[j] = st.x;
     ln_rs[j] = st.y;
@@ -631,15 +634,20 @@
   return C == xf::C && H == xf::H && dh == xf::DH && Nk > xf::SMAX - 16 && Nk <= xf::SMAX && rows_per_sample % xf::BM == 0 && M % xf::BM == 0 && M > 0;
 }
 std::atomic<long> g_af_xattn_fused_launches{0};
+std::atomic<long> g_af_twin_wrap_launches{0};
 int af_launch_xattn_fused(const AfXattnFusedParams& a, hipStream_t stream) {
   if (!af_xattn_fused_ok(a.M, a.rows_per_sample, xf::C, xf::H, xf::DH, a.Nk) || a.ldx % 8 || a.ldo % 8 || a.ldwq % 8 || a.ldwo % 8) {
     af_set_error_msg("xattn_fused: unsupported shape M=%d rows/sample=%d Nk=%d", a.M, a.rows_per_sample, a.Nk);
     return -1;
   }
+  if (a.x_wrap != 0 && (a.x_wrap < 0 || a.M != 2 * a.x_wrap || a.x_wrap % xf::BM || a.ln_parts_n > 0)) {
+    af_set_error_msg("xattn_fused: x_wrap = %d (half of M = %d in whole 256-row panels, finalised statistics)", a.x_wrap, a.M);
+    return -1;
+  }
   static unsigned long long attr_done = 0;
   if (int rc = af_ensure_dynamic_lds(attr_done, reinterpret_cast<const void*>(&xf::xattn_fused_kernel), xf::LDS_BYTES)) return rc;
   xf::Params p;
-  p.x = a.x; p.ldx = a.ldx; p.M = a.M;
+  p.x = a.x; p.ldx = a.ldx; p.M = a.M; p.x_wrap = a.x_wrap;
   p.ln_stats = a.ln_stats; p.ln_parts_n = a.ln_parts_n; p.ln_inv_count = a.ln_inv_count; p.ln_eps = a.ln_eps;
   p.wq = a.wq; p.ldwq = a.ldwq; p.q_colsum = a.q_colsum; p.q_bias = a.q_bias;
   p.kvpack = a.kvpack; p.rows_per_sample = a.rows_per_sample;
@@ -652,5 +660,6 @@
   hipLaunchKernelGGL(xf::xattn_fused_kernel, dim3(a.M / xf::BM), dim3(512), xf::LDS_BYTES, stream, p);
   HIP_CHECK_RET(hipGetLastError());
   g_af_xattn_fused_launches += 1;
+  if (a.x_wrap > 0) g_af_twin_wrap_launches += 1;
   return 0;
 }
diff --git a/adaface_amd/engine.py b/adaface_amd/engine.py
--- a/adaface_amd/engine.py
+++ b/adaface_amd/engine.py
@@ -133,24 +133,39 @@
         check(self._lib.af_set_conv_attn(self._h, int(ks), n, bi, ti), "af_set_conv_attn")
         self._ctx_key = None
 
-    def unet_forward(self, x: torch.Tensor, t: torch.Tensor, out: Optional[torch.Tensor] = None) -> torch.Tensor:
+    def unet_forward(self, x: torch.Tensor, t: torch.Tensor, out: Optional[torch.Tensor] = None,
+                     t_uniform: Optional[int] = None) -> torch.Tensor:
         x = x.contiguous().float()
         t = t.contiguous().long()
         Bf, _, H, W = x.shape
         if out is None:
             out = torch.empty(Bf, self.unet_cfg["out_channels"], H, W, device=x.device, dtype=torch.float32)
-        check(self._lib.af_unet_forward(self._h, ptr(x), ptr(t), ptr(out), Bf, H, W, stream_ptr()), "af_unet_forward")
-        return out
-
-    def unet_forward_twin(self, x: torch.Tensor, t: torch.Tensor, out: Optional[torch.Tensor] = None) -> torch.Tensor:
+        if t_uniform is None:
+            check(self._lib.af_unet_forward(self._h, ptr(x), ptr(t), ptr(out), Bf, H, W, stream_ptr()), "af_unet_forward")
+        else:
+            check(self._lib.af_unet_forward_t(self._h, ptr(x), ptr(t), int(t_uniform), ptr(out), Bf, H, W, stream_ptr()),
+                  "af_unet_forward_t")
+        return out
+
+    def unet_forward_twin(self, x: torch.Tensor, t: torch.Tensor, out: Optional[torch.Tensor] = None,
+                          t_uniform: Optional[int] = None) -> torch.Tensor:
         x = x.contiguous().float()
         t = t.contiguous().long()
         B, _, H, W = x.shape
         if out is None:
             out = torch.empty(2 * B, self.unet_cfg["out_channels"], H, W, device=x.device, dtype=torch.float32)
-        check(self._lib.af_unet_forward_twin(self._h, ptr(x), ptr(t), ptr(out), 2 * B, H, W, stream_ptr()),
-              "af_unet_forward_twin")
-        return out
+        if t_uniform is None:
+            check(self._lib.af_unet_forward_twin(self._h, ptr(x), ptr(t), ptr(out), 2 * B, H, W, stream_ptr()),
+                  "af_unet_forward_twin")
+        else:
+            check(self._lib.af_unet_forward_twin_t(self._h, ptr(x), ptr(t), int(t_uniform), ptr(out), 2 * B, H, W, stream_ptr()),
+                  "af_unet_forward_twin_t")
+        return out
+
+    def temb_cache_stats(self) -> Dict[str, int]:
+        v = [C.c_int64() for _ in range(3)]
+        check(self._lib.af_temb_cache_stats(self._h, *[C.byref(a) for a in v]), "af_temb_cache_stats")
+        return {"hits": v[0].value, "misses": v[1].value, "entries": v[2].value}
 
     def unet_block_outputs(self, x: torch.Tensor, t: torch.Tensor, blocks=None) -> Dict[int, torch.Tensor]:
         x = x.contiguous().float()
diff --git a/adaface_amd/ldm/models/diffusion/ddim.py b/adaface_amd/ldm/models/diffusion/ddim.py
--- a/adaface_amd/ldm/models/diffusion/ddim.py
+++ b/adaface_amd/ldm/models/diffusion/ddim.py
@@ -5,7 +5,7 @@
 
 from adaface_amd import ops
 from adaface_amd.ldm.modules.diffusionmodules.util import (extract_into_tensor, make_ddim_sampling_parameters,
-                                                           make_ddim_timesteps, noise_like)
+                                                           make_ddim_timesteps, noise_like, step_tensors, uniform_kw)
 
 
 class DDIMSampler(object):
@@ -93,9 +93,11 @@
         guide_scale = max_guide_scale
         self._twin_cache = None
 
+        time_range = [int(s) for s in time_range]
+        ts_all = step_tensors(time_range, b, device)
         for i, step in enumerate(time_range):
             index = total_steps - i - 1
-            ts = torch.full((b,), int(step), device=device, dtype=torch.long)
+            ts = ts_all[i]
             if mask is not None:
                 assert x0 is not None
                 img_orig = self.model.q_sample(x0, ts)
@@ -104,7 +106,7 @@
                                               quantize_denoised=quantize_denoised, temperature=temperature,
                                               noise_dropout=noise_dropout, score_corrector=score_corrector,
                                               corrector_kwargs=corrector_kwargs, guidance_scale=guide_scale,
-                                              unconditional_conditioning=unconditional_conditioning)
+                                              unconditional_conditioning=unconditional_conditioning, t_uniform=step)
             if callback:
                 callback(i)
             if img_callback:
@@ -132,16 +134,17 @@
     @torch.no_grad()
     def p_sample_ddim(self, x, c, t, index, repeat_noise=False, use_original_steps=False, quantize_denoised=False,
                       temperature=1., noise_dropout=0., score_corrector=None, corrector_kwargs=None,
-                      guidance_scale=1., unconditional_conditioning=None):
+                      guidance_scale=1., unconditional_conditioning=None, t_uniform=None):
         b, device = x.shape[0], x.device
         if unconditional_conditioning is None or guidance_scale == 1.:
-            e_c, e_u = self.model.apply_model(x, t, c), None
+            e_c, e_u = self.model.apply_model(x, t, c, **uniform_kw(self.model.apply_model, t_uniform)), None
         else:
             twin = self._twin_condition(c, unconditional_conditioning)
             if hasattr(self.model, "apply_model_cfg_twin"):
-                e = self.model.apply_model_cfg_twin(x, t, twin)
+                e = self.model.apply_model_cfg_twin(x, t, twin, **uniform_kw(self.model.apply_model_cfg_twin, t_uniform))
             else:
-                e = self.model.apply_model(torch.cat([x] * 2), torch.cat([t] * 2), twin)
+                e = self.model.apply_model(torch.cat([x] * 2), torch.cat([t] * 2), twin,
+                                           **uniform_kw(self.model.apply_model, t_uniform))
             e_c, e_u = e[:b], e[b:]
 
         alphas = self.model.alphas_cumprod if use_original_steps else self.ddim_alphas
@@ -194,11 +197,14 @@
         g = max_g
         x_dec = x_latent
         self._twin_cache = None
+        time_range = [int(s) for s in time_range]
+        ts_all = step_tensors(time_range, x_latent.shape[0], x_latent.device)
         for i, step in enumerate(time_range):
             index = total_steps - i - 1
-            ts = torch.full((x_latent.shape[0],), int(step), device=x_latent.device, dtype=torch.long)
+            ts = ts_all[i]
             x_dec, _ = self.p_sample_ddim(x_dec, cond, ts, index=index, use_original_steps=use_original_steps,
-                                          guidance_scale=g, unconditional_conditioning=unconditional_conditioning)
+                                          guidance_scale=g, unconditional_conditioning=unconditional_conditioning,
+                                          t_uniform=step)
             g = g - delta
         self._twin_cache = None
         return x_dec
diff --git a/adaface_amd/ldm/models/diffusion/ddpm.py b/adaface_amd/ldm/models/diffusion/ddpm.py
--- a/adaface_amd/ldm/models/diffusion/ddpm.py
+++ b/adaface_amd/ldm/models/diffusion/ddpm.py
@@ -20,7 +20,7 @@
         if conditioning_key not in (None, "crossattn"):
             raise NotImplementedError(f"conditioning_key '{conditioning_key}' is not used by SD-v1 txt2img")
 
-    def forward(self, x, t, c_concat: list = None, c_crossattn: list = None, cfg_twin: bool = False):
+    def forward(self, x, t, c_concat: list = None, c_crossattn: list = None, cfg_twin: bool = False, t_uniform=None):
         if self.conditioning_key is None:
             raise NotImplementedError("unconditional UNet is not on the path")
         c0 = c_crossattn[0]
@@ -28,9 +28,12 @@
             c_static_emb, c_in, extra_info = c0
         else:
             c_static_emb, c_in, extra_info = c0, None, None
+        kw = {}
         if cfg_twin:
-            return self.diffusion_model(x, t, context=c_static_emb, context_in=c_in, extra_info=extra_info, cfg_twin=True)
-        return self.diffusion_model(x, t, context=c_static_emb, context_in=c_in, extra_info=extra_info)
+            kw["cfg_twin"] = True
+        if t_uniform is not None:
+            kw["t_uniform"] = int(t_uniform)
+        return self.diffusion_model(x, t, context=c_static_emb, context_in=c_in, extra_info=extra_info, **kw)
 
 
 class DDPM(nn.Module):
@@ -169,25 +172,29 @@
         B, T, D = emb.shape
         return emb.unsqueeze(1).expand(B, n_layers, T, D).reshape(B * n_layers, T, D).contiguous()
 
-    def apply_model(self, x_noisy, t, cond, return_ids=False):
+    def apply_model(self, x_noisy, t, cond, return_ids=False, t_uniform=None):
         if not isinstance(cond, dict):
             if not isinstance(cond, list):
                 cond = [cond]
             key = 'c_concat' if self.model.conditioning_key == 'concat' else 'c_crossattn'
             cond = {key: cond}
+        if t_uniform is not None:
+            cond = dict(cond, t_uniform=int(t_uniform))
         x_recon = self.model(x_noisy, t, **cond)
         if isinstance(x_recon, tuple) and not return_ids:
             return x_recon[0]
         return x_recon
 
-    def apply_model_cfg_twin(self, x_noisy, t, cond_twin):
+    def apply_model_cfg_twin(self, x_noisy, t, cond_twin, t_uniform=None):
         cond = cond_twin
         if not isinstance(cond, dict):
             if not isinstance(cond, list):
                 cond = [cond]
             cond = {'c_crossattn': cond}
         if 'c_crossattn' not in cond:
-            return self.apply_model(torch.cat([x_noisy] * 2), torch.cat([t] * 2), cond_twin)
+            return self.apply_model(torch.cat([x_noisy] * 2), torch.cat([t] * 2), cond_twin, t_uniform=t_uniform)
+        if t_uniform is not None:
+            cond = dict(cond, t_uniform=int(t_uniform))
         return self.model(x_noisy, t, cfg_twin=True, **cond)
 
     @torch.no_grad()
diff --git a/adaface_amd/ldm/models/diffusion/plms.py b/adaface_amd/ldm/models/diffusion/plms.py
--- a/adaface_amd/ldm/models/diffusion/plms.py
+++ b/adaface_amd/ldm/models/diffusion/plms.py
@@ -5,7 +5,7 @@
 
 from adaface_amd import ops
 from adaface_amd.ldm.modules.diffusionmodules.util import (make_ddim_sampling_parameters, make_ddim_timesteps,
-                                                            noise_like)
+                                                            noise_like, step_tensors, uniform_kw)
 
 
 class PLMSSampler(object):
@@ -72,10 +72,13 @@
         total_steps = timesteps.shape[0]
         old_eps = []
         self._twin_cache = None
+        time_range = [int(s) for s in time_range]
+        ts_all = step_tensors(time_range, b, device)
         for i, step in enumerate(time_range):
             index = total_steps - i - 1
-            ts = torch.full((b,), int(step), device=device, dtype=torch.long)
-            ts_next = torch.full((b,), int(time_range[min(i + 1, len(time_range) - 1)]), device=device, dtype=torch.long)
+            i_next = min(i + 1, len(time_range) - 1)
+            ts = ts_all[i]
+            ts_next = ts_all[i_next]
             if mask is not None:
                 assert x0 is not None
                 img = self.model.q_sample(x0, ts) * mask + (1. - mask) * img
@@ -84,7 +87,8 @@
                                                    score_corrector=score_corrector, corrector_kwargs=corrector_kwargs,
                                                    unconditional_guidance_scale=unconditional_guidance_scale,
                                                    unconditional_conditioning=unconditional_conditioning,
-                                                   old_eps=old_eps, t_next=ts_next)
+                                                   old_eps=old_eps, t_next=ts_next, t_uniform=step,
+                                                   t_next_uniform=time_range[i_next])
             old_eps.append(e_t)
             if len(old_eps) >= 4:
                 old_eps.pop(0)
@@ -114,20 +118,22 @@
     @torch.no_grad()
     def p_sample_plms(self, x, c, t, index, repeat_noise=False, use_original_steps=False, quantize_denoised=False,
                       temperature=1., noise_dropout=0., score_corrector=None, corrector_kwargs=None,
-                      unconditional_guidance_scale=1., unconditional_conditioning=None, old_eps=None, t_next=None):
+                      unconditional_guidance_scale=1., unconditional_conditioning=None, old_eps=None, t_next=None,
+                      t_uniform=None, t_next_uniform=None):
         if quantize_denoised or score_corrector is not None or use_original_steps:
             raise NotImplementedError("quantize_denoised / score_corrector / use_original_steps are not on the txt2img path")
         b = x.shape[0]
         f32 = lambda v: float(np.float32(float(v)))
 
-        def get_model_output(xx, tt):
+        def get_model_output(xx, tt, step=None):
             if unconditional_conditioning is None or unconditional_guidance_scale == 1.:
-                return self.model.apply_model(xx, tt, c)
+                return self.model.apply_model(xx, tt, c, **uniform_kw(self.model.apply_model, step))
             twin = self._twin_condition(c, unconditional_conditioning)
             if hasattr(self.model, "apply_model_cfg_twin"):
-                e = self.model.apply_model_cfg_twin(xx, tt, twin)
+                e = self.model.apply_model_cfg_twin(xx, tt, twin, **uniform_kw(self.model.apply_model_cfg_twin, step))
             else:
-                e = self.model.apply_model(torch.cat([xx] * 2), torch.cat([tt] * 2), twin)
+                e = self.model.apply_model(torch.cat([xx] * 2), torch.cat([tt] * 2), twin,
+                                           **uniform_kw(self.model.apply_model, step))
             return ops.lincomb([(e[b:], unconditional_guidance_scale), (e[:b], 0.0)], cfg=True)
 
         def get_x_prev_and_pred_x0(e, idx):
@@ -139,10 +145,10 @@
                                  f32(self.ddim_sqrt_one_minus_alphas[idx]), sigma_t,
                                  None if sigma_t == 0. else noise, temperature)
 
-        e_t = get_model_output(x, t)
+        e_t = get_model_output(x, t, t_uniform)
         if len(old_eps) == 0:
             x_prev, _ = get_x_prev_and_pred_x0(e_t, index)
-            e_t_next = get_model_output(x_prev, t_next)
+            e_t_next = get_model_output(x_prev, t_next, t_next_uniform)
             e_t_prime = ops.lincomb([(e_t, 0.5), (e_t_next, 0.5)])
         elif len(old_eps) == 1:
             e_t_prime = ops.lincomb([(e_t, 3 / 2), (old_eps[-1], -1 / 2)])
diff --git a/adaface_amd/ldm/modules/diffusionmodules/openaimodel.py b/adaface_amd/ldm/modules/diffusionmodules/openaimodel.py
--- a/adaface_amd/ldm/modules/diffusionmodules/openaimodel.py
+++ b/adaface_amd/ldm/modules/diffusionmodules/openaimodel.py
@@ -122,7 +122,8 @@
         return (ks, tuple(batch), tuple(tokens))
 
     @torch.no_grad()
-    def forward(self, x, timesteps=None, context=None, y=None, context_in=None, extra_info=None, cfg_twin=False, **kwargs):
+    def forward(self, x, timesteps=None, context=None, y=None, context_in=None, extra_info=None, cfg_twin=False,
+                t_uniform=None, **kwargs):
         if y is not None:
             raise NotImplementedError("class-conditional UNet (num_classes) is not on the path")
         if timesteps is None or context is None:
@@ -146,7 +147,7 @@
             eng.set_context(context.to(x.device), B, layerwise)
             object.__setattr__(self, "_ctx_key", key if cache_ok else None)
             object.__setattr__(self, "_ctx_ref", context)
-        out = (eng.unet_forward_twin if cfg_twin else eng.unet_forward)(x, timesteps.to(x.device))
+        out = (eng.unet_forward_twin if cfg_twin else eng.unet_forward)(x, timesteps.to(x.device), t_uniform=t_uniform)
         if extra_info is not None:
             extra_info["ca_layers_activations"] = {k: {} for k in ("outfeat", "attn", "attnscore", "q")}
         return out.type(x.dtype) if x.dtype != torch.float32 else out
diff --git a/adaface_amd/ldm/modules/diffusionmodules/util.py b/adaface_amd/ldm/modules/diffusionmodules/util.py
--- a/adaface_amd/ldm/modules/diffusionmodules/util.py
+++ b/adaface_amd/ldm/modules/diffusionmodules/util.py
@@ -62,3 +62,21 @@
     if max_period != 10000 or repeat_only:
         raise NotImplementedError("only max_period=10000, repeat_only=False is on the hot path")
     return ops.timestep_embedding(timesteps, dim, dtype=dtype)
+
+
+def step_tensors(time_range, b, device):
+    steps = torch.as_tensor([int(s) for s in time_range], dtype=torch.long)
+    return steps.unsqueeze(1).repeat(1, b).to(device)
+
+
+def uniform_kw(fn, step):
+    if step is None:
+        return {}
+    import inspect
+    try:
+        params = inspect.signature(fn).parameters
+    except (TypeError, ValueError):
+        return {}
+    if "t_uniform" in params or any(p.kind is p.VAR_KEYWORD for p in params.values()):
+        return {"t_uniform": int(step)}
+    return {}
diff --git a/include/adaface_hip.h b/include/adaface_hip.h
--- a/include/adaface_hip.h
+++ b/include/adaface_hip.h
@@ -53,6 +53,11 @@
                     void* stream);
 int af_unet_forward_twin(af_handle* h, const float* x_dev, const int64_t* t_dev, float* eps_dev, int Bf, int H, int W,
                          void* stream);
+int af_unet_forward_t(af_handle* h, const float* x_dev, const int64_t* t_dev, int64_t t_value, float* eps_dev, int Bf, int H,
+                      int W, void* stream);
+int af_unet_forward_twin_t(af_handle* h, const float* x_dev, const int64_t* t_dev, int64_t t_value, float* eps_dev, int Bf,
+                           int H, int W, void* stream);
+int af_temb_cache_stats(af_handle* h, int64_t* hits, int64_t* misses, int64_t* entries);
 
 int af_clip_embed_tokens(af_handle* h, const int64_t* ids_dev, int64_t n, float* emb_dev, void* stream);
 int af_clip_text_forward(af_handle* h, const float* inputs_embeds_dev, int Bn, int T, float w_prev, float w_last,
@@ -132,6 +137,7 @@
 int64_t af_attn_short_launches(void);
 int64_t af_xattn_fused_launches(void);
 int64_t af_conv_attn_short_launches(void);
+int64_t af_twin_wrap_launches(void);
 int af_op_conv_attention(int dtype, const float* q_dev, const float* k_dev, const float* v_dev, float* o_dev, int B, int Hh,
                          int Ww, int Nk, int heads, int dh, float scale, int ks, int n_groups, int path, void* stream);
 int af_op_xattn_fused(const float* x_dev, const float* ln_stats_dev, const float* gamma_dev, const float* beta_dev,
```
